# michalfratczak/habdec

Hardware: AMD Instinct MI355X
Metric: IQ Msamples/s (batched 2.048 MS/s streams) (higher is better)
Workload: dtype f32

## Files before the change

### habdec_amd/csrc/dev_types.h

```cpp
#pragma once
#include <stdint.h>
#ifndef __HIPCC__
#ifndef __host__
#define __host__
#define __device__
#endif
#endif

namespace hd {

constexpr int kFftBins = 4096;
constexpr uint32_t kVentLimit = 30000;
constexpr uint32_t kFirBatch = 256;

struct StreamCall {
    uint32_t n_in;
    uint32_t n1;
    uint32_t n2;
    uint32_t zero_hist1;
    uint32_t zero_hist2;
    uint32_t pend_before;
    uint32_t fft_fill;
    uint32_t fft_take;
    uint32_t fft_run;
    uint32_t fir_m;
    uint32_t fir_taps;
    uint32_t fir_zero_hist;
    uint32_t pend_after;
    uint32_t dc_remove;
    uint32_t clear_pending;
    uint32_t fir_taps_prev;
};
__host__ __device__ inline uint32_t sc_taps_prev(const StreamCall& c) { return c.fir_taps_prev & 0xFFFFu; }
__host__ __device__ inline uint32_t sc_head_n(const StreamCall& c) { return (c.fir_taps_prev >> 16) & 0x3FFFu; }
__host__ __device__ inline bool sc_head_prev(const StreamCall& c) { return (c.fir_taps_prev >> 30) & 1u; }
__host__ __device__ inline bool sc_head_save(const StreamCall& c) { return (c.fir_taps_prev >> 31) & 1u; }
__host__ __device__ inline uint32_t sc_pack_taps_prev(uint32_t taps_prev, uint32_t head_n, bool head_prev, bool head_save)
{ return (taps_prev & 0xFFFFu) | ((head_n & 0x3FFFu) << 16) | ((head_prev ? 1u : 0u) << 30) | ((head_save ? 1u : 0u) << 31); }


struct SymbolParams {
    uint32_t spb;
    uint32_t R;
    uint32_t min_held;
    uint32_t float_abs;
    uint32_t reset;
};

struct SymState {
    uint32_t base;
    uint32_t held;
    uint32_t cached;
    uint32_t run_pos;
    float    run_sum;
    uint32_t _pad[3];
};

struct BitsHeader {
    uint32_t nbits;
    uint32_t held_after;
    uint32_t nflips;
    uint32_t overflow;
    uint32_t uncached;
    uint32_t demod_ck[2];
    uint32_t demod_n;
    uint32_t seq;
    uint32_t _pad[3];
};
static_assert(sizeof(BitsHeader) == 48, "result slot header");

struct SpectrumStatsDev {
    int32_t valid;
    int32_t peak1, peak2;
    float power1, power2;
    uint32_t seq;
    double mean, sigma;
};

}
```

### habdec_amd/csrc/engine.cpp

```cpp
#include <hip/hip_runtime.h>
#include <rocfft/rocfft.h>

#include <algorithm>
#include <atomic>
#include <chrono>
#include <cmath>
#include <cstdio>
#include <cstdlib>
#include <cstring>
#include <memory>
#include <condition_variable>
#include <mutex>
#include <thread>
#include <string>
#include <vector>

#include "../../include/habdec_amd.h"
#include "dev_types.h"
#include "host/afc_tracker.hpp"
#include "host/decim_plan.hpp"
#include "host/fir_design.hpp"
#include "host/iq_file_batch.hpp"
#include "host/survey.hpp"
#include "host/text_stage.hpp"
#include "host/tune_host.hpp"
#include "kernels/launch.h"
#include "kernels/survey.h"

#define HDK(fn, ...) (e->fast ? hd::fast::fn(__VA_ARGS__) : hd::exact::fn(__VA_ARGS__))

namespace {

thread_local std::string g_err;
int fail(int code, const std::string& msg) { g_err = msg; return code; }

#define HD_HIP(call)                                                                                   \
    do {                                                                                               \
        hipError_t e_ = (call);                                                                        \
        if (e_ != hipSuccess) return fail(HD_ERR_DEVICE, std::string(#call) + ": " + hipGetErrorString(e_)); \
    } while (0)

template <typename T>
struct DevBuf {
    T* p = nullptr;
    size_t n = 0;
    hipError_t alloc(size_t count)
    {
        n = count;
        hipError_t e = hipMalloc(reinterpret_cast<void**>(&p), std::max<size_t>(count, 1) * sizeof(T));
        if (e == hipSuccess) e = hipMemset(p, 0, std::max<size_t>(count, 1) * sizeof(T));
        return e;
    }
    ~DevBuf() { if (p) (void)hipFree(p); }
};
template <typename T>
struct PinBuf {
    T* p = nullptr;
    T* dev = nullptr;
    size_t n = 0;
    hipError_t alloc(size_t count)
    {
        n = count;
        hipError_t e = hipHostMalloc(reinterpret_cast<void**>(&p), std::max<size_t>(count, 1) * sizeof(T), hipHostMallocMapped | hipHostMallocCoherent);
        if (e == hipSuccess) std::memset(p, 0, std::max<size_t>(count, 1) * sizeof(T));
        if (e == hipSuccess) e = hipHostGetDevicePointer(reinterpret_cast<void**>(&dev), p, 0);
        return e;
    }
    ~PinBuf() { if (p) (void)hipHostFree(p); }
};

struct SizeState {
    size_t stage_buf[2] = {0, 0};
    size_t pending = 0;
    size_t fft_fill = 0;
    size_t fir_buf = 0;
    uint32_t fir_T_run = 0;
    uint32_t head_n = 0;
    uint64_t head_call = ~0ull;
    bool head_aside = false;
    uint32_t tune_phase = 0;
    uint32_t front_phase = 0;
    uint32_t win_ub = 0, inflight_m = 0;
    uint32_t last_n2 = 0, last_pend_before = 0, last_m = 0;
    int last_buf = 0;
};

struct StreamHost {
    double baud = 300;
    float lp_bw = 1500, lp_trans = 0.025f;
    bool dc = false;
    hd::LowpassDesigner lp;
    bool taps_dirty = false;
    uint32_t tune_step = 0;
    uint32_t held = 0;
    bool sym_reset = true;
    hd::TextStage text;
    hd::AfcTracker afc;
    hd::SpectrumStats stats{};
    bool have_spectrum = false;
    uint64_t spectra = 0;
    uint32_t last_nbits = 0, last_nflips = 0;
    uint64_t flip_list_full = 0;
    uint64_t bits_total = 0;
    std::vector<uint32_t> last_words;
    uint32_t demod_ck[2] = {0, 0}, demod_ck_n = 0xFFFFFFFFu;
    uint64_t demod_ck_call = 0;
    uint64_t demod_ck_hash = 0xCBF29CE484222325ull;
    uint64_t demod_ck_calls = 0, demod_ck_unknown = 0;
    double tune_hz = 0;
    uint64_t tune_from = 0, retunes = 0;
    bool auto_afc = false;
    double afc_hold_s = 6.0, afc_min_hz = 100.0;
    uint64_t afc_elapsed = 0;
    double front_hz = 0;
    uint32_t front_step = 0;
    uint64_t front_from = 0;
};

}

struct hd_engine {
    hd_engine_config cfg{};
    double fs = 0, fsd = 0;
    std::vector<hd::DecimStage> stages;
    uint32_t S = 0, D = 1;
    uint32_t n1_cap = 0, n2_cap = 0;
    uint32_t taps_cap = 0, fir_hist_cap = 0;
    size_t fbuf_stride = 0;
    uint32_t tail_cap = 0, backlog_cap = 0, slot_words = 0, flips_cap = 0, max_R = 0, min_R = 4;
    int bins_sep = 8;
    bool decode_enabled = true;
    bool fast = false;
    bool one_stream = false;
    bool no_tail = false;
    uint32_t tail_max_n2 = 2048;
    int last_route = -1;
    struct PendingTail { bool valid = false; hd::TailArgs ta{}; int slot = 0; int r2 = 0, t2 = 0; } pend;
    DevBuf<float2> fft_tw;
    bool no_claim = false;
    uint32_t step_run = 0;
    bool no_cu_step = false;
    uint32_t ring_run = 0;
    uint32_t ring_chain = 1;
    uint32_t ring_short_pct = 25;
    bool ring_short_set = false;
#ifndef HD_S1_SLOTS_BATCH
#define HD_S1_SLOTS_BATCH 4
#endif
    static constexpr uint32_t kS1Slots = HD_S1_SLOTS_BATCH;
    PinBuf<unsigned int> ring_gave_up;
    std::string fail_cause;
    bool device_failed = false;
    uint64_t step_launches = 0;
    DevBuf<unsigned int> step_ctr;
    uint32_t pend_max_taps = 0;
    bool dec_wgs_forced = false;
#ifdef HD_TIMING_EXPERIMENT
    int cu_exp = 0;
#else
    static constexpr int cu_exp = 0;
#endif
    uint32_t n_cus = 0, dec_wgs_per_cu = 0;
    hipStream_t qa = nullptr, qb = nullptr, qc = nullptr;
    hipStream_t qh = nullptr;
    DevBuf<float2> staging2;
    hipEvent_t ev_copy[2] = {nullptr, nullptr}, ev_staging_free[2] = {nullptr, nullptr};
    bool staging_used[2] = {false, false};
    uint64_t host_calls = 0, host_calls_in_place = 0;
    uint32_t timing_every = 8;
    hd_timing last_timing{};
    static constexpr uint32_t kLpFftMinTaps = 1024;
    uint32_t lpf_N[2] = {0, 0};
    rocfft_plan lpf_fwd[2] = {nullptr, nullptr}, lpf_inv[2] = {nullptr, nullptr};
    rocfft_execution_info lpf_info = nullptr;
    DevBuf<char> lpf_workbuf;
    DevBuf<float2> lpf_x, lpf_k;
    PinBuf<uint32_t> lpf_ntaps;
    uint32_t lpf_k_N = 0;
    bool lpf_k_stale = true;
    uint64_t lpf_calls = 0;

    DevBuf<float2> staging, dec1, dec1b, dec1c, hist1[2], hist2[2], fbuf[3], fft_in, spec, filtered;
    DevBuf<float> stage_taps[2], lp_taps, power, demod, tail, weight;
    DevBuf<unsigned long long> flipmask;
    DevBuf<uint32_t> flips_dbg;
    DevBuf<hd::SymState> d_symstate;
    DevBuf<hd::DemodCarry> carry[2];
    DevBuf<float2> fir_head;
    DevBuf<float> tune_tab;
    DevBuf<uint32_t> demod_ck_acc;
    uint32_t head_cap = 0;
    DevBuf<hd::SymbolParams> d_sym;
    PinBuf<hd::SymbolParams> h_sym;
    static constexpr int kSlots = 4;
    struct CallSlot {
        DevBuf<hd::StreamCall> d_call;
        PinBuf<hd::StreamCall> h_call;
        PinBuf<uint32_t> h_slots;
        PinBuf<hd::SpectrumStatsDev> h_stats;
        PinBuf<uint2> h_tune;
        PinBuf<uint2> h_front;
        bool timed = false, timed_step = false;
        hipEvent_t ev_front = nullptr, ev_done = nullptr, ev_params = nullptr, ev_spec = nullptr, t0 = nullptr, t1 = nullptr, t2 = nullptr, t3 = nullptr;
        bool busy = false;
        uint32_t seq = 0;
        uint64_t total_in = 0;
        uint32_t r1 = 1;
        ~CallSlot() { for (hipEvent_t ev : {ev_front, ev_done, ev_params, ev_spec, t0, t1, t2, t3}) if (ev) (void)hipEventDestroy(ev); }
    } slot[kSlots];
    uint64_t calls = 0;
    uint64_t delivered = 0;
    int cur = 0;
    int hist_cur = 0;
    int carry_cur = 0;
    bool sym_dirty = true;

    std::vector<StreamHost> st;
    std::vector<SizeState> mirror, mirror_next;
    std::recursive_mutex mtx;
    bool in_callback = false;
    hd_sentence_cb sentence_cb = nullptr; void* sentence_user = nullptr;
    hd_match_cb match_cb = nullptr; void* match_user = nullptr;
    hd_chars_cb chars_cb = nullptr; void* chars_user = nullptr;
    uint64_t sentences_ok = 0;

    ~hd_engine()
    {
        for (rocfft_plan pl : {lpf_fwd[0], lpf_fwd[1], lpf_inv[0], lpf_inv[1]}) if (pl) rocfft_plan_destroy(pl);
        if (lpf_info) rocfft_execution_info_destroy(lpf_info);
        if (qa) (void)hipStreamDestroy(qa);
        if (qb && qb != qa) (void)hipStreamDestroy(qb);
        if (qc && qc != qa) (void)hipStreamDestroy(qc);
        if (qh) (void)hipStreamDestroy(qh);
        for (hipEvent_t ev : {ev_copy[0], ev_copy[1], ev_staging_free[0], ev_staging_free[1]}) if (ev) (void)hipEventDestroy(ev);
    }
};

namespace {

std::once_flag g_rocfft_once;

hd::SymbolParams symbol_params(const hd_engine* e, const StreamHost& s)
{
    hd::SymbolParams p{};
    p.float_abs = e->cfg.lookup_mode ? 1u : 0u;
    p.min_held = 0xFFFFFFFFu;
    p.spb = 0; p.R = 4;
    if (e->fsd > 0 && s.baud > 0) {
        const double spb = std::round(e->fsd / s.baud);
        if (spb >= 1 && spb < 1e9) {
            p.spb = (uint32_t)spb;
            p.R = (uint32_t)std::max(4, int(p.spb / 4));
            p.min_held = (uint32_t)std::ceil(e->fsd / s.baud * 3);
        }
    }
    return p;
}

float cutoff_rel(const hd_engine* e, const StreamHost& s) { return (float)(s.lp_bw / e->fsd); }

int check_stream(const hd_engine* e, uint32_t s)
{
    if (!e) return fail(HD_ERR_INVALID, "null engine");
    if (s >= e->S) return fail(HD_ERR_INVALID, "stream index out of range");
    return HD_OK;
}

}

extern "C" {

const char* hd_last_error(void) { return g_err.c_str(); }

uint32_t hd_min_chunk(uint32_t decimation)
{
    std::vector<hd::DecimStage> st;
    if (!hd::decim_plan(decimation, st)) return 0;
    uint64_t need = decimation ? decimation : 1;
    uint64_t r = 1;
    for (const auto& g : st) { need = std::max<uint64_t>(need, (uint64_t)(g.taps.size() - 1) * r); r *= (uint64_t)g.ratio; }
    const uint64_t d = decimation ? decimation : 1;
    return (uint32_t)((need + d - 1) / d * d);
}

void hd_engine_config_default(hd_engine_config* c)
{
    std::memset(c, 0, sizeof(*c));
    c->device = 0; c->n_streams = 1; c->max_chunk = 65536; c->sampling_rate = 2.048e6; c->decimation = 64;
    c->baud = 300; c->rtty_bits = 8; c->rtty_stops = 2; c->lowpass_bw_hz = 1500; c->lowpass_trans = 0.025f;
    c->dc_remove = 0; c->lookup_mode = 1; c->enable_spectrum = 1; c->ungated = 0; c->keep_filtered = 0; c->pipeline = 0; c->arith = HD_ARITH_EXACT;
}

int hd_engine_create(const hd_engine_config* cfg, hd_engine** out)
{
    if (!cfg || !out) return fail(HD_ERR_INVALID, "null argument");
    *out = nullptr;
    if (cfg->n_streams < 1) return fail(HD_ERR_INVALID, "n_streams must be >= 1");
    if (!(cfg->sampling_rate > 0)) return fail(HD_ERR_INVALID, "sampling_rate must be > 0");
    if (cfg->max_chunk < 1) return fail(HD_ERR_INVALID, "max_chunk must be >= 1");
    if (cfg->arith != HD_ARITH_EXACT && cfg->arith != HD_ARITH_FAST) return fail(HD_ERR_INVALID, "arith must be HD_ARITH_EXACT (0) or HD_ARITH_FAST (1)");
    std::unique_ptr<hd_engine> e(new hd_engine);
    e->cfg = *cfg;
    e->fast = cfg->arith == HD_ARITH_FAST;
    if (!hd::decim_plan(cfg->decimation, e->stages))
        return fail(HD_ERR_INVALID, "Unsupported decimation factor: " + std::to_string(cfg->decimation));
    e->S = cfg->n_streams;
    e->D = cfg->decimation;
    if (cfg->max_chunk % e->D) return fail(HD_ERR_INVALID, "max_chunk must be a multiple of the decimation factor");
    e->fs = (double)(float)cfg->sampling_rate;
    e->fsd = e->fs / (double)e->D;
    e->decode_enabled = cfg->ungated || !(e->fsd > 4 * 40e3);
    if (cfg->baud > 0 && e->fsd / cfg->baud < 3.5)
        return fail(HD_ERR_UNSUPPORTED, "symbol rate above a third of the decimated rate (fewer than 4 samples per bit): the symbol extractor's windows would overlap");
    {
        const float rel = (float)(500.0f / e->fsd);
        e->bins_sep = std::max(8, (int)std::round((double)rel * (double)hd::kFftBins));
    }

    int ndev = 0;
    if (hipGetDeviceCount(&ndev) != hipSuccess || ndev <= cfg->device || cfg->device < 0)
        return fail(HD_ERR_DEVICE, "no HIP device " + std::to_string(cfg->device) + " (this library has no CPU path)");
    HD_HIP(hipSetDevice(cfg->device));
    HD_HIP(hipStreamCreateWithFlags(&e->qa, hipStreamNonBlocking));
    e->one_stream = cfg->pipeline == 0;
    e->no_tail = getenv("HD_NO_TAIL") != nullptr;
    e->no_claim = getenv("HD_NO_CLAIM") != nullptr;
    if (const char* v = getenv("HD_STEP_RUN")) e->step_run = (uint32_t)atoi(v);
    e->no_cu_step = getenv("HD_NO_CU_STEP") != nullptr;
    if (const char* v = getenv("HD_RING_RUN")) e->ring_run = (uint32_t)atoi(v);
    if (const char* v = getenv("HD_RING_CHAIN")) e->ring_chain = atoi(v) ? 1u : 0u;
    if (const char* v = getenv("HD_RING_SHORT_PCT")) { e->ring_short_pct = std::min<uint32_t>((uint32_t)atoi(v), 100u); e->ring_short_set = true; }
    if (const char* v = getenv("HD_TAIL_MAX_N2")) e->tail_max_n2 = (uint32_t)strtoul(v, nullptr, 0);
    {
        hipDeviceProp_t prop;
        HD_HIP(hipGetDeviceProperties(&prop, cfg->device));
        e->n_cus = (uint32_t)prop.multiProcessorCount;
        e->dec_wgs_per_cu = cfg->pipeline ? 6u : 8u;
        if (const char* v = getenv("HD_DEC_WGS_PER_CU")) { e->dec_wgs_per_cu = (uint32_t)atoi(v); e->dec_wgs_forced = true; }
#ifdef HD_TIMING_EXPERIMENT
        if (const char* v = getenv("HD_CU_EXP")) e->cu_exp = atoi(v);
#endif
    }
    for (hipEvent_t* ev : {&e->ev_copy[0], &e->ev_copy[1], &e->ev_staging_free[0], &e->ev_staging_free[1]}) HD_HIP(hipEventCreateWithFlags(ev, hipEventDisableTiming));
    if (e->one_stream) e->qb = e->qc = e->qa;
    else {
        if (!e->qb) HD_HIP(hipStreamCreateWithFlags(&e->qb, hipStreamNonBlocking));
        HD_HIP(hipStreamCreateWithFlags(&e->qc, hipStreamNonBlocking));
    }
    for (auto& sl : e->slot) {
        static const unsigned ev_flags = (unsigned)hipEventDisableSystemFence;
        HD_HIP(hipEventCreateWithFlags(&sl.ev_front, hipEventDisableTiming | ev_flags));
        HD_HIP(hipEventCreateWithFlags(&sl.ev_done, hipEventDisableTiming | ev_flags));
        HD_HIP(hipEventCreateWithFlags(&sl.ev_params, hipEventDisableTiming | ev_flags));
        HD_HIP(hipEventCreateWithFlags(&sl.ev_spec, hipEventDisableTiming | ev_flags));
        for (hipEvent_t* ev : {&sl.t0, &sl.t1, &sl.t2, &sl.t3}) HD_HIP(hipEventCreateWithFlags(ev, ev_flags));
    }

    const uint32_t S = e->S;
    const uint32_t r0 = e->stages.size() > 0 ? e->stages[0].ratio : 1;
    e->n1_cap = cfg->max_chunk / r0;
    e->n2_cap = cfg->max_chunk / e->D;
    const uint32_t m_cap = ((e->n2_cap + hd::kFirBatch - 1) / hd::kFirBatch) * hd::kFirBatch + hd::kFirBatch;
    e->taps_cap = (m_cap | 1u) + 1u;
    e->fir_hist_cap = (e->taps_cap + 1u) & ~1u;
    e->fbuf_stride = (size_t)e->fir_hist_cap + hd::kFirBatch + e->n2_cap + 2;
    e->fbuf_stride = (e->fbuf_stride + 1) & ~(size_t)1;
    e->backlog_cap = hd::kVentLimit + 1 + m_cap;
    e->tail_cap = 1u;
    while (e->tail_cap < hd::kVentLimit + 1 + m_cap + 1024) e->tail_cap <<= 1;

    e->st.resize(S);
    e->mirror.resize(S);
    e->mirror_next.resize(S);
    for (auto& s : e->st) {
        s.baud = cfg->baud; s.lp_bw = cfg->lowpass_bw_hz; s.lp_trans = cfg->lowpass_trans; s.dc = cfg->dc_remove != 0;
        s.text.framer.nbits = cfg->rtty_bits; s.text.framer.nstops = cfg->rtty_stops;
        s.lp.float_trig = cfg->lookup_mode != 0;
    }
    {
        const hd::SymbolParams p = symbol_params(e.get(), e->st[0]);
        const uint32_t spb = std::max<uint32_t>(p.spb, 1);
        uint32_t bits = 3u * e->backlog_cap / spb + 64u;
        bits = std::max<uint32_t>(256u, (bits + 31u) & ~31u);
        e->slot_words = (uint32_t)(sizeof(hd::BitsHeader) / 4) + bits / 32;
        e->max_R = std::max<uint32_t>(p.R, 4);
        e->min_R = e->max_R;
    }
    e->flips_cap = cfg->keep_filtered ? 256 : 0;

    HD_HIP(e->staging.alloc((size_t)S * cfg->max_chunk));
    if (e->stages.size() == 2) for (auto* b : {&e->dec1, &e->dec1b, &e->dec1c}) HD_HIP(b->alloc((size_t)S * e->n1_cap));
    HD_HIP(e->step_ctr.alloc(2 * 16 * 32 + 32));
    HD_HIP(e->ring_gave_up.alloc(4));
    e->ring_gave_up.p[0] = 0;
    if (!e->no_claim && e->n_cus % 32u == 0) {
        const uint32_t n_xcd = e->n_cus / 32u;
        HD_HIP(hipDeviceSynchronize());
        const uint32_t seen = HDK(probe_xcc_mask, e->qa, e->n_cus, e->step_ctr.p + 2 * 16 * 32);
        if (n_xcd > 16 || seen != (n_xcd >= 32 ? 0xFFFFFFFFu : (1u << n_xcd) - 1u)) e->no_claim = true;
    } else
        e->no_claim = true;
    if (e->stages.size() >= 1) {
        for (auto& h : e->hist1) HD_HIP(h.alloc((size_t)S * (e->stages[0].taps.size() - 1)));
        HD_HIP(e->stage_taps[0].alloc(e->stages[0].taps.size() + 1));
        HD_HIP(hipMemcpy(e->stage_taps[0].p, e->stages[0].taps.data(), e->stages[0].taps.size() * 4, hipMemcpyHostToDevice));
    }
    if (e->stages.size() == 2) {
        for (auto& h : e->hist2) HD_HIP(h.alloc((size_t)S * (e->stages[1].taps.size() - 1)));
        HD_HIP(e->stage_taps[1].alloc(e->stages[1].taps.size() + 1));
        HD_HIP(hipMemcpy(e->stage_taps[1].p, e->stages[1].taps.data(), e->stages[1].taps.size() * 4, hipMemcpyHostToDevice));
    }
    for (auto& b : e->fbuf) HD_HIP(b.alloc((size_t)S * e->fbuf_stride));
    HD_HIP(e->lp_taps.alloc((size_t)S * e->taps_cap));
    HD_HIP(e->demod.alloc((size_t)S * m_cap));
    if (cfg->keep_filtered) HD_HIP(e->filtered.alloc((size_t)S * m_cap));
    HD_HIP(e->tail.alloc((size_t)S * e->tail_cap));
    HD_HIP(e->weight.alloc((size_t)S * e->tail_cap));
    HD_HIP(e->flipmask.alloc((size_t)S * (e->tail_cap / 64)));
    HD_HIP(e->d_symstate.alloc(S));
    if (e->flips_cap) HD_HIP(e->flips_dbg.alloc((size_t)S * e->flips_cap));
    for (auto& c : e->carry) HD_HIP(c.alloc(S));
    e->head_cap = std::min<uint32_t>(e->taps_cap, 8192u);
    HD_HIP(e->fir_head.alloc((size_t)S * e->head_cap));
    HD_HIP(e->demod_ck_acc.alloc((size_t)2 * S));
    HD_HIP(e->d_sym.alloc(S));
    HD_HIP(e->h_sym.alloc(S));
    for (auto& sl : e->slot) {
        HD_HIP(sl.d_call.alloc(S));
        HD_HIP(sl.h_call.alloc(S));
        HD_HIP(sl.h_slots.alloc((size_t)S * e->slot_words));
        HD_HIP(sl.h_tune.alloc(S));
        HD_HIP(sl.h_front.alloc(S));
    }
    {
        std::vector<float> tab(4 * hd::kTuneTable);
        hd::tune_tables(tab.data(), tab.data() + 2 * hd::kTuneTable);
        HD_HIP(e->tune_tab.alloc(tab.size()));
        HD_HIP(hipMemcpy(e->tune_tab.p, tab.data(), tab.size() * sizeof(float), hipMemcpyHostToDevice));
    }
    if (cfg->enable_spectrum) {
        HD_HIP(e->fft_in.alloc((size_t)S * hd::kFftBins));
        HD_HIP(e->spec.alloc((size_t)S * hd::kFftBins));
        HD_HIP(e->power.alloc((size_t)S * hd::kFftBins));
        for (auto& sl : e->slot) HD_HIP(sl.h_stats.alloc(S));
        {
            std::vector<float2> tw(hd::kFftBins);
            for (size_t m = 0; m < hd::kFftBins; ++m) {
                const double a = 2.0 * 3.14159265358979323846264338327950288 * (double)m / (double)hd::kFftBins;
                tw[m] = make_float2((float)std::cos(a), (float)-std::sin(a));
            }
            HD_HIP(e->fft_tw.alloc(hd::kFftBins));
            HD_HIP(hipMemcpy(e->fft_tw.p, tw.data(), tw.size() * sizeof(float2), hipMemcpyHostToDevice));
        }
    }
    if (e->fast && e->taps_cap >= hd_engine::kLpFftMinTaps && getenv("HD_NO_LP_FFT") == nullptr) {
        std::call_once(g_rocfft_once, [] { rocfft_setup(); });
        uint32_t N = 1;
        while (N < m_cap + e->taps_cap) N <<= 1;
        e->lpf_N[1] = N; e->lpf_N[0] = N / 2;
        size_t wmax = 0;
        for (int w = 0; w < 2; ++w) {
            const size_t len = e->lpf_N[w];
            if (rocfft_plan_create(&e->lpf_fwd[w], rocfft_placement_inplace, rocfft_transform_type_complex_forward, rocfft_precision_single, 1, &len, S, nullptr) != rocfft_status_success ||
                rocfft_plan_create(&e->lpf_inv[w], rocfft_placement_inplace, rocfft_transform_type_complex_inverse, rocfft_precision_single, 1, &len, S, nullptr) != rocfft_status_success)
                return fail(HD_ERR_DEVICE, "rocfft_plan_create (low-pass transforms) failed");
            for (rocfft_plan pl : {e->lpf_fwd[w], e->lpf_inv[w]}) { size_t wsz = 0; rocfft_plan_get_work_buffer_size(pl, &wsz); wmax = std::max(wmax, wsz); }
        }
        if (rocfft_execution_info_create(&e->lpf_info) != rocfft_status_success) return fail(HD_ERR_DEVICE, "rocfft_execution_info_create failed");
        if (wmax) { HD_HIP(e->lpf_workbuf.alloc(wmax)); rocfft_execution_info_set_work_buffer(e->lpf_info, e->lpf_workbuf.p, wmax); }
        HD_HIP(e->lpf_x.alloc((size_t)S * N));
        HD_HIP(e->lpf_k.alloc((size_t)S * N));
        HD_HIP(e->lpf_ntaps.alloc(S));
    }
    {
        hd_engine::CallSlot& sl = e->slot[0];
        hipStream_t q = e->qa;
        const uint32_t T1 = e->stages.size() > 0 ? (uint32_t)e->stages[0].taps.size() : 0, T2 = e->stages.size() > 1 ? (uint32_t)e->stages[1].taps.size() : 0;
        if (e->stages.empty()) HDK(launch_passthrough, q, S, 1, e->staging.p, cfg->max_chunk, e->fbuf[0].p, e->fbuf_stride, sl.d_call.p, e->fir_hist_cap);
        if (e->stages.size() >= 1)
            HDK(launch_decimate, q, e->stages[0].ratio, T1, S, 1, e->staging.p, cfg->max_chunk, e->hist1[0].p, e->hist1[1].p, e->stage_taps[0].p,
                                e->stages.size() == 1 ? e->fbuf[0].p : e->dec1.p, e->stages.size() == 1 ? e->fbuf_stride : e->n1_cap, sl.d_call.p, 0,
                                e->stages.size() == 1, e->fir_hist_cap, nullptr);
        if (e->stages.size() >= 1)
            HDK(launch_decimate_tuned, q, e->stages[0].ratio, T1, S, 1, e->staging.p, cfg->max_chunk, e->hist1[0].p, e->hist1[1].p, e->stage_taps[0].p,
                                      e->stages.size() == 1 ? e->fbuf[0].p : e->dec1.p, e->stages.size() == 1 ? e->fbuf_stride : e->n1_cap, sl.d_call.p,
                                      e->stages.size() == 1, e->fir_hist_cap, nullptr, 0u, sl.h_front.dev, e->tune_tab.p);
        if (e->stages.size() == 2)
            HDK(launch_decimate, q, e->stages[1].ratio, T2, S, 1, e->dec1.p, e->n1_cap, e->hist2[0].p, e->hist2[1].p, e->stage_taps[1].p, e->fbuf[0].p,
                                e->fbuf_stride, sl.d_call.p, 1, 1, e->fir_hist_cap, nullptr);
        HDK(launch_chunk_post, q, S, e->fbuf[0].p, e->fbuf_stride, sl.d_call.p, e->fir_hist_cap, nullptr, e->tune_tab.p);
        if (cfg->enable_spectrum) {
            HDK(launch_fft_feed, q, S, e->fbuf[0].p, e->fbuf_stride, e->fft_in.p, sl.d_call.p, e->fir_hist_cap);
            hd::launch_spectrum_wave(q, S, e->fft_in.p, e->fft_tw.p, e->spec.p, e->power.p, sl.h_stats.dev, sl.d_call.p, e->fsd, e->bins_sep, 0u);
        }
        HDK(launch_fir_demod, q, S, 0, 0, e->fbuf[0].p, e->fbuf_stride, e->lp_taps.p, e->taps_cap, e->demod.p, e->demod.n / S, nullptr, e->carry[0].p,
                             e->carry[1].p, sl.d_call.p, e->fir_hist_cap, e->tail.p, e->tail_cap, e->d_symstate.p, e->fbuf[1].p,
                             e->fir_head.p, e->head_cap, e->fbuf[2].p);
        HDK(launch_symbols, q, S, 1, 1, e->max_R, e->tail.p, e->tail_cap, e->d_symstate.p, e->flipmask.p, e->weight.p, e->d_sym.p, sl.d_call.p,
                           sl.h_slots.dev, e->slot_words, nullptr, 0, e->min_R, 0u);
        HD_HIP(hipStreamSynchronize(q));
        HD_HIP(hipGetLastError());
        for (auto& h : e->hist1) if (h.p) HD_HIP(hipMemset(h.p, 0, h.n * sizeof(float2)));
        for (auto& h : e->hist2) if (h.p) HD_HIP(hipMemset(h.p, 0, h.n * sizeof(float2)));
        for (auto& c : e->carry) HD_HIP(hipMemset(c.p, 0, c.n * sizeof(hd::DemodCarry)));
        HD_HIP(hipMemset(e->d_symstate.p, 0, S * sizeof(hd::SymState)));
        if (const char* b0 = getenv("HD_SYM_BASE0")) {
            hd::SymState st0{};
            st0.base = st0.cached = st0.run_pos = (uint32_t)strtoul(b0, nullptr, 0);
            std::vector<hd::SymState> v(S, st0);
            HD_HIP(hipMemcpy(e->d_symstate.p, v.data(), S * sizeof(hd::SymState), hipMemcpyHostToDevice));
        }
    }
    HD_HIP(hipDeviceSynchronize());
    *out = e.release();
    return HD_OK;
}

void hd_engine_destroy(hd_engine* e)
{
    if (!e) return;
    (void)hipSetDevice(e->cfg.device);
    (void)hipDeviceSynchronize();
    delete e;
}
// ... 115 lines not shown
    if (int r = check_stream(e, s)) return r;
    if (!out) return fail(HD_ERR_INVALID, "null argument");
    std::lock_guard<std::recursive_mutex> l(e->mtx);
    const StreamHost& st = e->st[s];
    out->offset_hz = st.front_hz; out->step = st.front_step; out->phase = e->mirror[s].front_phase; out->from_call = st.front_from;
    return HD_OK;
}
int hd_stream_set_auto_afc(hd_engine* e, uint32_t s, int on, double hold_s, double min_hz)
{
    if (int r = check_stream(e, s)) return r;
    if (!(hold_s >= 0) || !(min_hz >= 0)) return fail(HD_ERR_INVALID, "hold_s and min_hz must be >= 0");
    std::lock_guard<std::recursive_mutex> l(e->mtx);
    StreamHost& st = e->st[s];
    st.auto_afc = on != 0; st.afc_hold_s = hold_s; st.afc_min_hz = min_hz; st.afc_elapsed = 0;
    return HD_OK;
}
int hd_stream_tune(hd_engine* e, uint32_t s, hd_tune_info* out)
{
    if (int r = check_stream(e, s)) return r;
    if (!out) return fail(HD_ERR_INVALID, "null argument");
    std::lock_guard<std::recursive_mutex> l(e->mtx);
    const StreamHost& st = e->st[s];
    out->offset_hz = st.tune_hz; out->step = st.tune_step; out->phase = e->mirror[s].tune_phase;
    out->retunes = st.retunes; out->from_call = st.tune_from; out->auto_afc = st.auto_afc ? 1 : 0;
    return HD_OK;
}

}


namespace {

int run_pending_tail(hd_engine* e)
{
    if (!e->pend.valid) return HD_OK;
    hd_engine::CallSlot& ps = e->slot[e->pend.slot];
    e->pend.valid = false;
    hd::TailArgs ta = e->pend.ta;
    const int lanes = (e->S >= 2 * e->n_cus ? 64 : 256);
    hd::TailArgs lay = ta;
    if (lanes != 64) {
        if (!HDK(tail_layout, lay, lanes, e->pend.r2, e->pend.t2, e->pend_max_taps, e->max_R, e->min_R, e->tail_cap, e->pend.ta.pend_max, 64 * 1024)) return fail(HD_ERR_INVALID, "stream tail layout");
    }
    if (!HDK(launch_tail, e->qa, lanes, e->pend.r2, e->pend.t2, e->S, lay, ps.ev_done)) return fail(HD_ERR_INVALID, "stream tail refused a shape it was selected for");
    HD_HIP(hipGetLastError());
    return HD_OK;
}

int collect(hd_engine* e, hd_engine::CallSlot& sl)
{
    if (!sl.busy) return HD_OK;
    if (e->pend.valid && &e->slot[e->pend.slot] == &sl) { if (const int r = run_pending_tail(e)) return r; }
    const auto w0 = std::chrono::steady_clock::now();
    HD_HIP(hipEventSynchronize(sl.ev_done));
    const auto w1 = std::chrono::steady_clock::now();
    sl.busy = false;
    if (sl.timed) {
        float a = 0, b = 0;
        HD_HIP(hipEventElapsedTime(&b, sl.t1, sl.t2));
        if (sl.timed_step) a = b; else HD_HIP(hipEventElapsedTime(&a, sl.t0, sl.t3));
        e->last_timing.ms_total = a;
        e->last_timing.ms_front = b;
        e->last_timing.samples = sl.total_in;
        e->last_timing.front_bytes = sl.total_in * 8 + (sl.total_in / sl.r1) * 8;
        ++e->last_timing.timed_calls;
    }
    int rc = HD_OK;
    {
        const auto t_lim = std::chrono::steady_clock::now() + std::chrono::milliseconds(200);
        const bool timing_experiment = e->cu_exp != 0;
        auto await = [&](const volatile uint32_t* tag, const char* what, uint32_t s) {
            for (uint32_t spins = 0; *tag != sl.seq; ++spins) {
                if (std::chrono::steady_clock::now() > t_lim) {
                    e->device_failed = true;
                    e->fail_cause = std::string(what) + " of stream " + std::to_string(s) + " does not carry its call's tag 200 ms after the completion event";
                    rc = fail(HD_ERR_DEVICE, e->fail_cause + ": the results of this engine are unreliable -- destroy the engine");
                    return;
                }
                if (spins > 64u) std::this_thread::yield();
            }
        };
        for (uint32_t s = 0; s < e->S && !e->device_failed && !timing_experiment; ++s) {
            await(&reinterpret_cast<const volatile hd::BitsHeader*>(sl.h_slots.p + (size_t)s * e->slot_words)->seq, "result slot", s);
            if (!e->device_failed && e->cfg.enable_spectrum && sl.h_stats.p && sl.h_call.p[s].fft_run)
                await(reinterpret_cast<const volatile uint32_t*>(&sl.h_stats.p[s].seq), "spectrum statistics", s);
        }
        std::atomic_thread_fence(std::memory_order_acquire);
    }
    if (e->ring_gave_up.p && e->ring_gave_up.p[0] && !e->device_failed) {
        e->device_failed = true;
        e->fail_cause = "k_stage1_cu (loader / consumer waves): a bounded wait ran out inside a launch (word " + std::to_string(e->ring_gave_up.p[0]) + ")";
    }
    if (e->device_failed && rc == HD_OK)
        rc = fail(HD_ERR_DEVICE, e->fail_cause + ": the results of this and of every later call of this engine are unreliable -- destroy the engine");
    if (e->device_failed) {
        e->last_timing.host_wait_us = std::chrono::duration<double, std::micro>(w1 - w0).count();
        e->last_timing.host_text_us = 0;
        return rc;
    }
    for (uint32_t s = 0; s < e->S; ++s) {
        StreamHost& st = e->st[s];
        const hd::StreamCall& c = sl.h_call.p[s];
        if (c.fft_run) {
            std::memcpy(&st.stats, &sl.h_stats.p[s], sizeof(st.stats));
            st.have_spectrum = true;
            ++st.spectra;
        }
        const bool past_batch_gate = c.fir_m || c.clear_pending;
        if (past_batch_gate && e->cfg.enable_spectrum) st.afc.step(st.have_spectrum, st.stats, hd::kFftBins, e->fsd);
        st.afc_elapsed += c.n_in;
        if (st.auto_afc && (double)st.afc_elapsed >= st.afc_hold_s * e->fs && std::abs(st.afc.correction) > st.afc_min_hz) {
            const double corr = st.afc.correction;
            uint32_t d = 0;
            if (hd::tune_step(st.tune_hz + corr, e->fsd, &d)) {
                st.tune_hz += corr; st.tune_step = d; st.tune_from = e->calls;
                if (!d) e->mirror[s].tune_phase = 0;
                st.afc.reset(corr, hd::kFftBins, e->fsd);
                st.afc_elapsed = 0;
                ++st.retunes;
            }
        }
        const uint32_t* slot = sl.h_slots.p + (size_t)s * e->slot_words;
        const hd::BitsHeader* hdr = reinterpret_cast<const hd::BitsHeader*>(slot);
        SizeState& sz = e->mirror[s];
        st.held = hdr->held_after;
        sz.inflight_m -= c.fir_m;
        sz.win_ub = hdr->uncached + sz.inflight_m;
        st.last_nbits = hdr->nbits; st.last_nflips = hdr->nflips;
        st.bits_total += hdr->nbits;
        st.demod_ck[0] = hdr->demod_ck[0]; st.demod_ck[1] = hdr->demod_ck[1]; st.demod_ck_n = hdr->demod_n; st.demod_ck_call = e->delivered;
        if (hdr->demod_n != 0xFFFFFFFFu) {
            for (const uint32_t x : {hdr->demod_n, hdr->demod_ck[0], hdr->demod_ck[1]}) st.demod_ck_hash = (st.demod_ck_hash ^ x) * 0x100000001B3ull;
            ++st.demod_ck_calls;
        } else ++st.demod_ck_unknown;
        if (hdr->overflow & 1u) rc = fail(HD_ERR_CAPACITY, "symbol result slot overflow on stream " + std::to_string(s));
        if (hdr->overflow & 2u) ++st.flip_list_full;
        const uint32_t* words = slot + sizeof(hd::BitsHeader) / 4;
        st.last_words.assign(words, words + (hdr->nbits + 31) / 32);
        if (!c.fir_m) continue;
        if (hdr->nbits) st.text.framer.push_packed(words, hdr->nbits);
        const std::string chars = st.text.run(hdr->nbits != 0, [&](const hd::SentenceMatch& m) {
            ++e->sentences_ok;
            if (e->sentence_cb) { e->in_callback = true; e->sentence_cb(e->sentence_user, s, m.callsign.c_str(), m.data.c_str(), m.crc.c_str()); e->in_callback = false; }
        }, [&](const hd::SentenceMatch& m, bool ok) {
            if (e->match_cb) { e->in_callback = true; e->match_cb(e->match_user, s, m.callsign.c_str(), m.data.c_str(), m.crc.c_str(), ok ? 1 : 0); e->in_callback = false; }
        });
        if (!chars.empty() && e->chars_cb) { e->in_callback = true; e->chars_cb(e->chars_user, s, chars.data(), chars.size()); e->in_callback = false; }
    }
    e->last_timing.host_wait_us = std::chrono::duration<double, std::micro>(w1 - w0).count();
    e->last_timing.host_text_us = std::chrono::duration<double, std::micro>(std::chrono::steady_clock::now() - w1).count();
    return rc;
}

int deliver(hd_engine* e, uint64_t depth)
{
    int rc = HD_OK;
    while (e->calls - e->delivered > depth) {
        if (const int r = collect(e, e->slot[e->delivered % hd_engine::kSlots])) rc = r;
        ++e->delivered;
    }
    return rc;
}

int flush_locked(hd_engine* e)
{
    if (e->delivered < e->calls) { if (const int r = run_pending_tail(e)) return r; }
    return deliver(e, 0);
}


enum class Route : uint32_t {
    separate = 0,
    tail = 2,
    step = 3,
};

struct CallPlan {
    size_t nst = 0;
    uint32_t R1 = 1, R2 = 1, T1 = 0, T2 = 0;
    uint32_t max_in = 0, min_in = 0xFFFFFFFFu, max_n1 = 0, max_n2 = 0, max_m = 0, max_taps = 0, max_new = 0, max_pend = 0;
    uint64_t total_in = 0;
    bool any_fft = false, any_dc = false, any_zero1 = false, any_tune = false, any_lp_restart = false;
    bool any_front = false;
};

struct CallRoute {
    Route route = Route::separate;
    int tail_lanes = 64;
    hd::TailArgs ta{}, ta_step{};
    bool lean = false, free_front = false, host_params = false, any_post = false, spectrum_on_qc = false;
    const hd::StreamCall* dcall = nullptr;
    float2* feed = nullptr;
};

struct CallBufs {
    float2 *fcur, *fnext, *fprev, *d1;
    int hin, hout, cin, cout;
};

CallBufs call_bufs(const hd_engine* e)
{
    CallBufs b;
    b.fcur = e->fbuf[e->cur].p; b.fnext = e->fbuf[(e->cur + 1) % 3].p; b.fprev = e->fbuf[(e->cur + 2) % 3].p;
    b.d1 = (e->calls % 3 == 0) ? e->dec1.p : (e->calls % 3 == 1) ? e->dec1b.p : e->dec1c.p;
    b.hin = e->hist_cur; b.hout = e->hist_cur ^ 1;
    b.cin = e->carry_cur; b.cout = e->carry_cur ^ 1;
    return b;
}

int plan_call(hd_engine* e, hd_engine::CallSlot& sl, const uint32_t* n_per_stream, uint32_t n_uniform, CallPlan& p, bool& redesigned)
{
    p = CallPlan{};
    p.nst = e->stages.size();
    if (p.nst > 0) { p.R1 = e->stages[0].ratio; p.T1 = (uint32_t)e->stages[0].taps.size(); }
    if (p.nst > 1) { p.R2 = e->stages[1].ratio; p.T2 = (uint32_t)e->stages[1].taps.size(); }
    redesigned = false;
    for (uint32_t s = 0; s < e->S; ++s) {
        StreamHost& st = e->st[s];
        SizeState& nx = e->mirror_next[s];
        nx = e->mirror[s];
        hd::StreamCall c{};
        const uint32_t n = n_per_stream ? n_per_stream[s] : n_uniform;
        c.n_in = n;
        c.n1 = n / p.R1;
        c.n2 = c.n1 / p.R2;
        if (n) {
            if (p.nst > 0) { const size_t want = (size_t)n + p.T1 + p.R1; if (nx.stage_buf[0] < want) { nx.stage_buf[0] = want; c.zero_hist1 = 1; } }
            if (p.nst > 1) { const size_t want = (size_t)c.n1 + p.T2 + p.R2; if (nx.stage_buf[1] < want) { nx.stage_buf[1] = want; c.zero_hist2 = 1; } }
        }
        c.dc_remove = st.dc && c.n2;
        sl.h_tune.p[s] = make_uint2(st.tune_step, nx.tune_phase);
        if (st.tune_step) { p.any_tune = true; nx.tune_phase += c.n2 * st.tune_step; }
        sl.h_front.p[s] = make_uint2(st.front_step, nx.front_phase);
        if (st.front_step | nx.front_phase) { p.any_front = true; nx.front_phase += n * st.front_step; }
        c.pend_before = (uint32_t)nx.pending;
        nx.pending += c.n2;
        c.fft_fill = (uint32_t)nx.fft_fill;
        if (e->cfg.enable_spectrum && n && nx.fft_fill < (size_t)hd::kFftBins && c.n2) {
            c.fft_take = (uint32_t)std::min<size_t>(hd::kFftBins - nx.fft_fill, c.n2);
            nx.fft_fill += c.fft_take;
        }
        if (e->cfg.enable_spectrum && n && nx.fft_fill >= (size_t)hd::kFftBins) { c.fft_run = 1; nx.fft_fill = 0; p.any_fft = true; }
        const bool past_batch_gate = n && nx.pending >= hd::kFirBatch;
        nx.last_m = 0;
        if (past_batch_gate && !e->decode_enabled) { c.clear_pending = 1; nx.pending = 0; }
        else if (past_batch_gate) {
            const uint32_t m = (uint32_t)(nx.pending - nx.pending % hd::kFirBatch);
            st.lp.batch = m;
            if (st.lp.design(cutoff_rel(e, st), st.lp_trans)) {
                st.taps_dirty = true;
                redesigned = true;
            }
            const uint32_t T = (uint32_t)st.lp.taps.size();
            if (!T) return fail(HD_ERR_UNSUPPORTED, "low-pass transition width leaves no taps (reference filters nothing then)");
            if (T > e->taps_cap) return fail(HD_ERR_CAPACITY, "low-pass tap count exceeds engine capacity");
            if (nx.fir_buf < (size_t)m + T) { nx.fir_buf = (size_t)m + T; c.fir_zero_hist = 1; }
            c.fir_m = m; c.fir_taps = T;
            c.fir_taps_prev = hd::sc_pack_taps_prev(nx.fir_T_run ? nx.fir_T_run : T, nx.head_n, !nx.head_aside && nx.head_call + 1 == e->calls, false);
            nx.fir_T_run = T;
            nx.head_n = std::min<uint32_t>(m, std::min<uint32_t>(e->head_cap, 0x3FFFu)); nx.head_call = e->calls; nx.head_aside = false;
            nx.pending -= m;
            nx.last_m = m;
            p.max_m = std::max(p.max_m, m);
            p.max_taps = std::max(p.max_taps, T);
            p.any_lp_restart |= c.fir_zero_hist != 0;
            const uint32_t pending_windows = st.sym_reset ? std::max(st.held, nx.win_ub) : nx.win_ub;
            p.max_new = std::max(p.max_new, pending_windows + m + 64u);
            nx.inflight_m += m;
            nx.win_ub += m;
        }
        if (!c.fir_m && nx.head_n && !nx.head_aside) {
            if (nx.head_call + 1 == e->calls) c.fir_taps_prev = hd::sc_pack_taps_prev(0, nx.head_n, false, true);
            else nx.head_n = 0;
            nx.head_aside = true;
        }
        c.pend_after = (uint32_t)nx.pending;
        p.max_pend = std::max(p.max_pend, std::max(c.pend_before, c.pend_after));
        nx.last_n2 = c.n2; nx.last_pend_before = c.pend_before; nx.last_buf = e->cur;
        sl.h_call.p[s] = c;
        p.max_in = std::max(p.max_in, n); p.min_in = std::min(p.min_in, n); p.max_n1 = std::max(p.max_n1, c.n1); p.max_n2 = std::max(p.max_n2, c.n2);
        p.any_dc |= c.dc_remove != 0;
        p.any_zero1 |= c.zero_hist1 != 0;
        p.total_in += n;
    }
    sl.total_in = p.total_in;
    sl.r1 = p.R1;
    sl.seq = (uint32_t)(e->calls + 1u);
    if (!sl.seq) sl.seq = 1u;
    return HD_OK;
}

void route_call(hd_engine* e, hd_engine::CallSlot& sl, const CallPlan& p, CallRoute& r)
{
    const uint32_t S = e->S;
    const int R2 = (int)p.R2, T2 = (int)p.T2;
    r = CallRoute{};
    r.tail_lanes = S >= 2 * e->n_cus ? 64 : 256;
    const bool tail = p.nst == 2 && !p.any_dc && !e->no_tail && p.max_n2 <= e->tail_max_n2 &&
                      ((r.tail_lanes == 256 && p.max_n2 >= 512u && HDK(tail_layout, r.ta, r.tail_lanes, R2, T2, p.max_taps, e->max_R, e->min_R, e->tail_cap, p.max_pend, 64 * 1024, 4)) ||
                       HDK(tail_layout, r.ta, r.tail_lanes, R2, T2, p.max_taps, e->max_R, e->min_R, e->tail_cap, p.max_pend, 64 * 1024));
    const uint32_t step_lds = (p.R1 == 32 || p.R1 == 64) ? HDK(step_lds_bytes, (int)p.R1, (int)p.T1) : 0u;
    const bool step = tail && !p.any_front && e->cfg.pipeline && !e->one_stream && p.min_in == p.max_in && p.max_in && step_lds &&
                      HDK(tail_layout, r.ta_step, 64, R2, T2, p.max_taps, e->max_R, e->min_R, e->tail_cap, p.max_pend, step_lds);
    r.route = step ? Route::step : tail ? Route::tail : Route::separate;
    r.any_post = p.any_dc || (p.any_tune && !tail);
    r.lean = tail && !e->one_stream;
    r.free_front = !tail && p.nst == 2 && !e->one_stream;
    r.host_params = tail && !step && e->one_stream;
    r.dcall = r.host_params ? sl.h_call.dev : sl.d_call.p;
    r.feed = (e->cfg.enable_spectrum && !r.any_post) ? e->fft_in.p : nullptr;
    if (r.route != Route::separate || !e->cfg.enable_spectrum || r.any_post || !p.any_fft) return;
    for (uint32_t s = 0; s < S; ++s) {
        hd::StreamCall& c = sl.h_call.p[s];
        if (c.fft_run == 1 && c.fft_fill == 0 && c.fft_take == (uint32_t)hd::kFftBins) { c.fft_take = 0; c.fft_run = 2; }
    }
    r.spectrum_on_qc = !e->one_stream && p.nst != 0;
    for (uint32_t s = 0; s < S && r.spectrum_on_qc; ++s) r.spectrum_on_qc = sl.h_call.p[s].fft_run != 1u;
}

void fill_tail(const hd_engine* e, const hd_engine::CallSlot& sl, const CallPlan& p, const CallRoute& r, const CallBufs& b, hd::TailArgs& t)
{
    t.dec1 = b.d1; t.dec1_stride = e->n1_cap; t.hist2_in = e->hist2[b.hin].p; t.hist2_out = e->hist2[b.hout].p; t.taps2 = e->stage_taps[1].p;
    t.fbuf = b.fcur; t.fbuf_next = b.fnext; t.fbuf_stride = e->fbuf_stride; t.fir_hist_cap = e->fir_hist_cap;
    t.lp_taps = e->lp_taps.p; t.taps_stride = e->taps_cap; t.demod = e->demod.p; t.demod_stride = e->demod.n / e->S;
    t.filtered = e->cfg.keep_filtered ? e->filtered.p : nullptr; t.carry_in = e->carry[b.cin].p; t.carry_out = e->carry[b.cout].p;
    t.tune = p.any_tune ? sl.h_tune.dev : nullptr; t.tune_tab = e->tune_tab.p;
    t.call = r.dcall; t.fft_in = r.feed; t.head_buf = e->fir_head.p; t.fbuf_prev = b.fprev; t.head_cap = e->head_cap;
    t.n_streams = e->S;
    t.ring = e->tail.p; t.ring_cap = e->tail_cap; t.sym = e->d_symstate.p; t.flipmask = e->flipmask.p; t.wsum = e->weight.p;
    t.sp = e->d_sym.p; t.slots = sl.h_slots.dev; t.slot_words = e->slot_words; t.seq = sl.seq;
    t.flips_dbg = e->flips_cap ? e->flips_dbg.p : nullptr; t.flips_cap = e->flips_cap;
    t.fft_tw = r.feed ? e->fft_tw.p : nullptr;
    t.spec = e->spec.p; t.power = e->power.p; t.stats = sl.h_stats.dev; t.rate = e->fsd; t.bins_sep = e->bins_sep;
}

hd::StepClaim make_claim(const hd_engine* e, const CallPlan& p, uint32_t run_len_cu )
{
    hd::StepClaim claim{};
    const int R1 = (int)p.R1, T1 = (int)p.T1;
    const uint64_t S = e->S;
    const uint32_t ntiles = run_len_cu ? HDK(ring_tiles, R1, T1, p.max_in) : (p.max_n1 + 63) / 64, n_xcd = e->n_cus / 32u, run_len = run_len_cu ? run_len_cu : e->step_run >= 2 ? e->step_run : 4u;
    const uint64_t runs = S * ntiles / run_len;
    const bool shape_ok = run_len_cu ? (HDK(stage1_cu_supported, R1, T1) && p.max_in % 2048u == 0) : ((R1 == 32 || R1 == 64) && p.max_n1 % 64 == 0);
    if (!e->no_claim && (p.nst == 2 || (run_len_cu && p.nst == 1)) && shape_ok && p.min_in == p.max_in && p.max_in && !p.any_zero1 && n_xcd && e->n_cus % 32u == 0 && n_xcd <= 16 &&
        ntiles && (ntiles % run_len == 0 || (run_len_cu && R1 >= 32 && (S * ntiles) % run_len == 0)) && runs % n_xcd == 0 && S * ntiles < (1ull << 32)) {
        claim.ctr = e->step_ctr.p + (size_t)(e->step_launches & 1u) * 16 * 32;
        claim.ctr_next = e->step_ctr.p + (size_t)((e->step_launches & 1u) ^ 1u) * 16 * 32;
        claim.n_xcd = n_xcd; claim.runs_per_xcd = (uint32_t)(runs / n_xcd); claim.run_len = run_len;
        if (run_len_cu && R1 >= 32 && e->ring_short_pct) {
            const uint32_t tpx = claim.runs_per_xcd * run_len, whole = (uint32_t)((uint64_t)tpx * (100u - e->ring_short_pct) / 100u) / run_len;
            claim.tiles_per_xcd = tpx; claim.short_from = whole; claim.runs_per_xcd = whole + (tpx - whole * run_len);
        }
        if (run_len_cu && R1 == 32 && e->ring_chain && S % n_xcd == 0) {
            const uint32_t hr = (uint32_t)((T1 - 1 + 31) / 32), rows = p.max_in / 32u, rl = e->ring_run >= 2u ? e->ring_run : 4u, sx = (uint32_t)(S / n_xcd);
            const hd::RingSchedule ch = hd::ring_schedule(rows, hr, rl, true), pl = hd::ring_schedule(rows, hr, 1u, false);
            const uint32_t sp = hd::ring_plain_streams(sx, e->ring_short_set ? e->ring_short_pct : 12u);
            if (ch.chained && pl.ntiles && (uint64_t)sx * pl.ntiles < (1ull << 31)) {
                claim.chain_rl = ch.rl; claim.chain_sx = sx; claim.chain_sc = sx - sp;
                claim.chain_nfull = ch.n_full; claim.chain_kclose = ch.k_close; claim.chain_ntp = pl.ntiles;
                claim.runs_per_xcd = hd::ring_tickets(ch, pl, sx, sx - sp);
                claim.run_len = ch.rl; claim.short_from = 0xFFFFFFFFu; claim.tiles_per_xcd = 0;
            }
        }
    }
    return claim;
}

uint32_t pick_ring_run(const hd_engine* e, uint32_t R1, uint32_t ntiles)
{
    const uint64_t S = e->S;
    const uint32_t n_xcd = e->n_cus / 32u ? e->n_cus / 32u : 1u, want = R1 >= 32 ? 4u : 8u;
    auto ok = [&](uint32_t r) { return r >= 2u && r <= ntiles && (R1 >= 32 ? (S * ntiles) % r == 0 : ntiles % r == 0) && (S * ntiles / r) % n_xcd == 0; };
    if (e->ring_run >= 2 && ok(e->ring_run)) return e->ring_run;
    for (uint32_t d = 0; d <= 8u; ++d) {
        if (ok(want + d)) return want + d;
        if (d && d < want && ok(want - d)) return want - d;
    }
    return 2u;
}

int enqueue_uploads(hd_engine* e, hd_engine::CallSlot& sl, const CallRoute& r)
{
    const uint32_t S = e->S;
    hipStream_t qa = e->qa;
    if (e->last_route >= 0 && e->last_route != (int)r.route) {
        if (const int rc = run_pending_tail(e)) return rc;
        HD_HIP(hipStreamSynchronize(qa)); HD_HIP(hipStreamSynchronize(e->qb));
    }
    e->last_route = (int)r.route;
    e->last_timing.path = (uint32_t)r.route;
    if (!r.lean && !r.free_front && e->calls >= 2 && !e->one_stream) HD_HIP(hipStreamWaitEvent(qa, e->slot[(e->calls - 2) % hd_engine::kSlots].ev_done, 0));
    const bool step = r.route == Route::step;
    sl.timed = e->timing_every && (e->calls % e->timing_every) == 0;
    sl.timed_step = sl.timed && step;
    if (sl.timed && !step) HD_HIP(hipEventRecord(sl.t0, qa));
    if (!r.lean && !r.free_front && !r.host_params) {
        HDK(launch_fetch_params, e->qc, sl.h_call.dev, sl.d_call.p, S * sizeof(hd::StreamCall));
        if (!e->one_stream) { HD_HIP(hipEventRecord(sl.ev_params, e->qc)); HD_HIP(hipStreamWaitEvent(qa, sl.ev_params, 0)); }
    }
    for (uint32_t s = 0; s < S; ++s) {
        StreamHost& st = e->st[s];
        if (!st.taps_dirty) continue;
        HD_HIP(hipMemcpyAsync(e->lp_taps.p + (size_t)s * e->taps_cap, st.lp.taps.data(), st.lp.taps.size() * 4, hipMemcpyHostToDevice, qa));
        st.taps_dirty = false;
        e->lpf_k_stale = true;
    }
    if (e->sym_dirty) {
        uint32_t mr = 4;
        for (uint32_t s = 0; s < S; ++s) {
            e->h_sym.p[s] = symbol_params(e, e->st[s]);
            e->h_sym.p[s].reset = e->st[s].sym_reset ? 1u : 0u;
            mr = std::max(mr, e->h_sym.p[s].R);
        }
        e->max_R = mr;
        { uint32_t lo = mr; for (uint32_t s2 = 0; s2 < S; ++s2) lo = std::min(lo, std::max<uint32_t>(e->h_sym.p[s2].R, 4)); e->min_R = lo; }
        HD_HIP(hipMemcpyAsync(e->d_sym.p, e->h_sym.p, S * sizeof(hd::SymbolParams), hipMemcpyHostToDevice, qa));
// ... 102 lines not shown
                                                    call1, 0, single ? 1 : 0, e->fir_hist_cap, single ? r.feed : nullptr, lin1)))
                return fail(HD_ERR_INVALID, "no kernel for this decimation stage");
        }
        if (sl.timed) HD_HIP(hipEventRecord(sl.t2, qa));
        if (r.free_front) HDK(launch_fetch_params, qa, sl.h_call.dev, sl.d_call.p, S * sizeof(hd::StreamCall));
        if (!single && !tail) {
            if (!HDK(launch_decimate, qa, p.R2, p.T2, S, p.max_n2, b.d1, e->n1_cap, e->hist2[b.hin].p, e->hist2[b.hout].p, e->stage_taps[1].p, b.fcur,
                                     e->fbuf_stride, r.dcall, 1, 1, e->fir_hist_cap, r.feed))
                return fail(HD_ERR_INVALID, "no kernel for this decimation stage");
        }
    }
    if (!tail) {
        if (r.any_post) HDK(launch_chunk_post, qa, S, b.fcur, e->fbuf_stride, r.dcall, e->fir_hist_cap, p.any_tune ? sl.h_tune.dev : nullptr, e->tune_tab.p);
        if (!r.spectrum_on_qc) call_spectrum(e, qa, sl, p, r);
    }
    if (!e->one_stream) HD_HIP(hipEventRecord(sl.ev_front, qa));
    if (r.spectrum_on_qc) {
        HD_HIP(hipStreamWaitEvent(e->qc, sl.ev_front, 0));
        call_spectrum(e, e->qc, sl, p, r);
        HD_HIP(hipEventRecord(sl.ev_spec, e->qc));
    }
    return HD_OK;
}

int lowpass_transforms(hd_engine* e, const CallPlan& p, const CallRoute& r, const CallBufs& b, uint32_t* lpN)
{
    *lpN = 0;
    if (!e->fast || !e->lpf_N[1] || p.max_taps < hd_engine::kLpFftMinTaps || !p.max_m || p.any_lp_restart) return HD_OK;
    const uint32_t S = e->S, Lmax = p.max_m + p.max_taps - 1;
    const int w = Lmax <= e->lpf_N[0] ? 0 : Lmax <= e->lpf_N[1] ? 1 : -1;
    if (w < 0) return HD_OK;
    const uint32_t N = e->lpf_N[w];
    hipStream_t qb = e->qb;
    rocfft_execution_info_set_stream(e->lpf_info, qb);
    if (e->lpf_k_stale || e->lpf_k_N != N) {
        for (uint32_t s = 0; s < S; ++s) e->lpf_ntaps.p[s] = (uint32_t)e->st[s].lp.taps.size();
        HDK(launch_lp_taps_gather, qb, S, e->lp_taps.p, e->taps_cap, e->lpf_ntaps.dev, e->lpf_k.p, N);
        void* kb[1] = {e->lpf_k.p};
        if (rocfft_execute(e->lpf_fwd[w], kb, nullptr, e->lpf_info) != rocfft_status_success) return fail(HD_ERR_DEVICE, "rocfft_execute (low-pass taps) failed");
        e->lpf_k_N = N; e->lpf_k_stale = false;
    }
    HDK(launch_lp_gather, qb, S, b.fcur, e->fbuf_stride, e->lpf_x.p, N, r.dcall, e->fir_hist_cap, e->fir_head.p, e->head_cap, b.fprev);
    void* xb[1] = {e->lpf_x.p};
    if (rocfft_execute(e->lpf_fwd[w], xb, nullptr, e->lpf_info) != rocfft_status_success) return fail(HD_ERR_DEVICE, "rocfft_execute (low-pass forward) failed");
    HDK(launch_lp_mul, qb, S, e->lpf_x.p, e->lpf_k.p, N, r.dcall);
    if (rocfft_execute(e->lpf_inv[w], xb, nullptr, e->lpf_info) != rocfft_status_success) return fail(HD_ERR_DEVICE, "rocfft_execute (low-pass inverse) failed");
    ++e->lpf_calls;
    *lpN = N;
    return HD_OK;
}

int enqueue_back(hd_engine* e, hd_engine::CallSlot& sl, const CallPlan& p, CallRoute& r)
{
    const uint32_t S = e->S;
    hipStream_t qb = e->qb;
    const CallBufs b = call_bufs(e);
    if (!e->one_stream) HD_HIP(hipStreamWaitEvent(qb, sl.ev_front, 0));
    const bool ev_ride = !sl.timed && e->one_stream;
    if (r.route == Route::tail) {
        if (r.lean) HDK(launch_fetch_params, qb, sl.h_call.dev, sl.d_call.p, S * sizeof(hd::StreamCall));
        fill_tail(e, sl, p, r, b, r.ta);
        if (!HDK(launch_tail, qb, r.tail_lanes, (int)p.R2, (int)p.T2, S, r.ta, ev_ride ? sl.ev_done : nullptr)) return fail(HD_ERR_INVALID, "stream tail refused a shape it was selected for");
    } else {
        uint32_t lpN = 0;
        if (const int rc = lowpass_transforms(e, p, r, b, &lpN)) return rc;
        HDK(launch_fir_demod, qb, S, p.max_m, lpN ? 0u : p.max_taps, b.fcur, e->fbuf_stride, e->lp_taps.p, e->taps_cap, e->demod.p, e->demod.n / S,
                             e->cfg.keep_filtered ? e->filtered.p : nullptr, e->carry[b.cin].p, e->carry[b.cout].p, r.dcall, e->fir_hist_cap,
                             e->tail.p, e->tail_cap, e->d_symstate.p, b.fnext, e->fir_head.p, e->head_cap, b.fprev, e->demod_ck_acc.p,
                             lpN ? e->lpf_x.p : nullptr, lpN, lpN ? 1.0f / (float)lpN : 1.0f);
        HDK(launch_symbols, qb, S, p.max_m, p.max_new, e->max_R, e->tail.p, e->tail_cap, e->d_symstate.p, e->flipmask.p, e->weight.p, e->d_sym.p,
                           r.dcall, sl.h_slots.dev, e->slot_words, e->flips_cap ? e->flips_dbg.p : nullptr, e->flips_cap, e->min_R, sl.seq, ev_ride ? sl.ev_done : nullptr,
                           e->demod_ck_acc.p);
    }
    if (sl.timed) HD_HIP(hipEventRecord(sl.t3, qb));
    if (r.spectrum_on_qc) HD_HIP(hipStreamWaitEvent(qb, sl.ev_spec, 0));
    if (!ev_ride) HD_HIP(hipEventRecord(sl.ev_done, qb));
    HD_HIP(hipGetLastError());
    return HD_OK;
}

void commit_call(hd_engine* e, hd_engine::CallSlot& sl, const CallPlan& p, const CallRoute& r)
{
    e->mirror.swap(e->mirror_next);
    sl.busy = true;
    if (r.route == Route::step) {
        e->pend.valid = true; e->pend.ta = r.ta_step; e->pend.slot = (int)(e->calls % hd_engine::kSlots);
        e->pend.r2 = (int)p.R2; e->pend.t2 = (int)p.T2; e->pend_max_taps = p.max_taps;
    }
    e->cur = (e->cur + 1) % 3;
    e->carry_cur ^= 1;
    if (p.max_in && p.nst) e->hist_cur ^= 1;
    ++e->calls;
}

}

extern "C" {

int hd_flush(hd_engine* e)
{
    if (!e) return fail(HD_ERR_INVALID, "null engine");
    std::lock_guard<std::recursive_mutex> lock(e->mtx);
    if (e->in_callback) return fail(HD_ERR_INVALID, "hd_flush cannot be called from a sentence / character callback (the delivery it would join is the one running)");
    HD_HIP(hipSetDevice(e->cfg.device));
    const int rc = flush_locked(e);
    if (e->device_failed) return fail(HD_ERR_DEVICE, "this engine is in its failed state (" + e->fail_cause + ") -- destroy the engine");
    return rc;
}

int hd_process_device(hd_engine* e, const void* d_iq, size_t stride, const uint32_t* n_per_stream, uint32_t n_uniform)
{
    if (!e) return fail(HD_ERR_INVALID, "null engine");
    if (!d_iq) return fail(HD_ERR_INVALID, "null IQ pointer");
    if ((reinterpret_cast<uintptr_t>(d_iq) & 15) || (stride & 1)) return fail(HD_ERR_INVALID, "IQ base must be 16-byte aligned and stream_stride even");
    std::lock_guard<std::recursive_mutex> lock(e->mtx);
    if (e->in_callback) return fail(HD_ERR_INVALID, "hd_process_* cannot be called from a sentence / character callback");
    if (e->device_failed) return fail(HD_ERR_DEVICE, "this engine is in its failed state (" + e->fail_cause + "): no new calls are accepted -- destroy the engine");
    const auto h0 = std::chrono::steady_clock::now();
    HD_HIP(hipSetDevice(e->cfg.device));
    const size_t nst = e->stages.size();
    const uint32_t T1 = nst > 0 ? (uint32_t)e->stages[0].taps.size() : 0, T2 = nst > 1 ? (uint32_t)e->stages[1].taps.size() : 0;
    const uint32_t R1 = nst > 0 ? e->stages[0].ratio : 1;

    for (uint32_t s = 0; s < e->S; ++s) {
        const uint32_t n = n_per_stream ? n_per_stream[s] : n_uniform;
        if (n > e->cfg.max_chunk) return fail(HD_ERR_CAPACITY, "more samples than max_chunk");
        if (n % e->D) return fail(HD_ERR_INVALID, "sample count must be a multiple of the decimation factor (queue the remainder)");
        if (n && nst > 0 && n + 1 < T1) return fail(HD_ERR_UNSUPPORTED, "chunk shorter than the first stage's history (undefined in the reference)");
        if (n && nst > 1 && n / R1 + 1 < T2) return fail(HD_ERR_UNSUPPORTED, "chunk shorter than the second stage's history (undefined in the reference)");
    }
    if (const int rc = deliver(e, hd_engine::kSlots - 1)) return rc;
    bool tables_dirty = e->sym_dirty;
    for (uint32_t s = 0; s < e->S && !tables_dirty; ++s) tables_dirty = e->st[s].taps_dirty;
    if (tables_dirty) { if (const int rc = flush_locked(e)) return rc; }
    hd_engine::CallSlot& sl = e->slot[e->calls % hd_engine::kSlots];
    CallPlan p;
    bool redesigned = false;
    do {
        if (redesigned) { if (const int rc = flush_locked(e)) return rc; }
        if (const int rc = plan_call(e, sl, n_per_stream, n_uniform, p, redesigned)) return rc;
    } while (redesigned);
    CallRoute r;
    route_call(e, sl, p, r);

    const float2* iq = static_cast<const float2*>(d_iq);
    int rc = enqueue_uploads(e, sl, r);
    if (!rc) rc = r.route == Route::step ? enqueue_step(e, sl, p, r, iq, stride) : enqueue_front(e, sl, p, r, iq, stride);
    if (!rc && r.route != Route::step) rc = enqueue_back(e, sl, p, r);
    if (rc) {
        e->device_failed = true;
        e->fail_cause = "call " + std::to_string(e->calls) + " was enqueued in part (" + g_err + ")";
        return rc;
    }
    commit_call(e, sl, p, r);
    e->last_timing.host_enqueue_us = std::chrono::duration<double, std::micro>(std::chrono::steady_clock::now() - h0).count();

    const uint64_t depth = !e->cfg.pipeline ? 0u : (r.route == Route::step && e->cfg.pipeline >= 2) ? 3u : 2u;
    return deliver(e, depth);
}

void* hd_pinned_alloc(size_t bytes)
{
    void* p = nullptr;
    if (hipHostMalloc(&p, bytes ? bytes : 1, hipHostMallocMapped | hipHostMallocPortable) != hipSuccess) { (void)hipGetLastError(); return nullptr; }
    return p;
}
// ... 87 lines not shown
            b.alive = src->batch.next(b.iq, stride, b.n.data());
            {
                std::lock_guard<std::mutex> l(m);
                filled = r + 1;
            }
            cv.notify_all();
            if (!b.alive && !looping) return;
        }
    });
    int rc = HD_OK;
    uint64_t total = 0;
    for (uint64_t r = 0; r < max_rounds; ++r) {
        {
            std::unique_lock<std::mutex> l(m);
            cv.wait(l, [&] { return filled > r; });
        }
        Slab& b = slab[r % kSlabs];
        if (!b.alive) {
            if (!looping) break;
            { std::lock_guard<std::mutex> l(m); consumed = r + 1; }
            cv.notify_all();
            continue;
        }
        bool uniform = true;
        for (uint32_t s = 1; s < S; ++s) uniform = uniform && b.n[s] == b.n[0];
        rc = hd_process_host(e, b.iq, stride, uniform ? nullptr : b.n.data(), uniform ? b.n[0] : 0);
        if (rc) break;
        for (uint32_t s = 0; s < S; ++s) total += b.n[s];
        {
            std::lock_guard<std::mutex> l(m);
            consumed = r + 1;
        }
        cv.notify_all();
    }
    {
        std::lock_guard<std::mutex> l(m);
        stop = true;
    }
    cv.notify_all();
    reader.join();
    const int rf = hd_flush(e);
    HD_HIP(hipDeviceSynchronize());
    release();
    if (samples_done) *samples_done = total;
    return rc ? rc : rf;
}


static size_t copy_out(const std::string& s, char* buf, size_t cap)
{
    if (buf && cap) { const size_t n = std::min(cap - 1, s.size()); std::memcpy(buf, s.data(), n); buf[n] = 0; }
    return s.size();
}
static size_t take_out(std::string& s, char* buf, size_t cap)
{
    const size_t n = copy_out(s, buf, cap);
    if (buf && cap > n) s.clear();
    return n;
}

size_t hd_stream_rtty(hd_engine* e, uint32_t s, char* buf, size_t cap)
{ if (check_stream(e, s)) return 0; std::lock_guard<std::recursive_mutex> l(e->mtx); return copy_out(e->st[s].text.stream, buf, cap); }
size_t hd_stream_last_sentence(hd_engine* e, uint32_t s, char* buf, size_t cap)
{ if (check_stream(e, s)) return 0; std::lock_guard<std::recursive_mutex> l(e->mtx); return copy_out(e->st[s].text.last_sentence, buf, cap); }
size_t hd_stream_take_sentences(hd_engine* e, uint32_t s, char* buf, size_t cap)
{ if (check_stream(e, s)) return 0; std::lock_guard<std::recursive_mutex> l(e->mtx); return take_out(e->st[s].text.ok_log, buf, cap); }
size_t hd_stream_take_matches(hd_engine* e, uint32_t s, char* buf, size_t cap)
{ if (check_stream(e, s)) return 0; std::lock_guard<std::recursive_mutex> l(e->mtx); return take_out(e->st[s].text.match_log, buf, cap); }
size_t hd_stream_take_chars(hd_engine* e, uint32_t s, char* buf, size_t cap)
{ if (check_stream(e, s)) return 0; std::lock_guard<std::recursive_mutex> l(e->mtx); return take_out(e->st[s].text.char_log, buf, cap); }

int hd_stream_afc(hd_engine* e, uint32_t s, hd_afc_info* out)
{
    if (int r = check_stream(e, s)) return r;
    if (!out) return fail(HD_ERR_INVALID, "null argument");
    std::lock_guard<std::recursive_mutex> l(e->mtx);
    const StreamHost& st = e->st[s];
    out->frequency_correction = st.afc.correction; out->shift_hz = st.afc.shift_hz;
    out->noise_floor = st.afc.noise_floor; out->noise_variance = st.afc.noise_sigma;
    out->peak_left = st.afc.gui_left; out->peak_right = st.afc.gui_right; out->spectra = st.spectra;
    return HD_OK;
}

static size_t fetch(hd_engine* e, const void* dev, size_t count, size_t elem, void* host, size_t cap)
{
    if (e->in_callback) { fail(HD_ERR_INVALID, "data getters cannot be called from a sentence / character callback (text getters can)"); return 0; }
    (void)flush_locked(e);
    const size_t n = std::min(count, cap);
    if (!n || !host) return count;
    if (hipSetDevice(e->cfg.device) != hipSuccess) return 0;
    if (hipMemcpy(host, dev, n * elem, hipMemcpyDeviceToHost) != hipSuccess) return 0;
    return count;
}

size_t hd_stream_spectrum(hd_engine* e, uint32_t s, float* iq, size_t cap)
{
    if (check_stream(e, s)) return 0;
    std::lock_guard<std::recursive_mutex> l(e->mtx);
    if (!e->cfg.enable_spectrum || !e->st[s].have_spectrum) return 0;
    return fetch(e, e->spec.p + (size_t)s * hd::kFftBins, hd::kFftBins, sizeof(float2), iq, cap);
}
size_t hd_stream_power(hd_engine* e, uint32_t s, float* p, size_t cap)
{
    if (check_stream(e, s)) return 0;
    std::lock_guard<std::recursive_mutex> l(e->mtx);
    if (!e->cfg.enable_spectrum || !e->st[s].have_spectrum) return 0;
    return fetch(e, e->power.p + (size_t)s * hd::kFftBins, hd::kFftBins, sizeof(float), p, cap);
}
size_t hd_stream_demodulated(hd_engine* e, uint32_t s, float* v, size_t cap)
{
    if (check_stream(e, s)) return 0;
    std::lock_guard<std::recursive_mutex> l(e->mtx);
    return fetch(e, e->demod.p + (size_t)s * (e->demod.n / e->S), e->mirror[s].last_m, sizeof(float), v, cap);
}
size_t hd_stream_decimated(hd_engine* e, uint32_t s, float* iq, size_t cap)
{
    if (check_stream(e, s)) return 0;
    std::lock_guard<std::recursive_mutex> l(e->mtx);
    const SizeState& sz = e->mirror[s];
    const float2* src = e->fbuf[sz.last_buf].p + (size_t)s * e->fbuf_stride + e->fir_hist_cap + sz.last_pend_before;
    return fetch(e, src, sz.last_n2, sizeof(float2), iq, cap);
}
size_t hd_stream_filtered(hd_engine* e, uint32_t s, float* iq, size_t cap)
{
    if (check_stream(e, s)) return 0;
    std::lock_guard<std::recursive_mutex> l(e->mtx);
    if (!e->cfg.keep_filtered) return 0;
    return fetch(e, e->filtered.p + (size_t)s * (e->demod.n / e->S), e->mirror[s].last_m, sizeof(float2), iq, cap);
}
size_t hd_stream_bits(hd_engine* e, uint32_t s, uint8_t* bits, size_t cap)
{
    if (check_stream(e, s)) return 0;
    std::lock_guard<std::recursive_mutex> l(e->mtx);
    const StreamHost& st = e->st[s];
    for (uint32_t i = 0; i < st.last_nbits && i < cap; ++i) bits[i] = (st.last_words[i >> 5] >> (i & 31)) & 1u;
    return st.last_nbits;
}
size_t hd_stream_flips(hd_engine* e, uint32_t s, uint32_t* flips, size_t cap)
{
    if (check_stream(e, s)) return 0;
    std::lock_guard<std::recursive_mutex> l(e->mtx);
    if (!e->flips_cap) return 0;
    const size_t n = std::min<size_t>(e->st[s].last_nflips, e->flips_cap);
    return fetch(e, e->flips_dbg.p + (size_t)s * e->flips_cap, n, sizeof(uint32_t), flips, cap);
}
size_t hd_stream_fir_taps(hd_engine* e, uint32_t s, float* taps, size_t cap)
{
    if (check_stream(e, s)) return 0;
    std::lock_guard<std::recursive_mutex> l(e->mtx);
    const auto& t = e->st[s].lp.taps;
    if (taps) std::memcpy(taps, t.data(), std::min(cap, t.size()) * sizeof(float));
    return t.size();
}
uint64_t hd_stream_bits_total(hd_engine* e, uint32_t s)
{
    if (check_stream(e, s)) return 0;
    std::lock_guard<std::recursive_mutex> l(e->mtx);
    return e->st[s].bits_total;
}
uint64_t hd_stream_flip_list_full(hd_engine* e, uint32_t s)
{
    if (check_stream(e, s)) return 0;
    std::lock_guard<std::recursive_mutex> l(e->mtx);
    return e->st[s].flip_list_full;
}
int hd_stream_demod_checksum(hd_engine* e, uint32_t s, uint64_t* call_index, uint32_t* n, uint32_t ck[2])
{
    if (check_stream(e, s)) return HD_ERR_INVALID;
    std::lock_guard<std::recursive_mutex> l(e->mtx);
    const StreamHost& st = e->st[s];
    if (call_index) *call_index = st.demod_ck_call;
    if (n) *n = st.demod_ck_n;
    if (ck) { ck[0] = st.demod_ck[0]; ck[1] = st.demod_ck[1]; }
    return HD_OK;
}
int hd_stream_demod_checksum_total(hd_engine* e, uint32_t s, uint64_t* calls, uint64_t* calls_without, uint64_t* hash)
{
    if (check_stream(e, s)) return HD_ERR_INVALID;
    std::lock_guard<std::recursive_mutex> l(e->mtx);
    const StreamHost& st = e->st[s];
    if (calls) *calls = st.demod_ck_calls;
    if (calls_without) *calls_without = st.demod_ck_unknown;
    if (hash) *hash = st.demod_ck_hash;
    return HD_OK;
}
uint32_t hd_stream_symbol_backlog(hd_engine* e, uint32_t s)
{
    if (check_stream(e, s)) return 0;
    std::lock_guard<std::recursive_mutex> l(e->mtx);
    return e->st[s].held;
}

}


struct hd_survey {
// ... 201 lines not shown
```

### habdec_amd/csrc/kernels/decimate.hip

```cpp
#include <hip/hip_runtime.h>
#include <hip/hip_ext.h>
#include <type_traits>
#include <cstdlib>

#include "launch.h"
#include "tune.h"
#include "tail_body.h"
#include "stage1_ring.h"

#ifndef HD_FRONT_SWEEPS
#define HD_FRONT_SWEEPS 2
#endif
#define HD_DEC_MAXW 4

namespace hd {
namespace HD_ARITH_NS {

#ifdef HD_STAMP_DEC
#ifndef HD_STAMP_DEC_D
#define HD_STAMP_DEC_D 32
#endif
__device__ unsigned long long g_dec_stamps[4096 * 8];
extern "C" void HD_DBG_NAME(hd_debug_dec_stamps)(unsigned long long* host, size_t n) { (void)hipMemcpyFromSymbol(host, HIP_SYMBOL(g_dec_stamps), n * 8); }
#define DSTAMP_DECL unsigned long long ds_t = __builtin_amdgcn_s_memtime(), ds_acc[4] = {0, 0, 0, 0}; const unsigned long long ds_r0 = __builtin_amdgcn_s_memrealtime(); unsigned long long ds_r1 = 0
#define DSTAMP(i) do { if (D == HD_STAMP_DEC_D) { const unsigned long long t_ = __builtin_amdgcn_s_memtime(); ds_acc[i] += t_ - ds_t; ds_t = t_; } } while (0)
#define DSTAMP_ARRIVED() do { if (D == HD_STAMP_DEC_D) { asm volatile("s_waitcnt vmcnt(0)" ::: "memory"); DSTAMP(0); if (!ds_r1) ds_r1 = __builtin_amdgcn_s_memrealtime(); } } while (0)
#define DSTAMP_WRITE() do { if (D == HD_STAMP_DEC_D && threadIdx.x == 0) { const uint32_t w_ = by * gdx + bx; if (w_ < 4096) { \
        unsigned long long* g_ = g_dec_stamps + w_ * 8; g_[0] = ds_r0; g_[1] = ds_r1; g_[2] = __builtin_amdgcn_s_memrealtime(); \
        g_[3] = ds_acc[0]; g_[4] = ds_acc[1]; g_[5] = ds_acc[2]; g_[6] = ds_acc[3]; g_[7] = count; } } } while (0)
#else
#define DSTAMP_DECL do { } while (0)
#define DSTAMP(i) do { } while (0)
#define DSTAMP_ARRIVED() do { } while (0)
#define DSTAMP_WRITE() do { } while (0)
#endif

template <int D> constexpr int dec_opl() { return D == 2 ? 4 : D == 4 ? 4 : D == 8 ? 2 : 1; }

template <int D, int T, int TO>
constexpr int dec_tile_f4()
{
    constexpr int OPL = dec_opl<D>(), TOUT = TO * OPL, RD = OPL * D, JS = (T - 1) & 1;
    constexpr int NJJ = (TOUT - 1) * D + T + JS, NL = NJJ + 2 * (NJJ / RD) + 4;
    return (NL + 1) / 2 + TOUT / 2 + 1;
}

#ifdef HD_STAMP_TAIL
extern "C" void HD_DBG_NAME(hd_debug_step_tail_stamps)(unsigned long long* host, size_t n) { (void)hipMemcpyFromSymbol(host, HIP_SYMBOL(g_tail_stamps), n * 8); }
#endif

template <bool TUNED> struct FrontTune { static constexpr bool staged = false; };
template <> struct FrontTune<true> { uint2 tn, tn_next; bool staged; };

template <int D, int T, int TO, bool TUNED = false>
__device__ __forceinline__ void decimate_body(const float2* __restrict__ in, size_t in_stride,
                                              const float2* __restrict__ hist_in, float2* __restrict__ hist_out,
                                              const float* __restrict__ taps,
                                              float2* __restrict__ out, size_t out_stride,
                                              const StreamCall* __restrict__ call, int stage, int final_stage,
                                              uint32_t fir_hist_cap, uint32_t tiles_per_wg, float2* __restrict__ fft_in,
                                              uint32_t n_streams, uint32_t lin_ntiles, StreamCall* __restrict__ call_copy,
                                              const uint32_t bx, const uint32_t by, const uint32_t gdx, float4* __restrict__ tile4,
                                              const uint32_t uniform_n = 0 ,
                                              const StepClaim claim = StepClaim{} ,
                                              const uint2* __restrict__ ftune = nullptr ,
                                              const float* ftab = nullptr )
{
    constexpr int OPL = dec_opl<D>();
    constexpr int TOUT = TO * OPL;
    constexpr int RD = OPL * D;
    constexpr int JS = (T - 1) & 1;
    constexpr int NJ = (TOUT - 1) * D + T;
    constexpr int NJJ = NJ + JS;
    constexpr int NL = NJJ + 2 * (NJJ / RD) + 4;
    constexpr int NP = (NJJ + 1) / 2;
    constexpr int ITER = (NP + TO - 1) / TO;
    static_assert((NL + 1) / 2 + TOUT / 2 + 1 == dec_tile_f4<D, T, TO>(), "tile size helper out of step");
    float2* tile = reinterpret_cast<float2*>(tile4);
    float2* ytile = tile + ((NL + 1) & ~1);

    struct CallHead { uint32_t n_in, n1, n2, zero_hist1, zero_hist2, pend_before, fft_fill, fft_take; };
    static_assert(sizeof(CallHead) == 32, "CallHead mirrors the head of StreamCall");
    const bool linear = lin_ntiles != 0;
    uint32_t s, first, count;
    const bool claimed = claim.ctr != nullptr && claim.run_len >= 2;
    unsigned int* my_ctr = nullptr;
    unsigned int* next_ctr = nullptr;
    auto retire = [&]() { if (threadIdx.x == 0) (void)__hip_atomic_exchange(next_ctr, 0u, __ATOMIC_RELAXED, __HIP_MEMORY_SCOPE_AGENT); };
    auto draw = [&]() -> unsigned int { unsigned int t = 0; if (threadIdx.x == 0) t = __hip_atomic_fetch_add(my_ctr, 1u, __ATOMIC_RELAXED, __HIP_MEMORY_SCOPE_AGENT); return t; };
    auto drawn = [&](unsigned int t) -> unsigned int { return (unsigned int)__builtin_amdgcn_readfirstlane((int)t); };
    uint32_t xcd = 0;
    unsigned int ticket = 0;
    bool jump = false; uint32_t jump_s = 0, jump_first = 0;
    if (claimed) {
        xcd = __builtin_amdgcn_s_getreg((3 << 11) | (0 << 6) | 20) & 15u;
        if (xcd >= claim.n_xcd) xcd = claim.n_xcd - 1;
        my_ctr = claim.ctr + (size_t)xcd * 32;
        next_ctr = claim.ctr_next + (size_t)xcd * 32;
        const unsigned int r = drawn(draw());
        if (r >= claim.runs_per_xcd) { if (r == claim.runs_per_xcd) retire(); return; }
        const uint32_t g0 = (xcd * claim.runs_per_xcd + r) * claim.run_len;
        s = g0 / lin_ntiles;
        first = g0 - s * lin_ntiles;
        count = claim.run_len;
    } else if (linear) {
        const uint64_t total = (uint64_t)n_streams * lin_ntiles;
        const uint64_t g0 = (uint64_t)bx * total / gdx, g1 = (uint64_t)(bx + 1) * total / gdx;
        s = (uint32_t)(g0 / lin_ntiles);
        first = (uint32_t)(g0 - (uint64_t)s * lin_ntiles);
        count = (uint32_t)(g1 - g0);
    } else {
        s = by; first = bx * tiles_per_wg; count = tiles_per_wg;
    }
    CallHead c{};
    if (uniform_n) { c.n_in = c.n1 = uniform_n; }
    else c = *reinterpret_cast<const CallHead*>(call + s);
    const uint32_t n = stage == 0 ? c.n_in : c.n1;
    const uint32_t nout = n / D;
    const uint32_t ntiles = (nout + TOUT - 1) / TOUT;
    if (!linear) {
        if (!n && bx == 0)
            for (uint32_t j = threadIdx.x; j < (uint32_t)(T - 1); j += TO)
                hist_out[(size_t)s * (T - 1) + j] = hist_in[(size_t)s * (T - 1) + j];
        if (first >= ntiles) return;
        count = min(first + tiles_per_wg, ntiles) - first;
    }
    if (!count) return;
    uint32_t pf_s = s;
    bool pf_zero_hist = (stage == 0 ? c.zero_hist1 : c.zero_hist2) != 0;
    CallHead c_next = c;
    FrontTune<TUNED> ft;
    if constexpr (TUNED) { ft.tn = ftune[s]; ft.tn_next = ft.tn; }

    float4 r[ITER];
    auto load_tile = [&](uint32_t tile_i, const bool fast) {
        const float2* in_s = in + (size_t)pf_s * in_stride;
        const float2* hist_s = hist_in + (size_t)pf_s * (T - 1);
        const bool zero_hist = pf_zero_hist;
        auto locate = [&](long xi, bool& ok) -> const float2* {
            const bool in_hist = xi < 0;
            ok = in_hist ? (!zero_hist && xi >= -(long)(T - 1)) : (xi < (long)n);
            const long hi = xi + (T - 1);
            const float2* ph = hist_s + (hi < 0 ? 0 : hi);
            const float2* pi = in_s + (xi < 0 ? 0 : (xi < (long)n ? xi : 0));
            return in_hist ? ph : pi;
        };
        const long xe = (long)tile_i * TOUT * D - (T - 1) - JS;
        const float4* src = reinterpret_cast<const float4*>(in_s + xe);
        if (fast && __builtin_amdgcn_readfirstlane((int)(xe >= 0 && xe + 2L * ITER * TO <= (long)n))) {
            const uint64_t b64 = reinterpret_cast<uint64_t>(src);
            const char* base = reinterpret_cast<const char*>(((uint64_t)(uint32_t)__builtin_amdgcn_readfirstlane((int)(uint32_t)(b64 >> 32)) << 32) |
                                                             (uint64_t)(uint32_t)__builtin_amdgcn_readfirstlane((int)(uint32_t)b64));
            const uint32_t lane_off = threadIdx.x * 16u;
#pragma unroll
            for (int it = 0; it < ITER; ++it) r[it] = *reinterpret_cast<const float4*>(base + (lane_off + (uint32_t)it * (TO * 16u)));
            return;
        }
        uint32_t tid_ = threadIdx.x;
        asm volatile("" : "+v"(tid_));
#pragma unroll
        for (int it = 0; it < ITER; ++it) {
            const int k = (int)tid_ + it * TO;
            const long lo = xe + 2L * it * TO, hi = lo + 2L * TO;
            if (lo >= 0 && hi <= (long)n) {
                r[it] = src[k];
// ... 187 lines not shown
    #pragma unroll
                    for (int q = 0; q < B / 2; ++q) x[q] = *reinterpret_cast<const float4*>(pb + 2 * q + 2 * ((2 * q) / D));
    #pragma unroll
                    for (int q = 0; q < B / 2; ++q) {
                        mac(x[q].x, x[q].y, tb[2 * q]);
                        mac(x[q].z, x[q].w, tb[2 * q + 1]);
                    }
                }
            }
            if (NS >= B && NS % B) {
                constexpr int J0 = NFULL * B;
    #pragma unroll
                for (int jj = J0; jj < NS; jj += 2) {
                    const float4 x = *reinterpret_cast<const float4*>(p + jj + 2 * (jj / D));
                    mac(x.x, x.y, taps[jj - JS]);
                    if (jj + 1 < NS) mac(x.z, x.w, taps[jj + 1 - JS]);
                }
            }
            yq[0] = make_float2(ar, ai);
        } else {
            float ar[OPL], ai[OPL];
#pragma unroll
            for (int q = 0; q < OPL; ++q) { ar[q] = 0.f; ai[q] = 0.f; }
            constexpr int B = 16;
            constexpr int W = (OPL - 1) * D + T + JS;
            constexpr int NB = (W + B - 1) / B;
            constexpr int B_LO = (JS + (OPL - 1) * D + B - 1) / B;
            constexpr int B_HI = (T + JS) / B - 1;
            auto edge_block = [&](auto bc) {
                HD_FIR_ARITH
                constexpr int j0 = decltype(bc)::value * B;
#pragma unroll
                for (int k = 0; k < B; k += 2) {
                    if (j0 + k < W) {
                        const float4 x = *reinterpret_cast<const float4*>(p + j0 + k + 2 * ((j0 + k) / RD));
#pragma unroll
                        for (int q = 0; q < OPL; ++q) {
                            const int t0 = j0 + k - JS - q * D, t1 = t0 + 1;
                            if (t0 >= 0 && t0 < T) { ar[q] = ar[q] + x.x * taps[t0]; ai[q] = ai[q] + x.y * taps[t0]; }
                            if (t1 >= 0 && t1 < T) { ar[q] = ar[q] + x.z * taps[t1]; ai[q] = ai[q] + x.w * taps[t1]; }
                        }
                    }
                }
            };
            auto for_blocks = [&](auto lo, auto hi, auto self) {
                if constexpr (decltype(lo)::value < decltype(hi)::value) {
                    edge_block(lo);
                    self(std::integral_constant<int, decltype(lo)::value + 1>{}, hi, self);
                }
            };
            constexpr int HEAD_END = B_LO < NB ? (B_LO <= B_HI ? B_LO : NB) : NB;
            for_blocks(std::integral_constant<int, 0>{}, std::integral_constant<int, HEAD_END>{}, for_blocks);
            if constexpr (B_LO <= B_HI) {
#pragma unroll 1
                for (int b = B_LO; b <= B_HI; ++b) {
                    HD_FIR_ARITH
                    const int j0 = b * B;
                    const float2* pb = p + j0 + 2 * (j0 / RD);
                    const float* tb = taps + (j0 - JS);
                    float4 x[B / 2];
#pragma unroll
                    for (int k = 0; k < B / 2; ++k) x[k] = *reinterpret_cast<const float4*>(pb + 2 * k + 2 * ((2 * k) / RD));
#pragma unroll
                    for (int k = 0; k < B / 2; ++k) {
#pragma unroll
                        for (int q = 0; q < OPL; ++q) {
                            const float k0 = tb[2 * k - q * D], k1 = tb[2 * k + 1 - q * D];
                            ar[q] = ar[q] + x[k].x * k0; ai[q] = ai[q] + x[k].y * k0;
                            ar[q] = ar[q] + x[k].z * k1; ai[q] = ai[q] + x[k].w * k1;
                        }
                    }
                }
                for_blocks(std::integral_constant<int, B_HI + 1>{}, std::integral_constant<int, NB>{}, for_blocks);
            }
#pragma unroll
            for (int q = 0; q < OPL; ++q) yq[q] = make_float2(ar[q], ai[q]);
        }
        const uint32_t o = (tile_i * TO + threadIdx.x) * OPL;
#pragma unroll
        for (int q = 0; q < OPL; ++q) { y_prev[q] = yq[q]; ytile[threadIdx.x * OPL + q] = yq[q]; }
        nv_prev = o < nout ? min((uint32_t)OPL, nout - o) : 0u;
        dst_prev = out + (size_t)s * out_stride + (final_stage ? (size_t)fir_hist_cap + c.pend_before : 0) + o;
        nf_prev = (fft_in && o < c.fft_take) ? min((uint32_t)OPL, c.fft_take - o) : 0u;
        fdst_prev = fft_in ? fft_in + (size_t)s * kFftBins + c.fft_fill + o : nullptr;
        __syncthreads();
        DSTAMP(3);
        ++tile_i;
        const bool seam = tile_i == ntiles;
        if (seam) {
            if (n) {
                float2* hout = hist_out + (size_t)s * (T - 1);
                const float2* in_s = in + (size_t)s * in_stride;
                for (uint32_t j = threadIdx.x; j < (uint32_t)(T - 1); j += TO) {
                    const uint32_t idx = n - (T - 1) + j;
                    if constexpr (TUNED) {
                        const uint2 tn = ft.tn;
                        const float2 x = in_s[idx];
                        float yr = x.x, yi = x.y;
                        if (tn.x | tn.y) tune_rotate1(ftab, tn.y + idx * tn.x, x.x, x.y, yr, yi);
                        hout[j] = idx < nout ? ytile[idx] : make_float2(yr, yi);
                    } else
                    hout[j] = idx < nout ? ytile[idx] : in_s[idx];
                }
            }
            if (!jump && done + 1 < count) {
                __syncthreads();
                ++s; tile_i = 0; c = c_next;
                if constexpr (TUNED) ft.tn = ft.tn_next;
                leave_copy(s);
            }
        }
        if (jump) {
            __syncthreads();
            s = jump_s; tile_i = jump_first; jump = false;
            if constexpr (TUNED) ft.tn = ftune[s];
            if (!tile_i) leave_copy(s);
        }
    }
    store_prev();
    flush_copy();
    DSTAMP_WRITE();
}

template <int D, int T, int TO>
__global__ __launch_bounds__(TO) __attribute__((amdgpu_waves_per_eu(D == 64 ? 1 : 2, TO == 64 ? 2 : HD_DEC_MAXW))) void k_decimate(const float2* __restrict__ in, size_t in_stride,
                                                   const float2* __restrict__ hist_in, float2* __restrict__ hist_out,
                                                   const float* __restrict__ taps,
                                                   float2* __restrict__ out, size_t out_stride,
                                                   const StreamCall* __restrict__ call, int stage, int final_stage,
                                                   uint32_t fir_hist_cap, uint32_t tiles_per_wg, float2* __restrict__ fft_in,
                                                   uint32_t n_streams, uint32_t lin_ntiles)
{
    __shared__ float4 tile4[dec_tile_f4<D, T, TO>()];
    decimate_body<D, T, TO>(in, in_stride, hist_in, hist_out, taps, out, out_stride, call, stage, final_stage, fir_hist_cap, tiles_per_wg, fft_in,
                            n_streams, lin_ntiles, nullptr, blockIdx.x, blockIdx.y, gridDim.x, tile4);
}

template <int TO> constexpr bool front_tab_in_lds()
{
#ifdef HD_FRONT_TAB_GLOBAL
    return false;
#else
    return TO > 64;
#endif
}

template <int D, int T, int TO>
__global__ __launch_bounds__(TO) __attribute__((amdgpu_waves_per_eu(D == 64 ? 1 : 2, TO == 64 ? 2 : HD_DEC_MAXW))) void k_decimate_tuned(const float2* __restrict__ in, size_t in_stride,
                                                   const float2* __restrict__ hist_in, float2* __restrict__ hist_out,
                                                   const float* __restrict__ taps,
                                                   float2* __restrict__ out, size_t out_stride,
                                                   const StreamCall* __restrict__ call, int final_stage,
                                                   uint32_t fir_hist_cap, uint32_t tiles_per_wg, float2* __restrict__ fft_in,
                                                   uint32_t n_streams, uint32_t lin_ntiles,
                                                   const uint2* __restrict__ ftune, const float* __restrict__ ftab)
{
    constexpr bool kLds = front_tab_in_lds<TO>();
    __shared__ float4 tile4[dec_tile_f4<D, T, TO>()];
    __shared__ float4 tab4[kLds ? kTuneTable : 1];
    if constexpr (kLds) {
        for (uint32_t i = threadIdx.x; i < kTuneTable; i += TO) tab4[i] = reinterpret_cast<const float4*>(ftab)[i];
        __syncthreads();
    }
    decimate_body<D, T, TO, true>(in, in_stride, hist_in, hist_out, taps, out, out_stride, call, 0, final_stage, fir_hist_cap, tiles_per_wg, fft_in,
                                  n_streams, lin_ntiles, nullptr, blockIdx.x, blockIdx.y, gridDim.x, tile4, 0u, StepClaim{}, ftune,
                                  kLds ? reinterpret_cast<const float*>(tab4) : ftab);
}
// ... 363 lines not shown
```

### habdec_amd/csrc/kernels/fir_demod.hip

```cpp
#include <hip/hip_runtime.h>

#include "arith.h"
#include "exact_math.h"
#include "launch.h"

namespace hd {
namespace HD_ARITH_NS {

#ifdef HD_STAMP_FIR
__device__ unsigned long long g_fir_stamps[8192 * 8];
extern "C" void HD_DBG_NAME(hd_debug_fir_stamps)(unsigned long long* host, size_t n) { (void)hipMemcpyFromSymbol(host, HIP_SYMBOL(g_fir_stamps), n * 8); }
#define FSTAMP_DECL unsigned long long fs_t = __builtin_amdgcn_s_memtime(), fs_acc[4] = {0, 0, 0, 0}; const unsigned long long fs_r0 = __builtin_amdgcn_s_memrealtime()
#define FSTAMP(i) do { const unsigned long long t_ = __builtin_amdgcn_s_memtime(); fs_acc[i] += t_ - fs_t; fs_t = t_; } while (0)
#define FSTAMP_WRITE() do { const uint32_t w_ = blockIdx.y * gridDim.x + blockIdx.x; if (threadIdx.x == 64 && w_ < 8192) { unsigned long long* g_ = g_fir_stamps + w_ * 8; \
        g_[0] = fs_r0; g_[1] = __builtin_amdgcn_s_memrealtime(); for (int i_ = 0; i_ < 4; ++i_) g_[2 + i_] = fs_acc[i_]; g_[6] = 1; } } while (0)
#else
#define FSTAMP_DECL do { } while (0)
#define FSTAMP(i) do { } while (0)
#define FSTAMP_WRITE() do { } while (0)
#endif

constexpr int kFirLanes = 256;
#ifndef HD_FIR_OUT
#define HD_FIR_OUT 6
// ... 142 lines not shown
        for (uint32_t t = nblk * 16u; t < T; ++t) {
            HD_FIR_ARITH
            const float kt = tp[t];
            const float2* x = lds + (uint32_t)kFirOut * threadIdx.x + t;
            fd_f32x2 pr[kFirOut];
#pragma unroll
            for (int q = 0; q < kFirOut; ++q) { const float2 v = x[q]; pr[q] = fd_f32x2{v.x, v.y} * kt; }
#pragma unroll
            for (int q = 0; q < kFirOut; ++q) acc[q] = acc[q] + pr[q];
        }
    }
    }
    FSTAMP(2);
    __syncthreads();
    if (active) {
#pragma unroll
        for (int q = 0; q < kFirOut; q += 2)
            reinterpret_cast<float4*>(lds)[(uint32_t)(kFirOut / 2) * threadIdx.x + (uint32_t)(q / 2)] = make_float4(acc[q].x, acc[q].y, acc[q + 1].x, acc[q + 1].y);
    }
    if (threadIdx.x < 2) s_ck[threadIdx.x] = 0u;
    __syncthreads();

    if (threadIdx.x != 0 && active) {
    const long i = i0 + (long)kFirOut * (long)threadIdx.x;
    float pr, pi;
    if (i > 0) { const float2 q = lds[kFirOut * threadIdx.x - 1]; pr = q.x; pi = q.y; }
    else {
        const DemodCarry kc = carry_in[s];
        if (kc.primed) { pr = kc.re; pi = kc.im; } else { pr = acc[0].x; pi = acc[0].y; }
    }
    const uint32_t nv = (uint32_t)min((long)kFirOut, (long)m - i);
    float d[kFirOut];
    d[0] = discriminate(acc[0].x, acc[0].y, pr, pi);
#pragma unroll
    for (int q = 1; q < kFirOut; ++q) d[q] = (uint32_t)q < nv ? discriminate(acc[q].x, acc[q].y, acc[q - 1].x, acc[q - 1].y) : 0.f;
    float* dm = demod + (size_t)s * demod_stride + i;
#pragma unroll
    for (int q = 0; q < kFirOut; q += 2) {
        if ((uint32_t)q + 1u < nv) *reinterpret_cast<float2*>(dm + q) = make_float2(d[q], d[q + 1]);
        else if ((uint32_t)q < nv) dm[q] = d[q];
    }
    if (sym_ring) {
        const SymState st = sym[s];
        float* ring = sym_ring + (size_t)s * ring_cap;
        const uint32_t pos = st.base + st.held + (uint32_t)i;
#pragma unroll
        for (int q = 0; q < kFirOut; ++q) if ((uint32_t)q < nv) ring[(pos + (uint32_t)q) & (ring_cap - 1)] = d[q];
    }
    if (filtered) {
#pragma unroll
        for (int q = 0; q < kFirOut; ++q) if ((uint32_t)q < nv) filtered[(size_t)s * demod_stride + i + q] = make_float2(acc[q].x, acc[q].y);
    }
    const long last = (long)m - 1;
    if (i <= last && last < i + (long)kFirOut) {
        DemodCarry kc; kc.primed = 1; kc._pad = 0;
        fd_f32x2 y = acc[0];
#pragma unroll
        for (int q = 1; q < kFirOut; ++q) if (last == i + q) y = acc[q];
        kc.re = y.x; kc.im = y.y;
        carry_out[s] = kc;
    }
    if (ck_acc) {
        uint32_t c0 = 0, c1 = 0;
#pragma unroll
        for (int q = 0; q < kFirOut; ++q) if ((uint32_t)q < nv) { const uint32_t b = __builtin_bit_cast(uint32_t, d[q]); c0 += b; c1 += ((uint32_t)i + (uint32_t)q + 1u) * b; }
        atomicAdd(&s_ck[0], c0); atomicAdd(&s_ck[1], c1);
    }
    }
    if (ck_acc) {
        __syncthreads();
        if (threadIdx.x < 2) atomicAdd(&ck_acc[2 * (size_t)s + threadIdx.x], s_ck[threadIdx.x]);
    }
    FSTAMP(3);
    FSTAMP_WRITE();
}

__global__ void k_fft_feed(const float2* __restrict__ fbuf, size_t stride, float2* __restrict__ fft_in,
                           const StreamCall* __restrict__ call, uint32_t fir_hist_cap)
{
    const uint32_t s = blockIdx.y;
    const StreamCall c = call[s];
    const uint32_t j = blockIdx.x * blockDim.x + threadIdx.x;
    if (j >= c.fft_take) return;
    fft_in[(size_t)s * kFftBins + c.fft_fill + j] = fbuf[(size_t)s * stride + fir_hist_cap + c.pend_before + j];
}

__global__ void k_fetch_params(const uint4* __restrict__ host_src, uint4* __restrict__ dst, uint32_t n16)
{
    const uint32_t i = blockIdx.x * blockDim.x + threadIdx.x;
    if (i < n16) dst[i] = host_src[i];
}

void launch_fetch_params(hipStream_t st, const void* host_mapped, void* dst, size_t bytes)
{
    const uint32_t n16 = (uint32_t)((bytes + 15) / 16);
    hipLaunchKernelGGL(k_fetch_params, dim3((n16 + 255) / 256), dim3(256), 0, st, static_cast<const uint4*>(host_mapped), static_cast<uint4*>(dst), n16);
}

void launch_fir_demod(hipStream_t st, uint32_t n_streams, uint32_t max_m, uint32_t max_taps, const float2* fbuf, size_t stride,
                      const float* taps, uint32_t taps_stride, float* demod, size_t demod_stride, float2* filtered,
                      const DemodCarry* carry_in, DemodCarry* carry_out, const StreamCall* call, uint32_t fir_hist_cap,
                      float* sym_ring, uint32_t ring_cap, const SymState* sym, float2* fbuf_next,
                      float2* head_side, uint32_t head_cap, const float2* fbuf_prev, uint32_t* ck_acc,
                      const float2* pre, uint32_t pre_stride, float pre_scale)
{
    const uint32_t tiles = max_m ? (max_m + kFirAdvance - 1) / kFirAdvance : 1;
    const size_t lds = (size_t)(kFirTile + (max_taps ? max_taps : 1) + kFirSlack + 4) * sizeof(float2);
    dim3 grid(tiles, n_streams);
    hipLaunchKernelGGL(k_fir_demod, grid, dim3(kFirLanes), lds, st, fbuf, stride, taps, taps_stride, demod, demod_stride, filtered,
                       carry_in, carry_out, call, fir_hist_cap, sym_ring, ring_cap, sym, fbuf_next, head_side, head_cap, fbuf_prev, ck_acc, pre, pre_stride, pre_scale);
}

__global__ __launch_bounds__(256) void k_lp_gather(const float2* __restrict__ fbuf, size_t stride, float2* __restrict__ work, uint32_t N, const StreamCall* __restrict__ call,
                                                    uint32_t fir_hist_cap, const float2* __restrict__ head_side, uint32_t head_cap, const float2* __restrict__ fbuf_prev)
{
    const uint32_t s = blockIdx.y;
    const StreamCall c = call[s];
    const uint32_t m = c.fir_m, T = c.fir_taps;
    if (!m || !T) return;
    const uint32_t Tp = sc_taps_prev(c) ? sc_taps_prev(c) : T, H = T - 1, L = H + m;
    const float2* buf = fbuf + (size_t)s * stride;
    const bool refold = Tp != T && !c.fir_zero_hist;
    const uint32_t head_n = refold ? sc_head_n(c) : 0u;
    const float2* head_in = sc_head_prev(c) ? fbuf_prev + (size_t)s * stride + fir_hist_cap : head_side + (size_t)s * head_cap;
    float2* w = work + (size_t)s * N;
    for (uint32_t j = blockIdx.x * 256u + threadIdx.x; j < N; j += gridDim.x * 256u) {
        float2 v = make_float2(0.f, 0.f);
        if (j < L) {
            if (j >= H) v = buf[fir_hist_cap + (j - H)];
            else if (c.fir_zero_hist) v = make_float2(0.f, 0.f);
            else if (!refold) v = buf[fir_hist_cap - H + j];
            else if (j < Tp - 1) v = buf[fir_hist_cap - (Tp - 1) + j];
            else if (j - (Tp - 1) < head_n) v = head_in[j - (Tp - 1)];
        }
        w[j] = v;
    }
}
__global__ __launch_bounds__(256) void k_lp_taps_gather(const float* __restrict__ taps, uint32_t taps_stride, const uint32_t* __restrict__ ntaps, float2* __restrict__ kf, uint32_t N)
{
    const uint32_t s = blockIdx.y, T = ntaps[s];
    for (uint32_t j = blockIdx.x * 256u + threadIdx.x; j < N; j += gridDim.x * 256u)
        kf[(size_t)s * N + j] = make_float2(j < T ? taps[(size_t)s * taps_stride + j] : 0.f, 0.f);
}
__global__ __launch_bounds__(256) void k_lp_mul(float2* __restrict__ work, const float2* __restrict__ kf, uint32_t N, const StreamCall* __restrict__ call)
{
    const uint32_t s = blockIdx.y;
    if (!call[s].fir_m || !call[s].fir_taps) return;
    for (uint32_t j = blockIdx.x * 256u + threadIdx.x; j < N; j += gridDim.x * 256u) {
        const float2 x = work[(size_t)s * N + j], k = kf[(size_t)s * N + j];
        work[(size_t)s * N + j] = make_float2(x.x * k.x + x.y * k.y, x.y * k.x - x.x * k.y);
    }
}
void launch_lp_gather(hipStream_t st, uint32_t n_streams, const float2* fbuf, size_t stride, float2* work, uint32_t N, const StreamCall* call, uint32_t fir_hist_cap,
                      const float2* head_side, uint32_t head_cap, const float2* fbuf_prev)
{
    hipLaunchKernelGGL(k_lp_gather, dim3((N + 1023) / 1024, n_streams), dim3(256), 0, st, fbuf, stride, work, N, call, fir_hist_cap, head_side, head_cap, fbuf_prev);
}
void launch_lp_taps_gather(hipStream_t st, uint32_t n_streams, const float* taps, uint32_t taps_stride, const uint32_t* ntaps, float2* kf, uint32_t N)
{
    hipLaunchKernelGGL(k_lp_taps_gather, dim3((N + 1023) / 1024, n_streams), dim3(256), 0, st, taps, taps_stride, ntaps, kf, N);
}
void launch_lp_mul(hipStream_t st, uint32_t n_streams, float2* work, const float2* kf, uint32_t N, const StreamCall* call)
{
    hipLaunchKernelGGL(k_lp_mul, dim3((N + 1023) / 1024, n_streams), dim3(256), 0, st, work, kf, N, call);
}

void launch_fft_feed(hipStream_t st, uint32_t n_streams, const float2* fbuf, size_t stride, float2* fft_in, const StreamCall* call,
// ... 9 lines not shown
```

### habdec_amd/csrc/kernels/launch.h

```cpp
#pragma once
#include <hip/hip_runtime.h>
#include <stddef.h>
#include <stdint.h>

#include "../dev_types.h"
#include "../host/ring_schedule.hpp"

namespace hd {

struct DemodCarry {
    float re, im;
    uint32_t primed;
    uint32_t _pad;
};

struct StepClaim {
    unsigned int* ctr = nullptr;
    unsigned int* ctr_next = nullptr;
    uint32_t n_xcd = 0, runs_per_xcd = 0, run_len = 0;
    uint32_t short_from = 0xFFFFFFFFu, tiles_per_xcd = 0;
    uint32_t chain_rl = 0, chain_sx = 0, chain_sc = 0;
    uint32_t chain_nfull = 0, chain_kclose = 0, chain_ntp = 0;
};

struct TailArgs {
    const float2* dec1; size_t dec1_stride;
    const float2* hist2_in; float2* hist2_out; const float* taps2;
    float2* fbuf; float2* fbuf_next; size_t fbuf_stride; uint32_t fir_hist_cap;
    const float* lp_taps; uint32_t taps_stride;
    float* demod; size_t demod_stride; float2* filtered;
    const DemodCarry* carry_in; DemodCarry* carry_out;
    const StreamCall* call; float2* fft_in;
    float2* head_buf ; const float2* fbuf_prev ; uint32_t head_cap, n_streams;
    float* ring; uint32_t ring_cap; SymState* sym; unsigned long long* flipmask; float* wsum; const SymbolParams* sp;
    uint32_t* slots; uint32_t slot_words; uint32_t* flips_dbg; uint32_t flips_cap;
    uint32_t seq;
    const float2* fft_tw; float2* spec; float* power; SpectrumStatsDev* stats; double rate; int bins_sep;
    uint32_t pend_max, f_off, v_off, ws_off, words_off, tp_off, h2_off, flips_off, fl_cap, strips_off, dyn_off, lds_bytes;
    uint32_t op;
    const uint2* tune; const float* tune_tab;
};

constexpr uint32_t kStepLdsBytes = 20480;

void launch_spectrum_wave(hipStream_t st, uint32_t n_streams, const float2* fft_in, const float2* tw4096, float2* spec, float* power,
                          SpectrumStatsDev* stats, const StreamCall* call, double rate, int bins_sep,
                          uint32_t seq ,
                          const float2* chunk = nullptr ,
                          size_t chunk_stride = 0, uint32_t fir_hist_cap = 0);

namespace exact {
#include "launch_decls.inc"
}
namespace fast {
#include "launch_decls.inc"
}

}
```

### habdec_amd/csrc/kernels/spectrum_wave.h

```cpp
#pragma once
#include <hip/hip_runtime.h>

#include "launch.h"
#include "sym_common.h"

namespace hd {

namespace specwave {

__device__ static constexpr float kW64[2][32] = {
#include "fft64_tw.inc"
};

constexpr int xpos(int k) { return 8 * (k & 7) + (k >> 3); }

__device__ __forceinline__ void fft8(f32x2 (&v)[8])
{
    constexpr float r = 0.70710678118654752440f;
    const f32x2 a0 = v[0] + v[4], a1 = v[0] - v[4], a2 = v[2] + v[6], a3 = v[2] - v[6];
    const f32x2 a4 = v[1] + v[5], a5 = v[1] - v[5], a6 = v[3] + v[7], a7 = v[3] - v[7];
    const f32x2 a3r = (f32x2){a3.y, -a3.x}, a7r = (f32x2){a7.y, -a7.x};
    const f32x2 b0 = a0 + a2, b2 = a0 - a2, b1 = a1 + a3r, b3 = a1 - a3r;
    const f32x2 b4 = a4 + a6, b6 = a4 - a6, b5 = a5 + a7r, b7 = a5 - a7r;
    const f32x2 t5 = (f32x2){(b5.x + b5.y) * r, (b5.y - b5.x) * r};
// ... 34 lines not shown
        fft8(v);
#pragma unroll
        for (int k2 = 0; k2 < 8; ++k2) a[8 * k1 + k2] = v[k2];
    }
    __builtin_amdgcn_sched_barrier(0);
}

__device__ __forceinline__ void pin64(f32x2 (&a)[64])
{
#pragma unroll
    for (int i = 0; i < 64; ++i) asm volatile("" : "+v"(a[i]));
}

template <int G>
__device__ __forceinline__ void finish4096(f32x2 (&a)[64], const float2* __restrict__ tw4096, float* __restrict__ plane, const uint32_t l)
{
#pragma unroll
    for (int g = 0; g < 64; g += G) {
        __builtin_amdgcn_sched_barrier(0);
        float2 w[G];
#pragma unroll
        for (int u = 0; u < G; ++u) w[u] = tw4096[(l * (uint32_t)xpos(g + u)) & (kFftBins - 1)];
#pragma unroll
        for (int u = 0; u < G; ++u) {
            const f32x2 v = a[g + u];
            a[g + u] = (f32x2){v.x * w[u].x - v.y * w[u].y, v.x * w[u].y + v.y * w[u].x};
        }
    }
    __builtin_amdgcn_sched_barrier(0);
#pragma unroll
    for (int k1 = 0; k1 < 64; ++k1) plane[k1 * 65 + l] = a[xpos(k1)].x;
    __builtin_amdgcn_s_waitcnt(0xC07F);
    __builtin_amdgcn_wave_barrier();
#pragma unroll
    for (int n2 = 0; n2 < 64; ++n2) a[n2].x = plane[l * 65 + n2];
    __builtin_amdgcn_s_waitcnt(0xC07F);
    __builtin_amdgcn_wave_barrier();
#pragma unroll
    for (int k1 = 0; k1 < 64; ++k1) plane[k1 * 65 + l] = a[xpos(k1)].y;
    __builtin_amdgcn_s_waitcnt(0xC07F);
    __builtin_amdgcn_wave_barrier();
#pragma unroll
    for (int n2 = 0; n2 < 64; ++n2) a[n2].y = plane[l * 65 + n2];
    pin64(a);
    fft64(a);
    pin64(a);
}

__device__ __forceinline__ double wave_sum(double v)
{
    for (int off = 32; off > 0; off >>= 1) v += __shfl_down(v, off, 64);
    return __shfl(v, 0, 64);
}

__device__ __forceinline__ void wave_argmax(float& v, int& idx)
{
    for (int off = 32; off > 0; off >>= 1) {
        const float ov = __shfl_down(v, off, 64);
        const int oi = __shfl_down(idx, off, 64);
        if (ov > v || (ov == v && oi < idx)) { v = ov; idx = oi; }
    }
    v = __shfl(v, 0, 64); idx = __shfl(idx, 0, 64);
}

}

constexpr uint32_t kSpecWaveLds = 64 * 65 * 4;

__device__ __forceinline__ void spectrum_wave_body(const float2* __restrict__ x, const float2* __restrict__ tw4096, float2* __restrict__ spec,
                                                   float* __restrict__ power, SpectrumStatsDev* __restrict__ stats, const uint32_t s, const double rate,
                                                   const int bins_sep, float* __restrict__ plane, const uint32_t seq)
{
    const uint32_t l = threadIdx.x & 63u;
    f32x2 a[64];
#pragma unroll
    for (int g = 0; g < 64; g += 8) {
        const float2* xg = x + 64 * g;
        asm volatile("" : "+s"(xg));
#pragma unroll
        for (int u = 0; u < 8; ++u) { const float2 v = xg[64 * u + l]; a[g + u] = (f32x2){v.x, v.y}; }
    }
    specwave::fft64(a);
    specwave::finish4096<16>(a, tw4096, plane, l);
    float2* so = spec + (size_t)s * kFftBins;
    float* po = power + (size_t)s * kFftBins;
    int mybad = 0;
    double lsum = 0.0;
#define HD_SW_P(j_) a[specwave::xpos(((j_) + 32) & 63)].x
    float2* sg = so;
    float* pg = po;
#pragma unroll
    for (int j = 0; j < 64; ++j) {
        if ((j & 7) == 0) {
            __builtin_amdgcn_sched_barrier(0);
            sg = so + 64 * j; pg = po + 64 * j;
            asm volatile("" : "+s"(sg), "+s"(pg));
        }
        const int k2 = (j + 32) & 63;
        const f32x2 v = a[specwave::xpos(k2)];
        sg[l + 64 * (j & 7)] = make_float2(v.x, v.y);
        float q = (v.x * v.x + v.y * v.y) / (float)kFftBins;
        q = q * q;
        q = (float)((double)q / rate);
        q = 10.0f * log10f(q);
        if (v.x != v.x || v.y != v.y || isinf(v.x) || isinf(v.y) || q != q || isinf(q)) mybad = 1;
        HD_SW_P(j) = q;
        pg[l + 64 * (j & 7)] = q;
        lsum += (double)q;
    }
    const bool bad = __builtin_amdgcn_ballot_w64(mybad != 0) != 0ull;
    const double mean = specwave::wave_sum(lsum) / (double)kFftBins;
    double lvar = 0.0;
    float bv = -__builtin_huge_valf();
    int bi = kFftBins;
#pragma unroll
    for (int j = 0; j < 64; ++j) {
        const float pj = HD_SW_P(j);
        const double d = (double)pj - mean;
        lvar += d * d;
        if (pj > bv) { bv = pj; bi = (int)l + 64 * j; }
    }
    const double sigma = sqrt(specwave::wave_sum(lvar) / (double)kFftBins);
    specwave::wave_argmax(bv, bi);
    const int p1 = bi;
    const float p1v = bv;
    const int lo = max(p1 - 2 * bins_sep, 0), hi = min(p1 + 2 * bins_sep, (int)kFftBins);
    const float floor0 = __shfl(HD_SW_P(0), 0, 64);
    float cv = -__builtin_huge_valf();
    int ci = kFftBins;
#pragma unroll
    for (int j = 0; j < 64; ++j) {
        const int i = (int)l + 64 * j;
        const float pj = HD_SW_P(j);
        if (i >= lo && i < hi && pj > floor0 && abs(i - p1) > bins_sep / 2 && pj > cv) { cv = pj; ci = i; }
    }
    specwave::wave_argmax(cv, ci);
    if (l == 0) {
        int pa = p1, pb = 0;
        float av = p1v, bvv = floor0;
        if (ci < (int)kFftBins) { pb = ci; bvv = cv; }
        if (pb < pa) { const int ti = pa; pa = pb; pb = ti; const float tv = av; av = bvv; bvv = tv; }
        SpectrumStatsDev o;
        o.valid = bad ? 0 : 1;
        o.peak1 = pa; o.peak2 = pb; o.power1 = av; o.power2 = bvv; o.seq = 0u;
        o.mean = mean; o.sigma = sigma;
        stats[s] = o;
        asm volatile("s_waitcnt vmcnt(0)" ::: "memory");
        __hip_atomic_store(&stats[s].seq, seq, __ATOMIC_RELAXED, __HIP_MEMORY_SCOPE_SYSTEM);
    }
#undef HD_SW_P
}

}
```

### habdec_amd/csrc/kernels/spectrum_wave.hip

```cpp
#include <hip/hip_runtime.h>

#include "spectrum_wave.h"

namespace hd {

__global__ __launch_bounds__(64) __attribute__((amdgpu_waves_per_eu(2, 2))) void k_spectrum_wave(const float2* __restrict__ fft_in, const float2* __restrict__ tw4096, float2* __restrict__ spec,
                                                        float* __restrict__ power, SpectrumStatsDev* __restrict__ stats,
                                                        const StreamCall* __restrict__ call, double rate, int bins_sep, const uint32_t seq,
                                                        const float2* __restrict__ chunk, const size_t chunk_stride, const uint32_t fir_hist_cap)
{
    __shared__ float plane[64 * 65];
    const uint32_t s = blockIdx.x;
    const uint32_t run = call[s].fft_run;
    if (!run) return;
    const float2* x = run == 2u ? chunk + (size_t)s * chunk_stride + fir_hist_cap + call[s].pend_before : fft_in + (size_t)s * kFftBins;
    spectrum_wave_body(x, tw4096, spec, power, stats, s, rate, bins_sep, plane, seq);
}

void launch_spectrum_wave(hipStream_t st, uint32_t n_streams, const float2* fft_in, const float2* tw4096, float2* spec, float* power,
                          SpectrumStatsDev* stats, const StreamCall* call, double rate, int bins_sep, uint32_t seq, const float2* chunk, size_t chunk_stride, uint32_t fir_hist_cap)
{
    hipLaunchKernelGGL(k_spectrum_wave, dim3(n_streams), dim3(64), 0, st, fft_in, tw4096, spec, power, stats, call, rate, bins_sep, seq, chunk, chunk_stride, fir_hist_cap);
}

}
```

### habdec_amd/csrc/kernels/stage1_ring.h

```cpp
#pragma once
#include <hip/hip_runtime.h>

#include "arith.h"
#include "launch.h"

namespace hd {
namespace HD_ARITH_NS {

typedef float r_f32x2 __attribute__((ext_vector_type(2)));
typedef float r_f32x4 __attribute__((ext_vector_type(4)));

constexpr int kRingRowBytes = 272;
constexpr int kRingNSLAlone = 4;
constexpr int kWorkSlotBytes = 64 * kRingRowBytes;
constexpr int kWorkKeepBytes = 128;
constexpr int kStepCtlBytes = 256 + 5 * kWorkKeepBytes;
constexpr int kRingCtlBytes = 384;
constexpr uint32_t kRingSpinLimit = 1u << 22;
template <int T> constexpr int ring_halo_rows() { return (T - 1 + 31) / 32; }
template <int T> constexpr int ring_slot_bytes() { return (64 + ring_halo_rows<T>()) * kRingRowBytes; }
template <int T, int NSL = kRingNSLAlone> constexpr int ring_bytes() { return 2 * NSL * ring_slot_bytes<T>() + kRingCtlBytes; }
template <int T> constexpr int ring_adv() { return 64 - ring_halo_rows<T>(); }

__host__ __device__ constexpr uint32_t ring_sys_tiles(uint32_t n, uint32_t adv) { return (n / 32u + adv - 1u) / adv; }
// ... 460 lines not shown
            }
            __builtin_amdgcn_s_sleep(1);
        }
        RSTAMP(0);
        const uint32_t plo = (uint32_t)pw, s = plo >> 12, tile = plo & 0xFFFu;
        const unsigned char* p = geo.ring + slot * (uint32_t)ring_slot_bytes<T>() + lane * (uint32_t)kRingRowBytes;

        {
        constexpr int OPL = 32 / D;
        constexpr int NSW = (OPL - 1) * D + T;
        constexpr int CW1 = (JS + NSW - 1) / 16;
        constexpr bool kResident = T <= 64;
        float k[kResident ? T : 1];
        if constexpr (kResident) {
#pragma unroll
            for (int t = 0; t < T; ++t) k[t] = taps[JS + t];
        }
        r_f32x2 acc[OPL];
#pragma unroll
        for (int q = 0; q < OPL; ++q) acc[q] = (r_f32x2){0.f, 0.f};
        r_f32x4 xw[2][8];
        auto rdw = [&](r_f32x4 (&x)[8], const int c) {
            const unsigned char* pc = p + coff(c);
#pragma unroll
            for (int q8 = 0; q8 < 8; ++q8) x[q8] = *reinterpret_cast<const r_f32x4*>(pc + 16 * q8);
        };
        rdw(xw[0], C0);
        if constexpr (CW1 > C0) rdw(xw[1], C0 + 1);
        ring_for_each_index([&](auto ci) {
            constexpr int c = C0 + decltype(ci)::value;
            const r_f32x4 (&x)[8] = xw[(c - C0) & 1];
            if constexpr (kResident) {
                HD_FIR_ARITH
#pragma unroll
                for (int j = 0; j < 16; ++j) {
                    const int slot_j = 16 * c + j;
                    const r_f32x2 smp = (j & 1) ? x[j >> 1].zw : x[j >> 1].xy;
#pragma unroll
                    for (int q = 0; q < OPL; ++q) {
                        const int t = slot_j - JS - D * q;
                        if (t >= 0 && t < T) acc[q] = acc[q] + smp * k[t];
                    }
                }
            } else {
                constexpr int TLO = 16 * c - JS - D * (OPL - 1) < 0 ? 0 : 16 * c - JS - D * (OPL - 1);
                constexpr int THI = 16 * c + 15 - JS >= T ? T - 1 : 16 * c + 15 - JS;
                constexpr int P0 = TLO / 2, NP = THI >= TLO ? THI / 2 - P0 + 1 : 0;
                typedef const r_f32x2 __attribute__((address_space(4)))* cpair_t;
                const cpair_t tp2 = (cpair_t)(uintptr_t)a.taps;
                r_f32x2 kp[NP > 0 ? NP : 1];
#pragma unroll
                for (int i = 0; i < NP; ++i) kp[i] = tp2[P0 + i];
                ring_for_each_index([&](auto ji) {
                    constexpr int j = decltype(ji)::value, slot_j = 16 * c + j, t0 = slot_j - JS;
                    const r_f32x2 smp = (j & 1) ? x[j >> 1].zw : x[j >> 1].xy;
                    constexpr bool odd = (t0 & 1) != 0;
                    ring_for_each_index([&](auto gi) {
                        constexpr int g = decltype(gi)::value, tg = t0 - D * 8 * g;
                        if constexpr (tg - D * 7 >= 0 && tg < T) {
                            ring_slot8<odd>(reinterpret_cast<r_f32x2 (&)[8]>(acc[8 * g]), smp, kp[(tg - 0 * D) / 2 - P0], kp[(tg - 1 * D) / 2 - P0],
                                            kp[(tg - 2 * D) / 2 - P0], kp[(tg - 3 * D) / 2 - P0], kp[(tg - 4 * D) / 2 - P0], kp[(tg - 5 * D) / 2 - P0],
                                            kp[(tg - 6 * D) / 2 - P0], kp[(tg - 7 * D) / 2 - P0]);
                        } else {
                            ring_for_each_index([&](auto qi) {
                                constexpr int q = 8 * g + decltype(qi)::value, t = t0 - D * q;
                                if constexpr (t >= 0 && t < T) ring_slot1<odd>(acc[q], smp, kp[t / 2 - P0]);
                            }, std::make_integer_sequence<int, 8>{});
                        }
                    }, std::make_integer_sequence<int, OPL / 8>{});
                }, std::make_integer_sequence<int, 16>{});
                __builtin_amdgcn_sched_barrier(0);
            }
            if constexpr (c + 2 <= CW1) rdw(xw[(c - C0) & 1], c + 2);
        }, std::make_integer_sequence<int, CW1 - C0 + 1>{});
        RSTAMP(1);
        __builtin_amdgcn_fence(__ATOMIC_RELEASE, "workgroup");
        if (lane == 0) __hip_atomic_store(&ctl->slot[slot], (unsigned long long)kSlotFree << 32, __ATOMIC_RELAXED, __HIP_MEMORY_SCOPE_WORKGROUP);
        const uint32_t o0 = (tile * 64u + lane) * (uint32_t)OPL;
        if (!a.call) {
            float2* dst = a.out + (size_t)s * a.out_stride + o0;
#pragma unroll
            for (int q = 0; q < OPL; q += 2) *reinterpret_cast<float4*>(dst + q) = make_float4(acc[q].x, acc[q].y, acc[q + 1].x, acc[q + 1].y);
        } else {
            const uint32_t pend = a.call[s].pend_before, ftake = a.call[s].fft_take, ffill = a.call[s].fft_fill;
            float2* dst = a.out + (size_t)s * a.out_stride + a.fir_hist_cap + pend + o0;
            if (((a.fir_hist_cap + pend) & 1u) == 0u) {
#pragma unroll
                for (int q = 0; q < OPL; q += 2) *reinterpret_cast<float4*>(dst + q) = make_float4(acc[q].x, acc[q].y, acc[q + 1].x, acc[q + 1].y);
            } else {
#pragma unroll
                for (int q = 0; q < OPL; ++q) dst[q] = make_float2(acc[q].x, acc[q].y);
            }
            if (a.fft_in && o0 < ftake) {
                float2* fd = a.fft_in + (size_t)s * kFftBins + ffill + o0;
                if (o0 + (uint32_t)OPL <= ftake && (ffill & 1u) == 0u) {
#pragma unroll
                    for (int q = 0; q < OPL; q += 2) *reinterpret_cast<float4*>(fd + q) = make_float4(acc[q].x, acc[q].y, acc[q + 1].x, acc[q + 1].y);
                } else {
#pragma unroll
                    for (int q = 0; q < OPL; ++q) if (o0 + (uint32_t)q < ftake) fd[q] = make_float2(acc[q].x, acc[q].y);
                }
            }
        }
        if (tile + 1 == a.ntiles) {
            const float2* in_s = a.in + (size_t)s * a.in_stride;
            float2* hout = a.hist_out + (size_t)s * (T - 1);
            for (uint32_t j = lane; j < (uint32_t)(T - 1); j += 64u) hout[j] = in_s[a.n - (T - 1) + j];
        }
        }
    }
}


template <int D> constexpr int work_row_bytes() { return D * 8 + 16; }
template <int D> constexpr int work_slot_bytes() { return 64 * work_row_bytes<D>(); }
template <int T, int D> constexpr int work_halo_rows() { return (T - 1 + D - 1) / D; }
static_assert(work_slot_bytes<32>() == kWorkSlotBytes && work_row_bytes<32>() == kRingRowBytes, "the /32 worker slot");

template <int NT>
__device__ __forceinline__ void glds16_x11(const void* base, const uint32_t* off, uint32_t lds_dst)
{
    unsigned keep, scc_keep;
#define HD_GN(n) "global_load_lds_dwordx4 %" #n ", %13 nt\n\ts_add_u32 m0, m0, 0x400\n\ts_nop 0\n\t"
#define HD_GD(n) "global_load_lds_dwordx4 %" #n ", %13\n\ts_add_u32 m0, m0, 0x400\n\ts_nop 0\n\t"
#define HD_G11_OPS : "=&s"(keep), "=&s"(scc_keep) : "v"(off[0]), "v"(off[1]), "v"(off[2]), "v"(off[3]), "v"(off[4]), "v"(off[5]), "v"(off[6]), "v"(off[7]), "v"(off[8]), "v"(off[9]), "v"(off[10]), "s"(base), "s"(lds_dst) : "memory"
#define HD_G11_HEAD "s_cselect_b32 %1, 1, 0\n\ts_mov_b32 %0, m0\n\ts_mov_b32 m0, %14\n\ts_nop 0\n\t"
#define HD_G11_TAIL "s_mov_b32 m0, %0\n\ts_cmp_lg_u32 %1, 0"
    if constexpr (NT >= 11)
        asm volatile(HD_G11_HEAD HD_GN(2) HD_GN(3) HD_GN(4) HD_GN(5) HD_GN(6) HD_GN(7) HD_GN(8) HD_GN(9) HD_GN(10) HD_GN(11) HD_GN(12) HD_G11_TAIL HD_G11_OPS);
    else
        asm volatile(HD_G11_HEAD HD_GN(2) HD_GN(3) HD_GN(4) HD_GN(5) HD_GN(6) HD_GN(7) HD_GN(8) HD_GD(9) HD_GD(10) HD_GD(11) HD_GD(12) HD_G11_TAIL HD_G11_OPS);
#undef HD_GN
#undef HD_GD
#undef HD_G11_OPS
#undef HD_G11_HEAD
#undef HD_G11_TAIL
}

template <int T, int D = 32>
__device__ __forceinline__ void ring_worker(const RingArgs& a, unsigned char* __restrict__ slot, unsigned char* keep_lds ,
                                            unsigned char* dump_lds ,
                                            const uint32_t role )
{
    static_assert(D == 32 || D == 64, "a row is one output's stride");
    constexpr int HR = work_halo_rows<T, D>();
    constexpr uint32_t ADV = 64u - (uint32_t)HR;
    constexpr int JS = HR * D - (T - 1);
    constexpr int NS = JS + T;
    constexpr int CPR = D / 2 + 1;
    constexpr int ROWB = work_row_bytes<D>();
    constexpr int NX = D / 2;
    constexpr int UPS = D / 32;
    constexpr int NU = (HR + 1) * UPS;
    constexpr int NB0 = ((int)ADV * CPR + 63) / 64;
    constexpr int HQ = D / 32;
    static_assert(NS == HR * D + 1, "the window ends with slot 0 of row HR");
    const uint32_t lane = threadIdx.x & 63u;
    typedef const float __attribute__((address_space(4)))* ctaps_t;
    const ctaps_t taps = (ctaps_t)(uintptr_t)a.taps - JS;
    const uint32_t dst = (uint32_t)__builtin_amdgcn_readfirstlane((int)lds_addr_of(slot));
    const unsigned char* p = slot + lane * (uint32_t)ROWB;
    const uint32_t rows = a.n / (uint32_t)D;
    RSTAMP_DECL;
    uint32_t n_done = 0; (void)n_done;

    uint32_t boff[CPR], hist_off[HR * HQ];
#pragma unroll
    for (int i = 0; i < CPR; ++i) { const uint32_t P = 64u * i + lane, row = P / (uint32_t)CPR, col = P - row * (uint32_t)CPR; boff[i] = row * (uint32_t)(D * 8) + (col < (uint32_t)(CPR - 1) ? col : (uint32_t)(CPR - 2)) * 16u; }
#pragma unroll
    for (int r = 0; r < HR * HQ; ++r) {
        const int h = (r / HQ - HR) * D + (r % HQ) * 32 + (int)(lane >> 1) + (T - 1);
        hist_off[r] = (uint32_t)(h < 0 ? 0 : h) * 8u + (lane & 1u) * 4u;
    }
    auto issue = [&](const uint32_t s, const int32_t row0, const bool run_start, const bool chained) {
        const unsigned char* in_s = reinterpret_cast<const unsigned char*>(a.in + (size_t)s * a.in_stride);
        if (row0 < 0) {
            const unsigned char* hb = reinterpret_cast<const unsigned char*>(a.hist_in + (size_t)s * (T - 1));
// ... 203 lines not shown
```

### habdec_amd/csrc/kernels/tail_body.h

```cpp
#pragma once
#include <hip/hip_runtime.h>

#include "arith.h"
#include "exact_math.h"
#include "launch.h"
#include "sym_common.h"
#include "spectrum_wave.h"
#include "tune.h"

namespace hd {
namespace HD_ARITH_NS {

constexpr uint32_t kTailHdrBytes = 64;
constexpr uint32_t kTailStrip = 512;

typedef float f32x4 __attribute__((ext_vector_type(4)));
typedef const float __attribute__((address_space(4)))* cfloat_ptr;
__device__ __forceinline__ cfloat_ptr as_const(const float* p) { return (cfloat_ptr)(uintptr_t)p; }

#define HD_TB_TAP4(A_, B_, C_, D_, k_)                                                        \
    {                                                                                         \
        HD_FIR_ARITH                                                                          \
        const f32x2 p0_ = (A_) * (k_), p1_ = (B_) * (k_), p2_ = (C_) * (k_), p3_ = (D_) * (k_); \
        a0 = a0 + p0_; a1 = a1 + p1_; a2 = a2 + p2_; a3 = a3 + p3_;                           \
// ... 30 lines not shown
{
    HD_FIR_ARITH
    f32x2 pr[OP];
#pragma unroll
    for (int q = 0; q < OP; ++q) {
        const f32x4 w = win[(D2 * q + U) >> 1];
        if constexpr (U & 1) pr[q] = w.zw * k; else pr[q] = w.xy * k;
    }
#pragma unroll
    for (int q = 0; q < OP; ++q) acc[q] = acc[q] + pr[q];
}

template <int NT>
__device__ __forceinline__ void tb_sync()
{
    if constexpr (NT == 64) {
        __builtin_amdgcn_fence(__ATOMIC_RELEASE, "workgroup");
        __builtin_amdgcn_wave_barrier();
        __builtin_amdgcn_fence(__ATOMIC_ACQUIRE, "workgroup");
    } else {
        __syncthreads();
    }
}

template <int NT, int OP, int D2, int T2>
__device__ __forceinline__ void tail_body(const TailArgs& a, const uint32_t s, unsigned char* __restrict__ lds)
{
    constexpr int P = NT * OP;
    constexpr int XCH = P * D2;
    constexpr int XN = (T2 - 1) + XCH;
    constexpr int XB = XCH / 2 / NT;
    constexpr int HB = (T2 - 1 + NT - 1) / NT;
    constexpr int NW = NT / 64;
    const uint32_t B = 2 * P + a.pend_max;
    static_assert(((T2 - 1) & 1) == 0 && XCH % (2 * NT) == 0, "16-byte pairs must stay aligned");
    const uint32_t tid = NT == 64 ? (threadIdx.x & 63u) : threadIdx.x, lane = tid & 63u, wave = tid >> 6;

    uint32_t* sh = reinterpret_cast<uint32_t*>(lds);
    float2* X = reinterpret_cast<float2*>(lds + kTailHdrBytes);
    constexpr bool kCompact = NT == 64;
    static_assert(!kCompact || 2 * NT + 2 <= XCH, "the exchange array must fit the dead part of the stage-1 image");
#ifdef HD_X_NOPAD
    constexpr bool kXPad = false;
#else
    constexpr bool kXPad = kCompact && OP == 4 && D2 == 2;
#endif
    auto xpos = [](uint32_t j) -> uint32_t { return kXPad ? j + 2u * (j >> 3) : j; };
    constexpr uint32_t kXStepH = kXPad ? NT + 2 * (NT >> 3) : NT, kXStepP = kXPad ? 2 * NT + 2 * (2 * NT >> 3) : 2 * NT, kXPiece = kXPad ? XCH + 2 * (XCH >> 3) : XCH;
    static_assert(NT % 8 == 0 && XCH % 8 == 0, "whole pad groups per step");
    const uint32_t xh0 = xpos(tid), xp0 = xpos((uint32_t)(T2 - 1) + 2u * tid);
    constexpr int YOFF = kXPad ? (((T2 - 2) + 2 * ((T2 - 2) >> 3) + 1 + 1) & ~1) : ((T2 - 1 + 1) & ~1);
    static_assert(!kXPad || YOFF + 2 * NT + 2 <= XN, "the exchange array must fit the dead part of the padded stage-1 image");
    float2* Y = kCompact ? X + YOFF : X + ((XN + 4 + 1) & ~1);
    float2* carryY = reinterpret_cast<float2*>(sh + 8);
    float2* F = reinterpret_cast<float2*>(lds + a.f_off);
    float* V = reinterpret_cast<float*>(lds + a.v_off);
    float* WS = reinterpret_cast<float*>(lds + a.ws_off);
    unsigned long long* words = reinterpret_cast<unsigned long long*>(lds + a.words_off);
    float* TP = reinterpret_cast<float*>(lds + a.tp_off);
    float* H2 = reinterpret_cast<float*>(lds + a.h2_off);

    TSTAMP_DECL;
    const StreamCall c = a.call[s];
    const uint2 tn = a.tune ? a.tune[s] : make_uint2(0u, 0u);
    const bool rot = tn.x != 0u;
    const uint32_t n1 = c.n1, n2 = c.n2, m = c.fir_m, T = c.fir_taps, pb = c.pend_before;
    const uint32_t H = T ? T - 1 : 0;
    const uint32_t Tp = sc_taps_prev(c) ? sc_taps_prev(c) : T;
    const bool run = m && T;
    const bool keepf = !c.clear_pending;
    const float2* in_s = a.dec1 + (size_t)s * a.dec1_stride;
    float2* cur = a.fbuf + (size_t)s * a.fbuf_stride;
    float2* nxt = a.fbuf_next + (size_t)s * a.fbuf_stride;
    float2* head_side = a.head_buf + (size_t)s * a.head_cap;
    const float2* head_prevbuf = a.fbuf_prev + (size_t)s * a.fbuf_stride + a.fir_hist_cap;
    const float2* head_in = sc_head_prev(c) ? head_prevbuf : head_side;
    const float* tp = a.lp_taps + (size_t)s * a.taps_stride;
    const uint32_t fhc = a.fir_hist_cap;


    const uint32_t ring_cap = a.ring_cap, rmask = ring_cap - 1;
    float* vring = a.ring + (size_t)s * ring_cap;
    float* gw = a.wsum + (size_t)s * ring_cap;
    unsigned long long* gmask = a.flipmask + (size_t)s * (ring_cap / 64);
    uint32_t* slot = a.slots + (size_t)s * a.slot_words;
    BitsHeader* hdr = reinterpret_cast<BitsHeader*>(slot);
    const SymState old = a.sym[s];
    const SymbolParams q = a.sp[s];
    const DemodCarry kin = a.carry_in[s];
    const uint32_t R = q.R;
    SymState st = old;
    bool search = false, do_sums = false;
    if (m) {
        st = state_after_push(old, q, m);
        search = !(st.held < q.min_held || st.held < q.spb);
        do_sums = search || !(q.min_held == 0xFFFFFFFFu || st.held < R);
    }
    const uint32_t end_old = old.base + old.held;
    uint32_t c0 = st.cached;
    uint32_t vcnt = 0;
    uint32_t ck0 = 0, ck1 = 0;
    unsigned long long carry_word = 0ull;
    const uint32_t old_cnt = do_sums ? end_old - c0 : 0u;

    const bool refold = Tp != T && !c.fir_zero_hist && run;
    const uint32_t head_n = refold ? sc_head_n(c) : 0u;
    auto fold = [&](uint32_t k) -> float2 {
        if (k < H && c.fir_zero_hist) return make_float2(0.f, 0.f);
        if (!refold || k >= H) return cur[fhc - H + k];
        if (k < Tp - 1) return cur[fhc - (Tp - 1) + k];
        const uint32_t h = k - (Tp - 1);
        return h < head_n ? head_in[h] : make_float2(0.f, 0.f);
    };
    const uint32_t f_old = H + pb;
    const float4* in4 = reinterpret_cast<const float4*>(in_s);
    const uint32_t n1p = n1 >> 1;
    float4 tx[XB];
    auto prefetch = [&](uint32_t pc) {
#pragma unroll
        for (int u = 0; u < XB; ++u) {
            const uint32_t k = pc * (XCH / 2) + tid + u * NT;
            tx[u] = k < n1p ? in4[k] : make_float4(0.f, 0.f, 0.f, 0.f);
        }
    };
    constexpr uint32_t kFirst = 256;
    const uint32_t take0 = min(old_cnt, kFirst);
    {
        float2 th[HB];
#pragma unroll
        for (int u = 0; u < HB; ++u) {
            const uint32_t k = tid + u * NT;
            th[u] = (k < (uint32_t)(T2 - 1) && !c.zero_hist2) ? a.hist2_in[(size_t)s * (T2 - 1) + k] : make_float2(0.f, 0.f);
        }
        prefetch(0);
        if (do_sums && (c0 & 63u)) carry_word = gmask[(c0 & rmask) >> 6] & ((1ull << (c0 & 63u)) - 1ull);
        constexpr int LB = 4;
        const bool special = c.fir_zero_hist || refold;
        constexpr int NB2 = ((T2 + 7) / 4 * 4 + NT - 1) / NT;
        if (T + 8 <= 4u * NT && f_old <= 8u * NT && R <= 4u * NT && !special) {
            float tt[4], t2[NB2], tv[4], tw[4];
            float2 tf[8];
#pragma unroll
            for (int u = 0; u < 4; ++u) { const uint32_t k = tid + u * NT; tt[u] = k < T ? tp[k] : 0.f; }
#pragma unroll
            for (int u = 0; u < NB2; ++u) { const uint32_t k = tid + u * NT; t2[u] = k < (uint32_t)T2 ? a.taps2[k] : 0.f; }
#pragma unroll
            for (int u = 0; u < 8; ++u) { const uint32_t k = tid + u * NT; tf[u] = k < f_old ? cur[fhc - H + k] : make_float2(0.f, 0.f); }
            if (do_sums) {
#pragma unroll
                for (int u = 0; u < 4; ++u) { const uint32_t k = tid + u * NT; tv[u] = k < take0 ? vring[(c0 + k) & rmask] : 0.f; }
#pragma unroll
                for (int u = 0; u < 4; ++u) { const uint32_t k = tid + u * NT; tw[u] = k < R ? gw[(c0 - R + k) & rmask] : 0.f; }
            }
#pragma unroll
            for (int u = 0; u < 4; ++u) { const uint32_t k = tid + u * NT; if (k < T + 8) TP[k] = tt[u]; }
#pragma unroll
            for (int u = 0; u < NB2; ++u) { const uint32_t k = tid + u * NT; if (k < (uint32_t)((T2 + 7) & ~3)) H2[k] = t2[u]; }
#pragma unroll
            for (int u = 0; u < 8; ++u) { const uint32_t k = tid + u * NT; if (k < f_old) F[k] = tf[u]; }
            if (do_sums) {
#pragma unroll
                for (int u = 0; u < 4; ++u) { const uint32_t k = tid + u * NT; if (k < take0) V[k] = tv[u]; }
#pragma unroll
                for (int u = 0; u < 4; ++u) { const uint32_t k = tid + u * NT; if (k < R) WS[k] = tw[u]; }
            }
        } else {
// ... 151 lines not shown
#pragma unroll
            for (int q = 0; q < OP; ++q) {
                const uint32_t th = tn.y + (o0 + OP * tid + q) * tn.x;
                const float2 cc = tab2[th >> 24], ff = tab2[kTuneTable + ((th >> 16) & 255u)];
                tpc[q] = make_float4(cc.x, cc.y, ff.x, ff.y);
            }
        }
#pragma unroll
        for (int u = 0; u < XB; ++u) {
            *reinterpret_cast<float4*>(X + xp0 + u * kXStepP) = tx[u];
        }
        tb_sync<NT>();
        if (pc + 1 < npieces) prefetch(pc + 1);
        TSTAMP(2);

        {
            constexpr int NWIN = ((D2 * (OP - 1) + 3) >> 1) + 1;
            const f32x4* h2 = reinterpret_cast<const f32x4*>(H2);
            const f32x4* px = reinterpret_cast<const f32x4*>(X + xpos((uint32_t)(OP * tid) * D2));
            f32x4 kc = h2[0];
            f32x2 acc[OP];
            f32x4 win[NWIN];
#pragma unroll
            for (int q = 0; q < OP; ++q) acc[q] = (f32x2){0.f, 0.f};
            constexpr int NB4 = T2 / 4;
            auto block = [&](const f32x4 n0, const f32x4 n1, const f32x4 kn) {
                __builtin_amdgcn_sched_barrier(0);
                tb_s2_tap<0, OP, D2, NWIN>(acc, win, kc.x);
                tb_s2_tap<1, OP, D2, NWIN>(acc, win, kc.y);
                tb_s2_tap<2, OP, D2, NWIN>(acc, win, kc.z);
                tb_s2_tap<3, OP, D2, NWIN>(acc, win, kc.w);
#pragma unroll
                for (int j = 0; j + 2 < NWIN; ++j) win[j] = win[j + 2];
                win[NWIN - 2] = n0; win[NWIN - 1] = n1;
                kc = kn;
            };
            if constexpr (kXPad) {
                static_assert(NWIN == 5, "the padded image's offsets below are those of four outputs per lane at /2");
#pragma unroll
                for (int j = 0; j < NWIN; ++j) win[j] = px[j + (j >> 2)];
                const f32x4* pq = px;
                int b = 0;
#pragma unroll 1
                for (; b + 2 <= NB4; b += 2, pq += 5) {
                    { const f32x4 n0 = pq[6], n1 = pq[7]; const f32x4 kn = h2[b + 1]; block(n0, n1, kn); }
                    { const f32x4 n0 = pq[8], n1 = pq[10]; const f32x4 kn = h2[b + 2]; block(n0, n1, kn); }
                }
                if (b < NB4) { const f32x4 n0 = pq[6], n1 = pq[7]; const f32x4 kn = h2[b + 1]; block(n0, n1, kn); }
            } else {
#pragma unroll
                for (int j = 0; j < NWIN; ++j) win[j] = px[j];
#pragma unroll 2
                for (int b = 0; b < NB4; ++b) {
                    const f32x4 n0 = px[2 * b + NWIN], n1 = px[2 * b + NWIN + 1];
                    const f32x4 kn = h2[b + 1];
                    block(n0, n1, kn);
                }
            }
            if constexpr (T2 % 4 >= 1) tb_s2_tap<0, OP, D2, NWIN>(acc, win, kc.x);
            if constexpr (T2 % 4 >= 2) tb_s2_tap<1, OP, D2, NWIN>(acc, win, kc.y);
            if constexpr (T2 % 4 >= 3) tb_s2_tap<2, OP, D2, NWIN>(acc, win, kc.z);
            TSTAMP(18);
            const bool keepF = keepf || npieces == 1;
            if (rot) {
                const uint32_t q4_lo = n1 - (uint32_t)(T2 - 1);
#pragma unroll
                for (int q = 0; q < OP; ++q) {
                    const uint32_t ol = OP * tid + q, oo = o0 + ol;
                    if (pc + 1 == npieces && n1 && ol < po && oo >= q4_lo && oo < n2)
                        a.hist2_out[(size_t)s * (T2 - 1) + (oo - q4_lo)] = make_float2(acc[q].x, acc[q].y);
                    float yr, yi;
                    tune_apply(tpc[q].x, tpc[q].y, tpc[q].z, tpc[q].w, acc[q].x, acc[q].y, yr, yi);
                    acc[q] = (f32x2){yr, yi};
                }
            }
            bool done4 = false;
            if constexpr (OP == 4) {
                const uint32_t oo = o0 + 4 * tid;
                if (4 * tid + 3 < po && !(pb & 1u)) {
                    const float4 y01 = make_float4(acc[0].x, acc[0].y, acc[1].x, acc[1].y), y23 = make_float4(acc[2].x, acc[2].y, acc[3].x, acc[3].y);
                    if (keepF) { float4* f4 = reinterpret_cast<float4*>(F + (f_old + oo - fbase)); f4[0] = y01; f4[1] = y23; }
                    { float4* c4 = reinterpret_cast<float4*>(cur + fhc + pb + oo); c4[0] = y01; c4[1] = y23; }
                    if (a.fft_in && oo < c.fft_take) {
                        float2* fi = a.fft_in + (size_t)s * kFftBins + c.fft_fill + oo;
                        if (oo + 3 < c.fft_take && !(c.fft_fill & 1u)) { reinterpret_cast<float4*>(fi)[0] = y01; reinterpret_cast<float4*>(fi)[1] = y23; }
                        else {
#pragma unroll
                            for (int q = 0; q < 4; ++q) if (oo + q < c.fft_take) fi[q] = make_float2(acc[q].x, acc[q].y);
                        }
                    }
                    done4 = true;
                }
            }
            if (!done4) {
#pragma unroll
                for (int q = 0; q < OP; ++q) {
                    const uint32_t ol = OP * tid + q;
                    if (ol < po) {
                        const uint32_t oo = o0 + ol;
                        const float2 y = make_float2(acc[q].x, acc[q].y);
                        if (keepF) F[f_old + oo - fbase] = y;
                        cur[fhc + pb + oo] = y;
                        if (a.fft_in && oo < c.fft_take) a.fft_in[(size_t)s * kFftBins + c.fft_fill + oo] = y;
                    }
                }
            }
        }
        float2 xt[HB];
#pragma unroll
        for (int u = 0; u < HB; ++u) { const uint32_t k = tid + u * NT; xt[u] = k < (uint32_t)(T2 - 1) ? X[xh0 + kXPiece + u * kXStepH] : make_float2(0.f, 0.f); }
        if (pc + 1 == npieces && n1) {
            tb_sync<NT>();
            for (uint32_t k = tid; k < (uint32_t)(T2 - 1); k += NT) {
                const uint32_t idx = n1 - (T2 - 1) + k;
                if (rot && idx < n2) continue;
                a.hist2_out[(size_t)s * (T2 - 1) + k] = idx < n2 ? F[f_old + idx - fbase] : in_s[idx];
            }
        }
        tb_sync<NT>();
#pragma unroll
        for (int u = 0; u < HB; ++u) { const uint32_t k = tid + u * NT; if (k < (uint32_t)(T2 - 1)) X[xh0 + u * kXStepH] = xt[u]; }
        fcount += po;
        TSTAMP(3);

        if (run && ((pc & 1u) || pc + 1 == npieces)) {
            const uint32_t i_hi = (pc + 1 == npieces) ? m : min(m, (pb + o0 + po) & ~1u);
            const f32x4* hk = reinterpret_cast<const f32x4*>(TP);
            float2* Yl = Y;
            if (kCompact) { if (tid == 0) Yl[0] = carryY[0]; }
            const uint32_t c0v = c0;
            for (uint32_t i0 = i_done; i0 < i_hi; i0 += 8 * NT) {
                const uint32_t live = min((uint32_t)(8 * NT), i_hi - i0);
                const uint32_t nvA = 4u * tid < live ? min(4u, live - 4u * tid) : 0u;
                const uint32_t nvB = 4u * NT + 4u * tid < live ? min(4u, live - 4u * NT - 4u * tid) : 0u;
                f32x2 a0 = {0.f, 0.f}, a1 = {0.f, 0.f}, a2 = {0.f, 0.f}, a3 = {0.f, 0.f};
                f32x2 b0 = {0.f, 0.f}, b1 = {0.f, 0.f}, b2 = {0.f, 0.f}, b3 = {0.f, 0.f};
                {
                    const f32x4* pA = reinterpret_cast<const f32x4*>(F + (i0 - fbase)) + 2 * tid;
                    const f32x4* pB = live > 4u * NT ? pA + 2 * NT : pA;
                    f32x4 A0 = pA[0], A1 = pA[1], A2 = pA[2], A3 = pA[3], A4, A5;
                    f32x4 B0 = pB[0], B1 = pB[1], B2 = pB[2], B3 = pB[3], B4, B5;
                    f32x4 kc = hk[0], k1, k2;
                    uint32_t t = 0;
                    for (; t + 12 <= T; t += 12) {
                        const uint32_t j = t >> 1, jk = t >> 2;
                        A4 = pA[j + 4]; A5 = pA[j + 5]; B4 = pB[j + 4]; B5 = pB[j + 5]; k1 = hk[jk + 1];
                        __builtin_amdgcn_sched_barrier(0);
                        HD_TB_BLK(A0, A1, A2, A3, kc, a0, a1, a2, a3)
                        HD_TB_BLK(B0, B1, B2, B3, kc, b0, b1, b2, b3)
                        A0 = pA[j + 6]; A1 = pA[j + 7]; B0 = pB[j + 6]; B1 = pB[j + 7]; k2 = hk[jk + 2];
                        __builtin_amdgcn_sched_barrier(0);
                        HD_TB_BLK(A2, A3, A4, A5, k1, a0, a1, a2, a3)
                        HD_TB_BLK(B2, B3, B4, B5, k1, b0, b1, b2, b3)
                        A2 = pA[j + 8]; A3 = pA[j + 9]; B2 = pB[j + 8]; B3 = pB[j + 9]; kc = hk[jk + 3];
                        __builtin_amdgcn_sched_barrier(0);
                        HD_TB_BLK(A4, A5, A0, A1, k2, a0, a1, a2, a3)
                        HD_TB_BLK(B4, B5, B0, B1, k2, b0, b1, b2, b3)
                    }
                    for (; t + 4 <= T; t += 4) {
                        const uint32_t j = t >> 1;
                        A4 = pA[j + 4]; A5 = pA[j + 5]; B4 = pB[j + 4]; B5 = pB[j + 5]; k1 = hk[(t >> 2) + 1];
                        HD_TB_BLK(A0, A1, A2, A3, kc, a0, a1, a2, a3)
                        HD_TB_BLK(B0, B1, B2, B3, kc, b0, b1, b2, b3)
                        A0 = A2; A1 = A3; A2 = A4; A3 = A5; B0 = B2; B1 = B3; B2 = B4; B3 = B5; kc = k1;
                    }
                    if (t < T) { HD_TB_TAPN(A0.xy, A0.zw, A1.xy, A1.zw, kc.x, a0, a1, a2, a3) HD_TB_TAPN(B0.xy, B0.zw, B1.xy, B1.zw, kc.x, b0, b1, b2, b3) ++t; }
                    if (t < T) { HD_TB_TAPN(A0.zw, A1.xy, A1.zw, A2.xy, kc.y, a0, a1, a2, a3) HD_TB_TAPN(B0.zw, B1.xy, B1.zw, B2.xy, kc.y, b0, b1, b2, b3) ++t; }
                    if (t < T) { HD_TB_TAPN(A1.xy, A1.zw, A2.xy, A2.zw, kc.z, a0, a1, a2, a3) HD_TB_TAPN(B1.xy, B1.zw, B2.xy, B2.zw, kc.z, b0, b1, b2, b3) ++t; }
                    const f32x2 lastA = nvA == 4 ? a3 : nvA == 3 ? a2 : nvA == 2 ? a1 : a0;
                    const f32x2 lastB = nvB == 4 ? b3 : nvB == 3 ? b2 : nvB == 2 ? b1 : b0;
                    Yl[1 + tid] = make_float2(lastA.x, lastA.y);
                    Yl[1 + NT + tid] = make_float2(lastB.x, lastB.y);
                }
                TSTAMP(12);
                tb_sync<NT>();
                {
                    f32x2 c0 = a0, c1 = a1, c2 = a2, c3 = a3;
                    uint32_t nv = nvA, i = i0 + 4 * tid;
                    float2 qv = Yl[tid];
#pragma unroll 1
                    for (int w = 0; w < 2; ++w) {
                        if (nv) {
                            float pr = qv.x, pi = qv.y;
                            if (i == 0 && !kin.primed) { pr = c0.x; pi = c0.y; }
                            float d[4];
                            d[0] = discriminate(c0.x, c0.y, pr, pi);
                            d[1] = discriminate(c1.x, c1.y, c0.x, c0.y);
                            d[2] = discriminate(c2.x, c2.y, c1.x, c1.y);
                            d[3] = discriminate(c3.x, c3.y, c2.x, c2.y);
                            const f32x2 av[4] = {c0, c1, c2, c3};
#pragma unroll
                            for (int u = 0; u < 4; ++u)
                                if ((uint32_t)u < nv) { const uint32_t b = __builtin_bit_cast(uint32_t, d[u]); ck0 += b; ck1 += (i + (uint32_t)u + 1u) * b; }
                            float* dm = a.demod + (size_t)s * a.demod_stride + i;
                            const uint32_t pos = end_old + i;
                            const float4 d4 = make_float4(d[0], d[1], d[2], d[3]);
                            if (nv == 4 && !(i & 3u)) *reinterpret_cast<float4*>(dm) = d4;
                            else {
                                if (nv >= 2) *reinterpret_cast<float2*>(dm) = make_float2(d[0], d[1]); else dm[0] = d[0];
                                if (nv == 4) *reinterpret_cast<float2*>(dm + 2) = make_float2(d[2], d[3]); else if (nv == 3) dm[2] = d[2];
                            }
                            if (nv == 4 && !(pos & 3u)) *reinterpret_cast<float4*>(vring + (pos & rmask)) = d4;
                            else {
#pragma unroll
                                for (int u = 0; u < 4; ++u) if ((uint32_t)u < nv) vring[(pos + u) & rmask] = d[u];
                            }
                            if (do_sums) {
                                if (nv == 4 && !((pos - c0v) & 3u)) *reinterpret_cast<float4*>(V + (pos - c0v)) = d4;
                                else {
#pragma unroll
                                    for (int u = 0; u < 4; ++u) if ((uint32_t)u < nv) V[pos + u - c0v] = d[u];
                                }
                            }
                            if (a.filtered) {
#pragma unroll
                                for (int u = 0; u < 4; ++u) if ((uint32_t)u < nv) a.filtered[(size_t)s * a.demod_stride + i + u] = make_float2(av[u].x, av[u].y);
                            }
                            if (i + nv == m) {
                                DemodCarry k; k.primed = 1; k._pad = 0;
                                const f32x2 lastv = nv == 4 ? c3 : nv == 3 ? c2 : nv == 2 ? c1 : c0;
                                k.re = lastv.x; k.im = lastv.y;
                                a.carry_out[s] = k;
                            }
                        }
                        c0 = b0; c1 = b1; c2 = b2; c3 = b3; nv = nvB; i = i0 + 4 * NT + 4 * tid; qv = Yl[NT + tid];
                    }
                }
                TSTAMP(14);
                tb_sync<NT>();
                {
                    const uint32_t lo = live - 1, lw = lo / (4u * NT), ll = (lo % (4u * NT)) >> 2;
                    if (tid == ll) { const float2 cy = Yl[1 + lw * NT + tid]; Yl[0] = cy; if (kCompact) carryY[0] = cy; }
                }
            }
            i_done = i_hi;
            TSTAMP(4);
            {
                const uint32_t shf = i_done - fbase, keep = fcount - shf;
                if (shf) {
                    tb_sync<NT>();
                    for (uint32_t k0 = 0; k0 < keep; k0 += 4 * NT) {
                        float2 t4[4];
#pragma unroll
                        for (int u = 0; u < 4; ++u) { const uint32_t k = k0 + tid + u * NT; t4[u] = k < keep ? F[k + shf] : make_float2(0.f, 0.f); }
                        tb_sync<NT>();
#pragma unroll
                        for (int u = 0; u < 4; ++u) { const uint32_t k = k0 + tid + u * NT; if (k < keep) F[k] = t4[u]; }
                    }
                    fbase = i_done; fcount = keep;
                }
            }
            TSTAMP(5);
            if (do_sums) vcnt = end_old + i_done - c0;
        }
        ++pc;
    }
    tb_sync<NT>();

    const uint32_t h = st.held;
    const uint32_t end = st.base + h;
    const uint32_t pend = end - R + 1;
    const bool hunt = m && do_sums && search;
    const uint32_t limit = hunt ? h - q.spb : 0u;
    const uint32_t carried_to = st.run_pos - st.base;
    const uint32_t wr0 = (st.base + R) & ~63u;
    const uint32_t nw = hunt ? ((st.base + limit) - wr0 + 63u) >> 6 : 0u;
    const uint32_t lmw = (nw + 1u) & ~1u;
    const uint32_t dyn_floats = hunt ? (((a.lds_bytes - a.dyn_off) - lmw * 8u) >> 2) & ~3u : 0u;
    const uint32_t vc_want = (hunt && limit > carried_to) ? limit - carried_to : 0u;
    const uint32_t woff = st.base & 3u, voff = (st.base + carried_to) & 3u;
    const uint32_t vc_cap = min((vc_want + voff + 7u) & ~3u, (dyn_floats * 5u / 8u) & ~3u);
    const uint32_t wc_cap = dyn_floats - vc_cap;
    const uint32_t wc_n = hunt ? min(limit, wc_cap > woff + 4u ? wc_cap - woff - 4u : 0u) : 0u;
    const uint32_t vc_n = min(vc_want, vc_cap > voff + 4u ? vc_cap - voff - 4u : 0u);
    const uint32_t wq_n = wc_n ? (wc_n + woff + 3u) >> 2 : 0u, vq_n = vc_n ? (vc_n + voff + 3u) >> 2 : 0u;
    const uint32_t wpos4 = st.base & ~3u, vpos4 = (st.base + carried_to) & ~3u;
    constexpr int MB = 512 / NT, CB = 1024 / NT / 4 > 0 ? 1024 / NT / 4 : 1, SB = CB;
    unsigned long long tm0[MB];
    float4 tc0[CB], ts0[SB];
    if (hunt) {
        __threadfence_block();
#pragma unroll
        for (int u = 0; u < MB; ++u) { const uint32_t i = tid + u * NT; tm0[u] = i < nw ? gmask[((wr0 + 64u * i) & rmask) >> 6] : 0ull; }
// ... 164 lines not shown
            const uint32_t cnt = min(kTailStrip, b - k0);
            const float4* s4 = reinterpret_cast<const float4*>(sb);
            uint32_t i = 0;
            if (cnt >= 32) {
                float4 cc[8], nn[8];
                auto ld = [&](float4 (&x)[8], const uint32_t at) {
#pragma unroll
                    for (int u = 0; u < 8; ++u) x[u] = s4[(at >> 2) + u];
                };
                auto adds = [&](const float4 (&x)[8]) {
#pragma unroll
                    for (int u = 0; u < 8; ++u) { acc = acc + x[u].x; acc = acc + x[u].y; acc = acc + x[u].z; acc = acc + x[u].w; }
                };
                ld(cc, 0u);
                for (; i + 96 <= cnt; i += 64) { ld(nn, i + 32); adds(cc); ld(cc, i + 64); adds(nn); }
                if (i + 64 <= cnt) { ld(nn, i + 32); adds(cc); adds(nn); i += 64; }
                else { adds(cc); i += 32; }
            }
            for (; i < cnt; ++i) acc = acc + sb[i];
            __builtin_amdgcn_wave_barrier();
        }
        return acc;
    };
    const uint32_t frontier = sh[2];
    for (uint32_t r = wave; r <= nfl; r += NW) {
        const bool tail_task = r == nfl;
        const uint32_t ra = r ? flips[r - 1] : 0u;
        uint32_t from, to;
        float acc0 = 0.0f;
        if (!tail_task) { to = flips[r]; from = r ? ra : min(carried_to, to); if (!r) acc0 = st.run_sum; }
        else { from = nfl ? ra : carried_to; to = max(from, frontier); if (!nfl) acc0 = st.run_sum; }
        const float acc = chain(acc0, from, to);
        if (lane == 0) {
            if (tail_task) sh[3] = __builtin_bit_cast(uint32_t, acc);
            else {
                const float mean = acc / (float)(to - ra);
                const uint32_t cnt = (uint32_t)roundf((float)(to - ra) / (float)q.spb);
                runinfo[r] = (cnt << 1) | (mean > 0.0f ? 1u : 0u);
            }
        }
    }
    tb_sync<NT>();
    TSTAMP(10);
    if (tid == 0) {
        uint32_t nbits = 0, curw = 0, overflow = sh[1];
        for (uint32_t r = 0; r < nfl; ++r) {
            const uint32_t bit = runinfo[r] & 1u;
            for (uint32_t k = runinfo[r] >> 1; k; --k) {
                if (nbits >= cap_bits) { overflow |= 1u; break; }
                curw |= bit << (nbits & 31);
                if ((nbits & 31) == 31) { outw[nbits >> 5] = curw; curw = 0; }
                ++nbits;
            }
        }
        if (nbits & 31) outw[nbits >> 5] = curw;
        if (a.flips_dbg)
            for (uint32_t r = 0; r < nfl && r < a.flips_cap; ++r) a.flips_dbg[(size_t)s * a.flips_cap + r] = flips[r];
        const uint32_t last = nfl ? flips[nfl - 1] : 0u;
        st.run_pos = st.base + max(nfl ? last : carried_to, frontier);
        st.run_sum = __builtin_bit_cast(float, sh[3]);
        st.cached = pend;
        st.base += last;
        st.held = h - last;
        a.sym[s] = st;
        hdr->nbits = nbits; hdr->held_after = st.held; hdr->nflips = nfl; hdr->overflow = overflow; hdr->uncached = end - st.cached;
    }
    TSTAMP(11);
    };
    second_half();
    {
#pragma unroll
        for (int o = 32; o >= 1; o >>= 1) { ck0 += (uint32_t)__shfl_xor((int)ck0, o, 64); ck1 += (uint32_t)__shfl_xor((int)ck1, o, 64); }
        if constexpr (NT == 64) {
            if (tid == 0) { hdr->demod_ck[0] = ck0; hdr->demod_ck[1] = ck1; hdr->demod_n = m; }
        } else {
            tb_sync<NT>();
            if (tid == 0) { sh[5] = 0; sh[6] = 0; }
            tb_sync<NT>();
            if (lane == 0) { atomicAdd(&sh[5], ck0); atomicAdd(&sh[6], ck1); }
            tb_sync<NT>();
            if (tid == 0) { hdr->demod_ck[0] = sh[5]; hdr->demod_ck[1] = sh[6]; hdr->demod_n = m; }
        }
    }
    if (a.fft_tw && c.fft_run) {
        __threadfence_block();
        tb_sync<NT>();
        if (wave == 0)
            spectrum_wave_body(a.fft_in + (size_t)s * kFftBins, a.fft_tw, a.spec, a.power, a.stats, s, a.rate, a.bins_sep, reinterpret_cast<float*>(lds + kTailHdrBytes), a.seq);
    }
    asm volatile("s_waitcnt vmcnt(0)" ::: "memory");
#ifdef HD_RING_FAULT
    if (tid == 0 && g_tail_fault_armed && atomicCAS(&g_tail_fault_fired, 0u, 1u) == 0u) return;
#endif
    if (tid == 0) __hip_atomic_store(&hdr->seq, a.seq, __ATOMIC_RELAXED, __HIP_MEMORY_SCOPE_SYSTEM);
    TSTAMP_WRITE();
}

}
}
```

Measured before the change: 503,500.

## Defer spectrum and demod output stores until a getter requests them

In pipelined modes the tail kernel no longer writes the full spectrum and power arrays per FFT run. It computes only the statistics, and the arrays are recomputed on demand by a separate spectrum launch when a getter asks for them. For this the FFT input buffer is double-buffered per stream so the last completed window survives. The per-sample demod array write is also dropped when the demod values already live in the symbol ring, and the getter reconstructs them from the ring. This cuts global-memory store traffic in the hot kernel, at the cost of extra getter latency, a synchronous launch, and doubled FFT input memory.

Measured after the change: 512,200 (median of 6 runs). 1.7% higher.

```diff
diff --git a/habdec_amd/csrc/dev_types.h b/habdec_amd/csrc/dev_types.h
--- a/habdec_amd/csrc/dev_types.h
+++ b/habdec_amd/csrc/dev_types.h
@@ -31,6 +31,11 @@
     uint32_t clear_pending;
     uint32_t fir_taps_prev;
 };
+__host__ __device__ inline uint32_t sc_fft_run(const StreamCall& c) { return c.fft_run & 3u; }
+__host__ __device__ inline uint32_t sc_fft_buf(const StreamCall& c) { return (c.fft_run >> 8) & 1u; }
+__host__ __device__ inline size_t sc_fft_row(const StreamCall& c, uint32_t s) { return ((size_t)s * 2u + sc_fft_buf(c)) * (size_t)kFftBins; }
+__host__ __device__ inline uint32_t sc_pack_fft_run(uint32_t run, uint32_t buf) { return (run & 3u) | ((buf & 1u) << 8); }
+
 __host__ __device__ inline uint32_t sc_taps_prev(const StreamCall& c) { return c.fir_taps_prev & 0xFFFFu; }
 __host__ __device__ inline uint32_t sc_head_n(const StreamCall& c) { return (c.fir_taps_prev >> 16) & 0x3FFFu; }
 __host__ __device__ inline bool sc_head_prev(const StreamCall& c) { return (c.fir_taps_prev >> 30) & 1u; }
diff --git a/habdec_amd/csrc/engine.cpp b/habdec_amd/csrc/engine.cpp
--- a/habdec_amd/csrc/engine.cpp
+++ b/habdec_amd/csrc/engine.cpp
@@ -83,6 +83,10 @@
     uint32_t win_ub = 0, inflight_m = 0;
     uint32_t last_n2 = 0, last_pend_before = 0, last_m = 0;
     int last_buf = 0;
+    uint8_t fft_buf = 0;
+    uint8_t spec_buf = 0;
+    bool spec_stale = false;
+    bool demod_in_ring = false;
 };
 
 struct StreamHost {
@@ -132,6 +136,7 @@
     bool decode_enabled = true;
     bool fast = false;
     bool one_stream = false;
+    bool lazy_spectra = false;
     bool no_tail = false;
     uint32_t tail_max_n2 = 2048;
     int last_route = -1;
@@ -192,6 +197,7 @@
     uint32_t head_cap = 0;
     DevBuf<hd::SymbolParams> d_sym;
     PinBuf<hd::SymbolParams> h_sym;
+    PinBuf<hd::StreamCall> h_spec_call;
     static constexpr int kSlots = 4;
     struct CallSlot {
         DevBuf<hd::StreamCall> d_call;
@@ -324,6 +330,7 @@
     HD_HIP(hipStreamCreateWithFlags(&e->qa, hipStreamNonBlocking));
     e->one_stream = cfg->pipeline == 0;
     e->no_tail = getenv("HD_NO_TAIL") != nullptr;
+    { const char* v = getenv("HD_EAGER_SPECTRA"); e->lazy_spectra = cfg->pipeline >= 1 && cfg->enable_spectrum && !(v && atoi(v)); }
     e->no_claim = getenv("HD_NO_CLAIM") != nullptr;
     if (const char* v = getenv("HD_STEP_RUN")) e->step_run = (uint32_t)atoi(v);
     e->no_cu_step = getenv("HD_NO_CU_STEP") != nullptr;
@@ -439,7 +446,8 @@
         HD_HIP(hipMemcpy(e->tune_tab.p, tab.data(), tab.size() * sizeof(float), hipMemcpyHostToDevice));
     }
     if (cfg->enable_spectrum) {
-        HD_HIP(e->fft_in.alloc((size_t)S * hd::kFftBins));
+        HD_HIP(e->fft_in.alloc((size_t)S * 2 * hd::kFftBins));
+        if (e->lazy_spectra) HD_HIP(e->h_spec_call.alloc(S));
         HD_HIP(e->spec.alloc((size_t)S * hd::kFftBins));
         HD_HIP(e->power.alloc((size_t)S * hd::kFftBins));
         for (auto& sl : e->slot) HD_HIP(sl.h_stats.alloc(S));
@@ -721,7 +729,7 @@
         };
         for (uint32_t s = 0; s < e->S && !e->device_failed && !timing_experiment; ++s) {
             await(&reinterpret_cast<const volatile hd::BitsHeader*>(sl.h_slots.p + (size_t)s * e->slot_words)->seq, "result slot", s);
-            if (!e->device_failed && e->cfg.enable_spectrum && sl.h_stats.p && sl.h_call.p[s].fft_run)
+            if (!e->device_failed && e->cfg.enable_spectrum && sl.h_stats.p && hd::sc_fft_run(sl.h_call.p[s]))
                 await(reinterpret_cast<const volatile uint32_t*>(&sl.h_stats.p[s].seq), "spectrum statistics", s);
         }
         std::atomic_thread_fence(std::memory_order_acquire);
@@ -740,7 +748,7 @@
     for (uint32_t s = 0; s < e->S; ++s) {
         StreamHost& st = e->st[s];
         const hd::StreamCall& c = sl.h_call.p[s];
-        if (c.fft_run) {
+        if (hd::sc_fft_run(c)) {
             std::memcpy(&st.stats, &sl.h_stats.p[s], sizeof(st.stats));
             st.have_spectrum = true;
             ++st.spectra;
@@ -879,7 +887,12 @@
             c.fft_take = (uint32_t)std::min<size_t>(hd::kFftBins - nx.fft_fill, c.n2);
             nx.fft_fill += c.fft_take;
         }
-        if (e->cfg.enable_spectrum && n && nx.fft_fill >= (size_t)hd::kFftBins) { c.fft_run = 1; nx.fft_fill = 0; p.any_fft = true; }
+        c.fft_run = hd::sc_pack_fft_run(0, nx.fft_buf);
+        if (e->cfg.enable_spectrum && n && nx.fft_fill >= (size_t)hd::kFftBins) {
+            c.fft_run = hd::sc_pack_fft_run(1, nx.fft_buf); nx.fft_fill = 0; p.any_fft = true;
+            nx.spec_buf = nx.fft_buf;
+            if (e->lazy_spectra) nx.fft_buf ^= 1u;
+        }
         const bool past_batch_gate = n && nx.pending >= hd::kFirBatch;
         nx.last_m = 0;
         if (past_batch_gate && !e->decode_enabled) { c.clear_pending = 1; nx.pending = 0; }
@@ -951,17 +964,19 @@
     if (r.route != Route::separate || !e->cfg.enable_spectrum || r.any_post || !p.any_fft) return;
     for (uint32_t s = 0; s < S; ++s) {
         hd::StreamCall& c = sl.h_call.p[s];
-        if (c.fft_run == 1 && c.fft_fill == 0 && c.fft_take == (uint32_t)hd::kFftBins) { c.fft_take = 0; c.fft_run = 2; }
+        if (hd::sc_fft_run(c) == 1 && c.fft_fill == 0 && c.fft_take == (uint32_t)hd::kFftBins) { c.fft_take = 0; c.fft_run = hd::sc_pack_fft_run(2, hd::sc_fft_buf(c)); }
     }
     r.spectrum_on_qc = !e->one_stream && p.nst != 0;
-    for (uint32_t s = 0; s < S && r.spectrum_on_qc; ++s) r.spectrum_on_qc = sl.h_call.p[s].fft_run != 1u;
-}
+    for (uint32_t s = 0; s < S && r.spectrum_on_qc; ++s) r.spectrum_on_qc = hd::sc_fft_run(sl.h_call.p[s]) != 1u;
+}
+
+bool demod_in_ring(const hd_engine* e, Route route) { return e->cfg.pipeline >= 1 && route != Route::separate; }
 
 void fill_tail(const hd_engine* e, const hd_engine::CallSlot& sl, const CallPlan& p, const CallRoute& r, const CallBufs& b, hd::TailArgs& t)
 {
     t.dec1 = b.d1; t.dec1_stride = e->n1_cap; t.hist2_in = e->hist2[b.hin].p; t.hist2_out = e->hist2[b.hout].p; t.taps2 = e->stage_taps[1].p;
     t.fbuf = b.fcur; t.fbuf_next = b.fnext; t.fbuf_stride = e->fbuf_stride; t.fir_hist_cap = e->fir_hist_cap;
-    t.lp_taps = e->lp_taps.p; t.taps_stride = e->taps_cap; t.demod = e->demod.p; t.demod_stride = e->demod.n / e->S;
+    t.lp_taps = e->lp_taps.p; t.taps_stride = e->taps_cap; t.demod = demod_in_ring(e, r.route) ? nullptr : e->demod.p; t.demod_stride = e->demod.n / e->S;
     t.filtered = e->cfg.keep_filtered ? e->filtered.p : nullptr; t.carry_in = e->carry[b.cin].p; t.carry_out = e->carry[b.cout].p;
     t.tune = p.any_tune ? sl.h_tune.dev : nullptr; t.tune_tab = e->tune_tab.p;
     t.call = r.dcall; t.fft_in = r.feed; t.head_buf = e->fir_head.p; t.fbuf_prev = b.fprev; t.head_cap = e->head_cap;
@@ -970,7 +985,7 @@
     t.sp = e->d_sym.p; t.slots = sl.h_slots.dev; t.slot_words = e->slot_words; t.seq = sl.seq;
     t.flips_dbg = e->flips_cap ? e->flips_dbg.p : nullptr; t.flips_cap = e->flips_cap;
     t.fft_tw = r.feed ? e->fft_tw.p : nullptr;
-    t.spec = e->spec.p; t.power = e->power.p; t.stats = sl.h_stats.dev; t.rate = e->fsd; t.bins_sep = e->bins_sep;
+    t.spec = e->lazy_spectra ? nullptr : e->spec.p; t.power = e->lazy_spectra ? nullptr : e->power.p; t.stats = sl.h_stats.dev; t.rate = e->fsd; t.bins_sep = e->bins_sep;
 }
 
 hd::StepClaim make_claim(const hd_engine* e, const CallPlan& p, uint32_t run_len_cu )
@@ -1239,6 +1254,13 @@
 void commit_call(hd_engine* e, hd_engine::CallSlot& sl, const CallPlan& p, const CallRoute& r)
 {
     e->mirror.swap(e->mirror_next);
+    const bool in_ring = demod_in_ring(e, r.route);
+    const bool lazy = e->lazy_spectra && r.route != Route::separate;
+    for (uint32_t s = 0; s < e->S; ++s) {
+        SizeState& sz = e->mirror[s];
+        sz.demod_in_ring = in_ring;
+        if (hd::sc_fft_run(sl.h_call.p[s])) sz.spec_stale = lazy;
+    }
     sl.busy = true;
     if (r.route == Route::step) {
         e->pend.valid = true; e->pend.ta = r.ta_step; e->pend.slot = (int)(e->calls % hd_engine::kSlots);
@@ -1492,15 +1514,47 @@
     return HD_OK;
 }
 
+static int refresh_spectra(hd_engine* e)
+{
+    if (!e->lazy_spectra) return HD_OK;
+    bool any = false;
+    for (uint32_t s = 0; s < e->S; ++s) {
+        const SizeState& sz = e->mirror[s];
+        e->h_spec_call.p[s].fft_run = sz.spec_stale ? hd::sc_pack_fft_run(1, sz.spec_buf) : 0u;
+        any |= sz.spec_stale;
+    }
+    if (!any) return HD_OK;
+    HD_HIP(hipSetDevice(e->cfg.device));
+    hd::launch_spectrum_wave(e->qa, e->S, e->fft_in.p, e->fft_tw.p, e->spec.p, e->power.p, nullptr, e->h_spec_call.dev, e->fsd, e->bins_sep, 0u);
+    HD_HIP(hipGetLastError());
+    HD_HIP(hipStreamSynchronize(e->qa));
+    for (SizeState& sz : e->mirror) sz.spec_stale = false;
+    return HD_OK;
+}
+static bool getter_ready(hd_engine* e)
+{
+    if (e->in_callback) { fail(HD_ERR_INVALID, "data getters cannot be called from a sentence / character callback (text getters can)"); return false; }
+    (void)flush_locked(e);
+    return true;
+}
+static bool copy_to_host(hd_engine* e, void* host, const void* dev, size_t bytes)
+{
+    return !bytes || (hipSetDevice(e->cfg.device) == hipSuccess && hipMemcpy(host, dev, bytes, hipMemcpyDeviceToHost) == hipSuccess);
+}
 static size_t fetch(hd_engine* e, const void* dev, size_t count, size_t elem, void* host, size_t cap)
 {
-    if (e->in_callback) { fail(HD_ERR_INVALID, "data getters cannot be called from a sentence / character callback (text getters can)"); return 0; }
-    (void)flush_locked(e);
+    if (!getter_ready(e)) return 0;
     const size_t n = std::min(count, cap);
     if (!n || !host) return count;
-    if (hipSetDevice(e->cfg.device) != hipSuccess) return 0;
-    if (hipMemcpy(host, dev, n * elem, hipMemcpyDeviceToHost) != hipSuccess) return 0;
-    return count;
+    return copy_to_host(e, host, dev, n * elem) ? count : 0;
+}
+
+static size_t fetch_spectrum(hd_engine* e, const void* dev, size_t elem, void* host, size_t cap)
+{
+    if (!getter_ready(e) || refresh_spectra(e) != HD_OK) return 0;
+    const size_t n = std::min<size_t>(hd::kFftBins, cap);
+    if (!n || !host) return hd::kFftBins;
+    return copy_to_host(e, host, dev, n * elem) ? (size_t)hd::kFftBins : 0;
 }
 
 size_t hd_stream_spectrum(hd_engine* e, uint32_t s, float* iq, size_t cap)
@@ -1508,20 +1562,30 @@
     if (check_stream(e, s)) return 0;
     std::lock_guard<std::recursive_mutex> l(e->mtx);
     if (!e->cfg.enable_spectrum || !e->st[s].have_spectrum) return 0;
-    return fetch(e, e->spec.p + (size_t)s * hd::kFftBins, hd::kFftBins, sizeof(float2), iq, cap);
+    return fetch_spectrum(e, e->spec.p + (size_t)s * hd::kFftBins, sizeof(float2), iq, cap);
 }
 size_t hd_stream_power(hd_engine* e, uint32_t s, float* p, size_t cap)
 {
     if (check_stream(e, s)) return 0;
     std::lock_guard<std::recursive_mutex> l(e->mtx);
     if (!e->cfg.enable_spectrum || !e->st[s].have_spectrum) return 0;
-    return fetch(e, e->power.p + (size_t)s * hd::kFftBins, hd::kFftBins, sizeof(float), p, cap);
+    return fetch_spectrum(e, e->power.p + (size_t)s * hd::kFftBins, sizeof(float), p, cap);
 }
 size_t hd_stream_demodulated(hd_engine* e, uint32_t s, float* v, size_t cap)
 {
     if (check_stream(e, s)) return 0;
     std::lock_guard<std::recursive_mutex> l(e->mtx);
-    return fetch(e, e->demod.p + (size_t)s * (e->demod.n / e->S), e->mirror[s].last_m, sizeof(float), v, cap);
+    const SizeState& sz = e->mirror[s];
+    if (!sz.demod_in_ring) return fetch(e, e->demod.p + (size_t)s * (e->demod.n / e->S), sz.last_m, sizeof(float), v, cap);
+    if (!getter_ready(e)) return 0;
+    const size_t count = sz.last_m, n = std::min(count, cap);
+    if (!n || !v) return count;
+    hd::SymState st;
+    if (!copy_to_host(e, &st, e->d_symstate.p + s, sizeof(st))) return 0;
+    const float* ring = e->tail.p + (size_t)s * e->tail_cap;
+    const uint32_t first = (st.base + st.held - (uint32_t)count) & (e->tail_cap - 1u);
+    const size_t n0 = std::min<size_t>(n, e->tail_cap - first);
+    return copy_to_host(e, v, ring + first, n0 * sizeof(float)) && copy_to_host(e, v + n0, ring, (n - n0) * sizeof(float)) ? count : 0;
 }
 size_t hd_stream_decimated(hd_engine* e, uint32_t s, float* iq, size_t cap)
 {
diff --git a/habdec_amd/csrc/kernels/decimate.hip b/habdec_amd/csrc/kernels/decimate.hip
--- a/habdec_amd/csrc/kernels/decimate.hip
+++ b/habdec_amd/csrc/kernels/decimate.hip
@@ -79,8 +79,8 @@
     float2* tile = reinterpret_cast<float2*>(tile4);
     float2* ytile = tile + ((NL + 1) & ~1);
 
-    struct CallHead { uint32_t n_in, n1, n2, zero_hist1, zero_hist2, pend_before, fft_fill, fft_take; };
-    static_assert(sizeof(CallHead) == 32, "CallHead mirrors the head of StreamCall");
+    struct CallHead { uint32_t n_in, n1, n2, zero_hist1, zero_hist2, pend_before, fft_fill, fft_take, fft_run; };
+    static_assert(sizeof(CallHead) == 36, "CallHead mirrors the head of StreamCall");
     const bool linear = lin_ntiles != 0;
     uint32_t s, first, count;
     const bool claimed = claim.ctr != nullptr && claim.run_len >= 2;
@@ -434,7 +434,7 @@
         nv_prev = o < nout ? min((uint32_t)OPL, nout - o) : 0u;
         dst_prev = out + (size_t)s * out_stride + (final_stage ? (size_t)fir_hist_cap + c.pend_before : 0) + o;
         nf_prev = (fft_in && o < c.fft_take) ? min((uint32_t)OPL, c.fft_take - o) : 0u;
-        fdst_prev = fft_in ? fft_in + (size_t)s * kFftBins + c.fft_fill + o : nullptr;
+        fdst_prev = fft_in ? fft_in + ((size_t)s * 2u + ((c.fft_run >> 8) & 1u)) * kFftBins + c.fft_fill + o : nullptr;
         __syncthreads();
         DSTAMP(3);
         ++tile_i;
diff --git a/habdec_amd/csrc/kernels/fir_demod.hip b/habdec_amd/csrc/kernels/fir_demod.hip
--- a/habdec_amd/csrc/kernels/fir_demod.hip
+++ b/habdec_amd/csrc/kernels/fir_demod.hip
@@ -248,7 +248,7 @@
     const StreamCall c = call[s];
     const uint32_t j = blockIdx.x * blockDim.x + threadIdx.x;
     if (j >= c.fft_take) return;
-    fft_in[(size_t)s * kFftBins + c.fft_fill + j] = fbuf[(size_t)s * stride + fir_hist_cap + c.pend_before + j];
+    fft_in[sc_fft_row(c, s) + c.fft_fill + j] = fbuf[(size_t)s * stride + fir_hist_cap + c.pend_before + j];
 }
 
 __global__ void k_fetch_params(const uint4* __restrict__ host_src, uint4* __restrict__ dst, uint32_t n16)
diff --git a/habdec_amd/csrc/kernels/launch.h b/habdec_amd/csrc/kernels/launch.h
--- a/habdec_amd/csrc/kernels/launch.h
+++ b/habdec_amd/csrc/kernels/launch.h
@@ -28,7 +28,7 @@
     const float2* hist2_in; float2* hist2_out; const float* taps2;
     float2* fbuf; float2* fbuf_next; size_t fbuf_stride; uint32_t fir_hist_cap;
     const float* lp_taps; uint32_t taps_stride;
-    float* demod; size_t demod_stride; float2* filtered;
+    float* demod ; size_t demod_stride; float2* filtered;
     const DemodCarry* carry_in; DemodCarry* carry_out;
     const StreamCall* call; float2* fft_in;
     float2* head_buf ; const float2* fbuf_prev ; uint32_t head_cap, n_streams;
diff --git a/habdec_amd/csrc/kernels/spectrum_wave.h b/habdec_amd/csrc/kernels/spectrum_wave.h
--- a/habdec_amd/csrc/kernels/spectrum_wave.h
+++ b/habdec_amd/csrc/kernels/spectrum_wave.h
@@ -140,31 +140,36 @@
     }
     specwave::fft64(a);
     specwave::finish4096<16>(a, tw4096, plane, l);
-    float2* so = spec + (size_t)s * kFftBins;
-    float* po = power + (size_t)s * kFftBins;
     int mybad = 0;
     double lsum = 0.0;
 #define HD_SW_P(j_) a[specwave::xpos(((j_) + 32) & 63)].x
-    float2* sg = so;
-    float* pg = po;
-#pragma unroll
-    for (int j = 0; j < 64; ++j) {
-        if ((j & 7) == 0) {
-            __builtin_amdgcn_sched_barrier(0);
-            sg = so + 64 * j; pg = po + 64 * j;
-            asm volatile("" : "+s"(sg), "+s"(pg));
-        }
-        const int k2 = (j + 32) & 63;
-        const f32x2 v = a[specwave::xpos(k2)];
-        sg[l + 64 * (j & 7)] = make_float2(v.x, v.y);
-        float q = (v.x * v.x + v.y * v.y) / (float)kFftBins;
-        q = q * q;
-        q = (float)((double)q / rate);
-        q = 10.0f * log10f(q);
-        if (v.x != v.x || v.y != v.y || isinf(v.x) || isinf(v.y) || q != q || isinf(q)) mybad = 1;
-        HD_SW_P(j) = q;
-        pg[l + 64 * (j & 7)] = q;
-        lsum += (double)q;
+    const bool store = spec != nullptr;
+#pragma unroll
+    for (int g = 0; g < 64; g += 8) {
+        __builtin_amdgcn_sched_barrier(0);
+        if (store) {
+            float2* sg = spec + (size_t)s * kFftBins + 64 * g;
+            asm volatile("" : "+s"(sg));
+#pragma unroll
+            for (int u = 0; u < 8; ++u) { const f32x2 v = a[specwave::xpos((g + u + 32) & 63)]; sg[l + 64 * u] = make_float2(v.x, v.y); }
+        }
+#pragma unroll
+        for (int u = 0; u < 8; ++u) {
+            const f32x2 v = a[specwave::xpos((g + u + 32) & 63)];
+            float q = (v.x * v.x + v.y * v.y) / (float)kFftBins;
+            q = q * q;
+            q = (float)((double)q / rate);
+            q = 10.0f * log10f(q);
+            if (v.x != v.x || v.y != v.y || isinf(v.x) || isinf(v.y) || q != q || isinf(q)) mybad = 1;
+            HD_SW_P(g + u) = q;
+            lsum += (double)q;
+        }
+        if (store) {
+            float* pg = power + (size_t)s * kFftBins + 64 * g;
+            asm volatile("" : "+s"(pg));
+#pragma unroll
+            for (int u = 0; u < 8; ++u) pg[l + 64 * u] = HD_SW_P(g + u);
+        }
     }
     const bool bad = __builtin_amdgcn_ballot_w64(mybad != 0) != 0ull;
     const double mean = specwave::wave_sum(lsum) / (double)kFftBins;
@@ -193,7 +198,7 @@
         if (i >= lo && i < hi && pj > floor0 && abs(i - p1) > bins_sep / 2 && pj > cv) { cv = pj; ci = i; }
     }
     specwave::wave_argmax(cv, ci);
-    if (l == 0) {
+    if (l == 0 && stats) {
         int pa = p1, pb = 0;
         float av = p1v, bvv = floor0;
         if (ci < (int)kFftBins) { pb = ci; bvv = cv; }
diff --git a/habdec_amd/csrc/kernels/spectrum_wave.hip b/habdec_amd/csrc/kernels/spectrum_wave.hip
--- a/habdec_amd/csrc/kernels/spectrum_wave.hip
+++ b/habdec_amd/csrc/kernels/spectrum_wave.hip
@@ -11,9 +11,10 @@
 {
     __shared__ float plane[64 * 65];
     const uint32_t s = blockIdx.x;
-    const uint32_t run = call[s].fft_run;
+    const StreamCall c = call[s];
+    const uint32_t run = sc_fft_run(c);
     if (!run) return;
-    const float2* x = run == 2u ? chunk + (size_t)s * chunk_stride + fir_hist_cap + call[s].pend_before : fft_in + (size_t)s * kFftBins;
+    const float2* x = run == 2u ? chunk + (size_t)s * chunk_stride + fir_hist_cap + c.pend_before : fft_in + sc_fft_row(c, s);
     spectrum_wave_body(x, tw4096, spec, power, stats, s, rate, bins_sep, plane, seq);
 }
 
diff --git a/habdec_amd/csrc/kernels/stage1_ring.h b/habdec_amd/csrc/kernels/stage1_ring.h
--- a/habdec_amd/csrc/kernels/stage1_ring.h
+++ b/habdec_amd/csrc/kernels/stage1_ring.h
@@ -566,7 +566,7 @@
 #pragma unroll
             for (int q = 0; q < OPL; q += 2) *reinterpret_cast<float4*>(dst + q) = make_float4(acc[q].x, acc[q].y, acc[q + 1].x, acc[q + 1].y);
         } else {
-            const uint32_t pend = a.call[s].pend_before, ftake = a.call[s].fft_take, ffill = a.call[s].fft_fill;
+            const uint32_t pend = a.call[s].pend_before, ftake = a.call[s].fft_take, ffill = a.call[s].fft_fill, fbuf = (a.call[s].fft_run >> 8) & 1u;
             float2* dst = a.out + (size_t)s * a.out_stride + a.fir_hist_cap + pend + o0;
             if (((a.fir_hist_cap + pend) & 1u) == 0u) {
 #pragma unroll
@@ -576,7 +576,7 @@
                 for (int q = 0; q < OPL; ++q) dst[q] = make_float2(acc[q].x, acc[q].y);
             }
             if (a.fft_in && o0 < ftake) {
-                float2* fd = a.fft_in + (size_t)s * kFftBins + ffill + o0;
+                float2* fd = a.fft_in + ((size_t)s * 2u + fbuf) * kFftBins + ffill + o0;
                 if (o0 + (uint32_t)OPL <= ftake && (ffill & 1u) == 0u) {
 #pragma unroll
                     for (int q = 0; q < OPL; q += 2) *reinterpret_cast<float4*>(fd + q) = make_float4(acc[q].x, acc[q].y, acc[q + 1].x, acc[q + 1].y);
diff --git a/habdec_amd/csrc/kernels/tail_body.h b/habdec_amd/csrc/kernels/tail_body.h
--- a/habdec_amd/csrc/kernels/tail_body.h
+++ b/habdec_amd/csrc/kernels/tail_body.h
@@ -136,6 +136,7 @@
     const uint32_t ring_cap = a.ring_cap, rmask = ring_cap - 1;
     float* vring = a.ring + (size_t)s * ring_cap;
     float* gw = a.wsum + (size_t)s * ring_cap;
+    float* const dm_row = a.demod ? a.demod + (size_t)s * a.demod_stride : nullptr;
     unsigned long long* gmask = a.flipmask + (size_t)s * (ring_cap / 64);
     uint32_t* slot = a.slots + (size_t)s * a.slot_words;
     BitsHeader* hdr = reinterpret_cast<BitsHeader*>(slot);
@@ -453,7 +454,7 @@
                     if (keepF) { float4* f4 = reinterpret_cast<float4*>(F + (f_old + oo - fbase)); f4[0] = y01; f4[1] = y23; }
                     { float4* c4 = reinterpret_cast<float4*>(cur + fhc + pb + oo); c4[0] = y01; c4[1] = y23; }
                     if (a.fft_in && oo < c.fft_take) {
-                        float2* fi = a.fft_in + (size_t)s * kFftBins + c.fft_fill + oo;
+                        float2* fi = a.fft_in + sc_fft_row(c, s) + c.fft_fill + oo;
                         if (oo + 3 < c.fft_take && !(c.fft_fill & 1u)) { reinterpret_cast<float4*>(fi)[0] = y01; reinterpret_cast<float4*>(fi)[1] = y23; }
                         else {
 #pragma unroll
@@ -472,7 +473,7 @@
                         const float2 y = make_float2(acc[q].x, acc[q].y);
                         if (keepF) F[f_old + oo - fbase] = y;
                         cur[fhc + pb + oo] = y;
-                        if (a.fft_in && oo < c.fft_take) a.fft_in[(size_t)s * kFftBins + c.fft_fill + oo] = y;
+                        if (a.fft_in && oo < c.fft_take) a.fft_in[sc_fft_row(c, s) + c.fft_fill + oo] = y;
                     }
                 }
             }
@@ -563,13 +564,15 @@
 #pragma unroll
                             for (int u = 0; u < 4; ++u)
                                 if ((uint32_t)u < nv) { const uint32_t b = __builtin_bit_cast(uint32_t, d[u]); ck0 += b; ck1 += (i + (uint32_t)u + 1u) * b; }
-                            float* dm = a.demod + (size_t)s * a.demod_stride + i;
                             const uint32_t pos = end_old + i;
                             const float4 d4 = make_float4(d[0], d[1], d[2], d[3]);
-                            if (nv == 4 && !(i & 3u)) *reinterpret_cast<float4*>(dm) = d4;
-                            else {
-                                if (nv >= 2) *reinterpret_cast<float2*>(dm) = make_float2(d[0], d[1]); else dm[0] = d[0];
-                                if (nv == 4) *reinterpret_cast<float2*>(dm + 2) = make_float2(d[2], d[3]); else if (nv == 3) dm[2] = d[2];
+                            if (dm_row) {
+                                float* dm = dm_row + i;
+                                if (nv == 4 && !(i & 3u)) *reinterpret_cast<float4*>(dm) = d4;
+                                else {
+                                    if (nv >= 2) *reinterpret_cast<float2*>(dm) = make_float2(d[0], d[1]); else dm[0] = d[0];
+                                    if (nv == 4) *reinterpret_cast<float2*>(dm + 2) = make_float2(d[2], d[3]); else if (nv == 3) dm[2] = d[2];
+                                }
                             }
                             if (nv == 4 && !(pos & 3u)) *reinterpret_cast<float4*>(vring + (pos & rmask)) = d4;
                             else {
@@ -900,11 +903,11 @@
             if (tid == 0) { hdr->demod_ck[0] = sh[5]; hdr->demod_ck[1] = sh[6]; hdr->demod_n = m; }
         }
     }
-    if (a.fft_tw && c.fft_run) {
+    if (a.fft_tw && sc_fft_run(c)) {
         __threadfence_block();
         tb_sync<NT>();
         if (wave == 0)
-            spectrum_wave_body(a.fft_in + (size_t)s * kFftBins, a.fft_tw, a.spec, a.power, a.stats, s, a.rate, a.bins_sep, reinterpret_cast<float*>(lds + kTailHdrBytes), a.seq);
+            spectrum_wave_body(a.fft_in + sc_fft_row(c, s), a.fft_tw, a.spec, a.power, a.stats, s, a.rate, a.bins_sep, reinterpret_cast<float*>(lds + kTailHdrBytes), a.seq);
     }
     asm volatile("s_waitcnt vmcnt(0)" ::: "memory");
 #ifdef HD_RING_FAULT
```
